# feldroop/floxer

Hardware: AMD Instinct MI355X
Metric: aligned reads/sec, 10 kb ONT-like reads @ 8 % error vs a GRCh38-size reference (seed-and-verify path, CIGAR) (higher is better)
Workload: dtype u64

## Files before the change

### floxer_amd/__init__.py

```python
import ctypes as C

import numpy as np

from . import capi
from .capi import FloxerError, check, lib, ptr, as_u8, u8p, u32p, u64p

if capi.os.path.exists(capi.LIB_PATH):
    lib()

CIGAR_OPS = "MIDNSHP=X"
NULL_ID = 0xFFFFFFFF

ORDER = {"errors_first": 0, "count_first": 1, "none": 2}
CHOICE = {"round_robin": 0, "full_groups": 1, "first_reported": 2}
MODE_EXISTS, MODE_WITHOUT_CIGAR, MODE_WITH_CIGAR = 0, 1, 2


def hw_queue_request():
    requested, found = C.c_int(0), C.c_int(-1)
    check(lib().flx_hw_queue_request(C.byref(requested), C.byref(found)))
    return requested.value, found.value


def cigar_string(words):
# ... 21 lines not shown

def reverse_complement_rank(r):
    r = as_u8(r)
    out = np.zeros_like(r)
    lib().flx_reverse_complement_rank(ptr(r, u8p), len(r), ptr(out, u8p))
    return out


class pex_tree:

    def __init__(self, total_query_length, query_num_errors, leaf_max_num_errors, bottom_up=False):
        cap = 4 * (query_num_errors + 2) + 16
        nodes = (capi.PexNode * cap)()
        ni, nl = C.c_uint64(), C.c_uint64()
        check(lib().flx_pex_tree_build(total_query_length, query_num_errors, leaf_max_num_errors, int(bottom_up), nodes, cap,
                                       C.byref(ni), C.byref(nl)))
        rows = [(n.parent_id, n.from_, n.to, n.num_errors) for n in nodes[: ni.value + nl.value]]
        self.inner_nodes = rows[: ni.value]
        self.leaves = rows[ni.value:]

    def root(self):
        return self.inner_nodes[0] if self.inner_nodes else self.leaves[0]

    def get_leaves(self):
        return self.leaves

    def generate_seeds(self, step=1):
        return [(l[1], l[2] - l[1] + 1, l[3], i) for i, l in enumerate(self.leaves)][::step]


class fmindex:
    def __init__(self, references=None, path=None, device=None):
        self.h = C.c_void_p()
        if path is not None and references is None:
            check(lib().flx_index_load(path.encode(), C.byref(self.h)))
        else:
            refs = [as_u8(r) for r in references]
            pool = np.concatenate(refs) if refs else np.zeros(0, np.uint8)
            lens = np.array([len(r) for r in refs], dtype=np.uint64)
            if device is None:
                check(lib().flx_index_build(ptr(pool, u8p), ptr(lens, u64p), len(refs), C.byref(self.h)))
            else:
                check(lib().flx_index_build_on_device(int(device), ptr(pool, u8p), ptr(lens, u64p), len(refs), C.byref(self.h)))

    def save(self, path):
        check(lib().flx_index_save(self.h, path.encode()))

    def meta(self):
        n = C.c_uint64(0)
        lib().flx_index_meta_export(self.h, None, C.byref(n))
        buf = np.zeros(n.value, dtype=np.uint8)
        check(lib().flx_index_meta_export(self.h, ptr(buf, u8p), C.byref(n)))
        return buf.tobytes()

    @classmethod
    def from_meta(cls, meta):
        self = cls.__new__(cls)
        self.h = C.c_void_p()
        buf = np.frombuffer(meta, dtype=np.uint8).copy()
        check(lib().flx_index_meta_import(ptr(buf, u8p), len(buf), C.byref(self.h)))
        return self

    def image_layout(self):
        out = np.zeros(5, dtype=np.uint64)
        check(lib().flx_index_image_layout(self.h, ptr(out, u64p)))
        return [int(x) for x in out]

    def image_upload(self, device, pointers):
        arr = (C.c_void_p * 5)(*[C.c_void_p(int(p)) for p in pointers])
        check(lib().flx_index_image_upload(self.h, int(device), arr))

    def __del__(self):
        if getattr(self, "h", None):
            lib().flx_index_free(self.h)
            self.h = None

    @property
    def text_length(self):
        return lib().flx_index_text_length(self.h)

    @property
    def num_references(self):
        return lib().flx_index_num_references(self.h)

    @property
    def device_bytes(self):
        return lib().flx_index_device_bytes(self.h)

    @property
    def derived_device_bytes(self):
        return lib().flx_index_derived_device_bytes(self.h)

    def suffix_array(self):
        out = np.zeros(self.text_length, dtype=np.uint64)
        check(lib().flx_index_copy_sa(self.h, ptr(out, u64p)))
        return out

    def suffix_array_u32(self):
        out = np.empty(self.text_length, dtype=np.uint32)
        check(lib().flx_index_copy_sa_u32(self.h, ptr(out, u32p)))
        return out

    def bwt(self, reversed_text=False):
        out = np.zeros(self.text_length, dtype=np.uint8)
        check(lib().flx_index_copy_bwt(self.h, int(reversed_text), ptr(out, u8p)))
        return out


class context:

    def __init__(self, index, device=0, image=None):
        self.index = index
        self.image = image
        self.h = C.c_void_p()
        if image is None:
            check(lib().flx_ctx_create(device, index.h, C.byref(self.h)))
        else:
            arr = (C.c_void_p * 5)(*[C.c_void_p(int(b.data_ptr())) for b in image])
            sizes = np.array([int(b.numel()) * int(b.element_size()) for b in image], dtype=np.uint64)
            check(lib().flx_ctx_create_on_image(device, index.h, arr, ptr(sizes, u64p), C.byref(self.h)))

    def close(self):
        if getattr(self, "h", None):
            lib().flx_ctx_destroy(self.h)
            self.h = None

    __del__ = close

    def set_stream(self, hip_stream):
        check(lib().flx_ctx_set_stream(self.h, hip_stream))

    def enable_kernel_timing(self, on=True):
        check(lib().flx_ctx_enable_kernel_timing(self.h, int(on)))

    def reset_kernel_stats(self):
        check(lib().flx_ctx_reset_kernel_stats(self.h))

    def path_counters(self, reset=False):
        pc = capi.PathCounters()
        check(lib().flx_ctx_get_path_counters(self.h, C.byref(pc)))
        if reset:
            check(lib().flx_ctx_reset_path_counters(self.h))
        out = {n: int(getattr(pc, n)) for n, _ in capi.PathCounters._fields_ if n != "reserved"}
        out["records_dropped"] = int(pc.reserved[0])
        out["partial_records"] = int(pc.reserved[1])
        out["reads_rescued"] = int(pc.reserved[2])
        out["reads_split"] = int(pc.reserved[3])
        return out

    def search_counters(self):
        sc = capi.SearchCounters()
        check(lib().flx_ctx_get_search_counters(self.h, C.byref(sc)))
        return {n: int(getattr(sc, n)) for n, _ in capi.SearchCounters._fields_ if n != "reserved"}

    def derived_info(self):
        di = capi.DerivedInfo()
        check(lib().flx_ctx_derived_info(self.h, C.byref(di)))
        return {n: int(getattr(di, n)) for n, _ in capi.DerivedInfo._fields_ if n != "reserved"}

    def copy_derived(self, which):
        if which == "isa":
            out = np.empty(self.index.text_length, dtype=np.uint32)
        else:
            out = np.empty((4 ** self.derived_info()["filter_k"] + 63) // 64, dtype=np.uint64)
        check(lib().flx_ctx_copy_derived(self.h, {"isa": 0, "filter": 1, "filter_mirrored": 2}[which], out.ctypes.data_as(C.c_void_p), out.nbytes))
        return out

    def lane_overlap(self, n_lanes, iterations):
        start, stop = (C.c_float * n_lanes)(), (C.c_float * n_lanes)()
        check(lib().flx_ctx_lane_overlap(self.h, n_lanes, iterations, start, stop))
        return list(start), list(stop)

    def kernel_stats(self):
        arr = (capi.KernelStat * 64)()
        n = C.c_uint32(64)
        check(lib().flx_ctx_get_kernel_stats(self.h, arr, C.byref(n)))
        return {a.name.decode(): dict(launches=a.launches, device_ms=a.device_ms, algorithmic_bytes=a.algorithmic_bytes,
                                      work_units=a.work_units) for a in arr[: n.value]}


class statistics:

    def __init__(self, input_hint=None):
        self.h = C.c_void_p()
        check(lib().flx_stats_create(input_hint.encode() if input_hint else None, C.byref(self.h)))

    def __del__(self):
        if getattr(self, "h", None):
            lib().flx_stats_free(self.h)
            self.h = None

    def attach(self, ctx):
        check(lib().flx_ctx_set_stats(ctx.h, self.h))
        return self

    @property
    def num_queries(self):
        return lib().flx_stats_num_queries(self.h)

    def format(self, toml=True):
        n = C.c_uint64(0)
        lib().flx_stats_format(self.h, int(toml), None, C.byref(n))
        buf = C.create_string_buffer(n.value)
        check(lib().flx_stats_format(self.h, int(toml), buf, C.byref(n)))
        return buf.value.decode()


def search_config(max_num_anchors_hard=500, max_num_anchors_soft=50, anchor_group_order="count_first",
                  anchor_choice_strategy="round_robin", erase_useless_anchors=True):
    return capi.SearchConfig(max_num_anchors_hard, max_num_anchors_soft, ORDER[anchor_group_order], CHOICE[anchor_choice_strategy],
                             int(erase_useless_anchors), 0)


class searcher:
    def __init__(self, ctx, config=None):
        self.ctx = ctx
        self.config = config or search_config()

    def _seeds(self, seeds):
        arr = (capi.Seed * len(seeds))()
        for i, (off, ln, err, leaf) in enumerate(seeds):
            arr[i] = capi.Seed(off, ln, err, leaf, 0)
        return arr

    def search_seeds(self, sequence, seeds):
        seq = as_u8(sequence)
        arr = self._seeds(seeds)
        cap = max(64, len(seeds) * (self.config.max_num_anchors_soft + 1))
        out = (capi.Anchor * cap)()
        n = C.c_uint64(cap)
        stats = (capi.SeedStats * max(1, len(seeds)))()
        check(lib().flx_search_seeds(self.ctx.h, ptr(seq, u8p), len(seq), arr, len(seeds), C.byref(self.config), out, C.byref(n), stats))
        anchors = np.array([(a.seed_index, a.pex_leaf_index, a.reference_id, a.reference_position, a.num_errors) for a in out[: n.value]],
                           dtype=np.uint64).reshape(-1, 5)
        st = np.array([(s.num_kept_useful_anchors, s.num_kept_raw_anchors, s.num_excluded_raw_anchors_by_soft_cap, s.fully_excluded)
                       for s in stats[: len(seeds)]], dtype=np.uint64).reshape(-1, 4)
        return anchors, st

    def search_groups(self, sequence, seeds, max_hits=501):
        seq = as_u8(sequence)
        arr = self._seeds(seeds)
        cap = 1 << 16
        while True:
            out = (capi.HitGroup * cap)()
            n = C.c_uint64(cap)
            rc = lib().flx_search_groups(self.ctx.h, ptr(seq, u8p), len(seq), arr, len(seeds), max_hits, out, C.byref(n))
            if rc == -3:
                cap = n.value
                continue
            check(rc)
            break
        return np.array([(g.seed_index, g.lb, g.len, g.num_errors) for g in out[: n.value]], dtype=np.uint64).reshape(-1, 4)


def align_batch(ctx, query_pool, jobs, reference_pool=None, md=False, gaps=None):
    q = as_u8(query_pool)
    arr = (capi.AlignJob * max(1, len(jobs)))()
    cap_words = 16
    for i, (ro, rl, qo, ql, k, mode) in enumerate(jobs):
        arr[i] = capi.AlignJob(ro, qo, rl, ql, k, mode)
        cap_words += 2 * k + 2
    res = (capi.AlignResult * max(1, len(jobs)))()
    cig = np.zeros(cap_words, dtype=np.uint32)
    words = C.c_uint64(cap_words)
    if reference_pool is None:
        rp, rl_ = None, 0
    else:
        ref = as_u8(reference_pool)
        rp, rl_ = ptr(ref, u8p), len(ref)
    if md:
        cap_md = 16 + sum(8 * k + 6 for (_, _, _, _, k, mode) in jobs if mode == MODE_WITH_CIGAR)
        refs = (capi.MdRef * max(1, len(jobs)))()
        mdp = np.zeros(cap_md, dtype=np.uint8)
        md_bytes = C.c_uint64(cap_md)
        if gaps is not None:
            check(lib().flx_align_batch_gaps(ctx.h, rp, rl_, ptr(q, u8p), len(q), arr, len(jobs), res, ptr(cig, u32p), C.byref(words),
                                             refs, ptr(mdp, u8p), C.byref(md_bytes), C.byref(gaps)))
        else:
            check(lib().flx_align_batch_md(ctx.h, rp, rl_, ptr(q, u8p), len(q), arr, len(jobs), res, ptr(cig, u32p), C.byref(words),
                                           refs, ptr(mdp, u8p), C.byref(md_bytes)))
        out = []
        for r, m in zip(res[: len(jobs)], refs[: len(jobs)]):
            out.append((r.num_errors, r.begin, cigar_string(cig[r.cigar_offset: r.cigar_offset + r.cigar_length]),
                        mdp[m.offset: m.offset + m.length].tobytes() if m.length else None) if r.exists else None)
        return out
    if gaps is not None:
        check(lib().flx_align_batch_gaps(ctx.h, rp, rl_, ptr(q, u8p), len(q), arr, len(jobs), res, ptr(cig, u32p), C.byref(words),
                                         None, None, None, C.byref(gaps)))
    else:
        check(lib().flx_align_batch(ctx.h, rp, rl_, ptr(q, u8p), len(q), arr, len(jobs), res, ptr(cig, u32p), C.byref(words)))
    out = []
    for r in res[: len(jobs)]:
        out.append((r.num_errors, r.begin, cigar_string(cig[r.cigar_offset: r.cigar_offset + r.cigar_length])) if r.exists else None)
    return out


def _realign_room(options):
    if options is None or not options.enable:
        return (lambda nm: 2 * nm + 2), (lambda nm: 8 * nm + 6)
    sc = {k: int(getattr(options, k)) or v for k, v in REALIGN_DEFAULTS.items()}
    c_max = max(sc["match"] + sc["mismatch"], sc["gap_open"] + sc["gap_extend"] + sc["match"])
    c_min = min(sc["match"] + sc["mismatch"], sc["gap_open"] + sc["gap_extend"])
    col_min = min(sc["match"] + sc["mismatch"], sc["gap_extend"])
    return (lambda nm: max(2 * nm + 2, 2 * (nm * c_max // c_min) + 1)), (lambda nm: 8 * (nm * c_max // col_min) + 6)


# ... 1395 lines not shown
```

### floxer_amd/capi.py

```python
import ctypes as C
import importlib.util
import os
import sys

import numpy as np

_HERE = os.path.dirname(os.path.abspath(__file__))
LIB_PATH = os.environ.get("FLX_LIBRARY") or os.path.join(_HERE, "libfloxer_amd.so")

u8p = C.POINTER(C.c_uint8)
u32p = C.POINTER(C.c_uint32)
u64p = C.POINTER(C.c_uint64)


class FloxerError(RuntimeError):
    pass


class PexNode(C.Structure):
    _fields_ = [("parent_id", C.c_uint32), ("from_", C.c_uint32), ("to", C.c_uint32), ("num_errors", C.c_uint32)]


class Seed(C.Structure):
    _fields_ = [("seq_offset", C.c_uint64), ("length", C.c_uint32), ("num_errors", C.c_uint32), ("pex_leaf_index", C.c_uint32),
# ... 100 lines not shown
    _fields_ = [("offset", C.c_uint64), ("length", C.c_uint32), ("num_errors", C.c_uint32), ("score", C.c_int32), ("diag_lo", C.c_int32),
                ("diag_hi", C.c_int32), ("kept", C.c_uint32)]


class RealignCounters(C.Structure):
    _fields_ = [("paths_realigned", C.c_uint64), ("paths_changed", C.c_uint64), ("paths_kept", C.c_uint64), ("reserved", C.c_uint64 * 5)]


class CsOptions(C.Structure):
    _fields_ = [("form", C.c_uint32), ("reserved", C.c_uint32 * 7)]


CsJob = LeftAlignJob


class CoverageOptions(C.Structure):
    _fields_ = [("count_deletions", C.c_uint32), ("count_secondary", C.c_uint32), ("min_mapq", C.c_uint32), ("report_zero", C.c_uint32),
                ("reserved", C.c_uint32 * 4)]


class DepthRun(C.Structure):
    _fields_ = [("reference_id", C.c_int32), ("depth", C.c_uint32), ("start", C.c_uint64), ("end", C.c_uint64)]


class DepthWindow(C.Structure):
    _fields_ = [("reference_id", C.c_int32), ("max_depth", C.c_uint32), ("start", C.c_uint64), ("end", C.c_uint64), ("depth_sum", C.c_uint64),
                ("covered", C.c_uint64)]


class PileupOptions(C.Structure):
    _fields_ = [("count_secondary", C.c_uint32), ("min_mapq", C.c_uint32), ("min_depth", C.c_uint32), ("min_count", C.c_uint32),
                ("min_permille", C.c_uint32), ("reserved", C.c_uint32 * 3)]


class PileupSite(C.Structure):
    _fields_ = [("reference_id", C.c_int32), ("position", C.c_uint32), ("depth", C.c_uint32), ("del_", C.c_uint32), ("ins", C.c_uint32),
                ("alt", C.c_uint32 * 4), ("reserved", C.c_uint32)]


class SvOptions(C.Structure):
    _fields_ = [("min_length", C.c_uint32), ("max_distance", C.c_uint32), ("min_support", C.c_uint32), ("count_secondary", C.c_uint32),
                ("min_mapq", C.c_uint32), ("reserved", C.c_uint32 * 3), ("initial_capacity", C.c_uint64)]


class SvSignature(C.Structure):
    _fields_ = [("type", C.c_uint32), ("side_a", C.c_uint32), ("side_b", C.c_uint32), ("reserved", C.c_uint32), ("ref_a", C.c_int32),
                ("ref_b", C.c_int32), ("pos_a", C.c_uint32), ("q", C.c_uint32)]


class SvCluster(C.Structure):
    _fields_ = [("type", C.c_uint32), ("side_a", C.c_uint32), ("side_b", C.c_uint32), ("support", C.c_uint32), ("ref_a", C.c_int32),
                ("ref_b", C.c_int32), ("pos_a_min", C.c_uint32), ("pos_a_max", C.c_uint32), ("q_min", C.c_uint32), ("q_median", C.c_uint32),
                ("q_max", C.c_uint32), ("reserved", C.c_uint32)]


class ErrprofOptions(C.Structure):
    _fields_ = [("count_secondary", C.c_uint32), ("min_mapq", C.c_uint32), ("flush_threshold", C.c_uint32), ("reserved", C.c_uint32 * 5)]


class ConsensusOptions(C.Structure):
    _fields_ = [("count_secondary", C.c_uint32), ("min_mapq", C.c_uint32), ("min_depth", C.c_uint32), ("min_count", C.c_uint32),
                ("min_permille", C.c_uint32), ("mask_low_depth", C.c_uint32), ("reserved", C.c_uint32 * 2)]


class ConsensusChange(C.Structure):
    _fields_ = [("reference_id", C.c_int32), ("position", C.c_uint32), ("kind", C.c_uint32), ("ref_rank", C.c_uint32), ("alt_rank", C.c_uint32),
                ("length", C.c_uint32), ("count", C.c_uint32), ("cov", C.c_uint32), ("letters", C.c_uint64)]


class ConsensusAllele(C.Structure):
    _fields_ = [("reference_id", C.c_int32), ("position", C.c_uint32), ("length", C.c_uint32), ("count", C.c_uint32), ("letters", C.c_uint64)]


class VariantsOptions(C.Structure):
    _fields_ = [("count_secondary", C.c_uint32), ("min_mapq", C.c_uint32), ("min_depth", C.c_uint32), ("min_qual", C.c_uint32), ("max_del", C.c_uint32),
                ("cost_match", C.c_uint32), ("cost_mismatch", C.c_uint32), ("cost_het", C.c_uint32), ("prior_het", C.c_uint32), ("prior_hom", C.c_uint32),
                ("reserved", C.c_uint32 * 2)]


class Variant(C.Structure):
    _fields_ = [("reference_id", C.c_int32), ("position", C.c_uint32), ("kind", C.c_uint32), ("ref_rank", C.c_uint32), ("alt_rank", C.c_uint32),
                ("length", C.c_uint32), ("ref_count", C.c_uint32), ("alt_count", C.c_uint32), ("cov", C.c_uint32), ("gt", C.c_uint32), ("gq", C.c_uint32),
                ("qual", C.c_uint32), ("pl", C.c_uint32 * 3), ("reserved", C.c_uint32), ("letters", C.c_uint64)]


class VariantAllele(C.Structure):
    _fields_ = [("reference_id", C.c_int32), ("position", C.c_uint32), ("kind", C.c_uint32), ("length", C.c_uint32), ("count", C.c_uint32),
                ("reserved", C.c_uint32), ("letters", C.c_uint64)]


ERRPROF_SECTIONS = (("PAIR_EQ", 36), ("PAIR_X", 36), ("INS_LEN", 64), ("DEL_LEN", 64), ("INS_LETTER", 6), ("DEL_LETTER", 6), ("HP_DEL", 34), ("HP_INS", 34),
                    ("POS_MATCH", 100), ("POS_MISMATCH", 100), ("POS_INS", 100), ("POS_CLIP", 100), ("POS_DEL", 100), ("EQ_RUN", 256), ("IDENTITY", 101),
                    ("TOTALS", 8), ("reserved", 7))


class ErrprofTable(C.Structure):
    _fields_ = [(name, C.c_uint64 * n) for name, n in ERRPROF_SECTIONS]


class SortOptions(C.Structure):
    _fields_ = [("initial_capacity", C.c_uint64), ("tile_keys", C.c_uint32), ("reserved", C.c_uint32 * 5)]


class SortEntry(C.Structure):
    _fields_ = [("ordinal", C.c_uint64), ("reference_id", C.c_int32), ("position", C.c_int32), ("end", C.c_uint32), ("flag", C.c_uint32)]


class PafSummary(C.Structure):
    _fields_ = [(n, C.c_uint32) for n in ("query_start", "query_end", "ref_end", "matches", "mismatches", "ins_bases", "del_bases", "gap_opens")]


class PafOptions(C.Structure):
    _fields_ = [("write_cigar", C.c_uint32), ("write_unmapped", C.c_uint32), ("mapq_from_records", C.c_uint32), ("skip_secondary", C.c_uint32),
                ("reserved", C.c_uint32 * 4)]


class TailJob(C.Structure):
    _fields_ = [("cigar_offset", C.c_uint64), ("cigar_length", C.c_uint32), ("error_weight", C.c_uint32), ("x_drop", C.c_uint32),
                ("min_tail_rows", C.c_uint32)]


class TailResult(C.Structure):
    _fields_ = [(n, C.c_uint32) for n in ("left_rows", "left_cols", "left_errors", "left_words", "right_rows", "right_cols", "right_errors",
                                          "right_words")]


class ExtendJob(C.Structure):
    _fields_ = [("text_pos", C.c_uint64), ("q_pos", C.c_uint64), ("ref_limit", C.c_uint32), ("row_limit", C.c_uint32),
                ("direction", C.c_int32), ("error_weight", C.c_uint32), ("x_drop", C.c_uint32), ("max_errors", C.c_uint32)]


class ExtendResult(C.Structure):
    _fields_ = [("rows", C.c_uint32), ("cols", C.c_uint32), ("errors", C.c_uint32), ("stop_reason", C.c_uint32)]


class PartialCandidate(C.Structure):
    _fields_ = [("read_index", C.c_uint64), ("q_from", C.c_uint32), ("q_to", C.c_uint32), ("orientation", C.c_uint32),
                ("reference_id", C.c_int32), ("start", C.c_uint64), ("nm", C.c_uint32), ("cigar_length", C.c_uint32),
                ("cigar_offset", C.c_uint64)]


class MdRef(C.Structure):
    _fields_ = [("offset", C.c_uint64), ("length", C.c_uint32), ("reserved", C.c_uint32)]


class PathCounters(C.Structure):
    _fields_ = [(n, C.c_uint64) for n in ("seeds", "seeds_with_anchors", "seeds_excluded_by_hard_cap", "seeds_selected_on_host", "anchors",
                                          "cursor_extensions", "inner_tests_requested", "root_alignments_requested",
                                          "root_alignments_found", "records", "reads", "search_reruns")] + [("reserved", C.c_uint64 * 4)]


class SearchCounters(C.Structure):
    _fields_ = [(n, C.c_uint64) for n in ("launches", "subtrees_queued", "lane_handovers", "wave_handovers", "walks_abandoned")] + [("reserved", C.c_uint64 * 3)]


class ClimbAnchor(C.Structure):
    _fields_ = [("read", C.c_uint32), ("orientation", C.c_uint32), ("leaf", C.c_uint32), ("reference_id", C.c_uint32), ("position", C.c_uint64)]


class ClimbOptions(C.Structure):
    _fields_ = [("driver", C.c_uint32), ("reserved", C.c_uint32 * 3)]


class DerivedInfo(C.Structure):
    _fields_ = [(n, C.c_uint32) for n in ("filter_k", "filter_tmin", "have_isa", "have_filter", "have_filter_mirrored")] + [("reserved", C.c_uint32 * 3)]


class KernelStat(C.Structure):
    _fields_ = [("name", C.c_char * 32), ("launches", C.c_uint64), ("device_ms", C.c_double), ("algorithmic_bytes", C.c_uint64),
                ("work_units", C.c_uint64)]


EXPORTED = [
    "flx_last_error", "flx_version", "flx_ceil_div", "flx_floating_point_error_aware_ceil", "flx_saturate_value_to_int32_max",
    "flx_chars_to_rank_sequence", "flx_reverse_complement_rank", "flx_pex_tree_build", "flx_index_build", "flx_index_build_on_device", "flx_index_save",
    "flx_index_load", "flx_index_free", "flx_index_text_length", "flx_index_num_references", "flx_index_device_bytes", "flx_index_derived_device_bytes",
    "flx_index_copy_sa", "flx_index_copy_sa_u32", "flx_index_copy_bwt", "flx_ctx_create", "flx_ctx_destroy", "flx_ctx_set_stream", "flx_search_seeds",
    "flx_search_groups", "flx_align_batch", "flx_params_default", "flx_align_reads", "flx_reads_upload", "flx_reads_free",
    "flx_align_reads_resident", "flx_run_num_records",
    "flx_run_num_cigar_words", "flx_run_copy", "flx_run_free", "flx_ctx_enable_kernel_timing", "flx_ctx_reset_kernel_stats",
    "flx_ctx_get_kernel_stats", "flx_sam_open", "flx_sam_write", "flx_sam_close", "flx_sim_genome", "flx_sim_genome_repeats", "flx_sim_reads", "flx_ctx_get_path_counters",
    "flx_ctx_reset_path_counters", "flx_stats_create", "flx_stats_free", "flx_stats_merge", "flx_stats_num_queries", "flx_stats_format",
    "flx_ctx_set_stats", "flx_device_count", "flx_index_matches_reference", "flx_sam_set_threads", "flx_index_image_layout",
    "flx_index_image_upload", "flx_index_meta_export", "flx_index_meta_import", "flx_ctx_create_on_image",
    "flx_align_reads_with_options", "flx_align_reads_resident_with_options", "flx_select_records", "flx_assign_mapq", "flx_sam_set_mapq",
    "flx_align_reads_with_tags", "flx_align_reads_resident_with_tags", "flx_run_num_md_bytes", "flx_run_copy_md", "flx_align_batch_md",
    "flx_sam_write_tagged", "flx_align_reads_opt", "flx_align_reads_resident_opt", "flx_choose_partials", "flx_partial_mapq",
    "flx_extend_batch", "flx_sam_set_sa", "flx_align_reads_split", "flx_align_reads_resident_split", "flx_cigar_tails", "flx_cigar_tails_batch",
    "flx_align_shapes", "flx_align_reads_gaps", "flx_align_reads_resident_gaps", "flx_align_batch_gaps", "flx_left_align", "flx_left_align_batch",
    "flx_realign", "flx_realign_batch", "flx_align_batch_realign", "flx_ctx_get_realign_counters", "flx_align_reads_realign",
    "flx_align_reads_resident_realign", "flx_run_copy_scores", "flx_sam_write_scored",
    "flx_ctx_get_search_counters", "flx_climb_anchors", "flx_ctx_derived_info", "flx_ctx_copy_derived",
    "flx_hw_queue_request", "flx_ctx_lane_overlap",
    "flx_align_reads_cs", "flx_align_reads_resident_cs", "flx_run_num_cs_bytes", "flx_run_copy_cs", "flx_align_batch_cs", "flx_cs", "flx_cs_batch",
    "flx_sam_write_cs",
    "flx_coverage_create", "flx_coverage_create_for_lengths", "flx_coverage_free", "flx_coverage_add_run", "flx_coverage_add_records",
    "flx_coverage_absorb", "flx_coverage_finish", "flx_coverage_num_runs", "flx_coverage_copy_runs", "flx_coverage_num_windows",
    "flx_coverage_copy_windows", "flx_coverage_copy_depth", "flx_coverage_geometry", "flx_coverage_host",
    "flx_pileup_create", "flx_pileup_create_for_lengths", "flx_pileup_free", "flx_pileup_add_records", "flx_pileup_add_run",
    "flx_pileup_add_run_resident", "flx_pileup_absorb", "flx_pileup_finish", "flx_pileup_num_sites", "flx_pileup_copy_sites",
    "flx_pileup_copy_counts", "flx_pileup_host", "flx_pileup_sites_host",
    "flx_sort_create", "flx_sort_free", "flx_sort_add_records", "flx_sort_add_run", "flx_sort_finish", "flx_sort_num_records", "flx_sort_copy",
    "flx_sort_geometry", "flx_sort_host", "flx_sam_open_sorted",
    "flx_paf_create", "flx_paf_free", "flx_paf_summarize", "flx_paf_summarize_host", "flx_paf_open", "flx_paf_write", "flx_paf_close",
    "flx_sv_create", "flx_sv_create_for_lengths", "flx_sv_free", "flx_sv_add_records", "flx_sv_add_run", "flx_sv_absorb", "flx_sv_finish",
    "flx_sv_num_signatures", "flx_sv_copy_signatures", "flx_sv_num_clusters", "flx_sv_copy_clusters", "flx_sv_host", "flx_sv_clusters_host",
    "flx_errprof_create", "flx_errprof_create_for_text", "flx_errprof_free", "flx_errprof_add_records", "flx_errprof_add_run",
    "flx_errprof_add_run_resident", "flx_errprof_absorb", "flx_errprof_copy", "flx_errprof_host",
    "flx_consensus_create", "flx_consensus_create_for_text", "flx_consensus_free", "flx_consensus_add_records", "flx_consensus_add_run",
    "flx_consensus_add_run_resident", "flx_consensus_finish", "flx_consensus_num_letters", "flx_consensus_copy_letters",
    "flx_consensus_num_changes", "flx_consensus_copy_changes", "flx_consensus_num_alleles", "flx_consensus_copy_alleles",
    "flx_consensus_geometry", "flx_consensus_host",
    "flx_variants_create", "flx_variants_create_for_text", "flx_variants_free", "flx_variants_add_records", "flx_variants_add_run",
    "flx_variants_add_run_resident", "flx_variants_finish", "flx_variants_num_rows", "flx_variants_copy_rows", "flx_variants_num_alleles",
    "flx_variants_copy_alleles", "flx_variants_geometry", "flx_variants_genotype", "flx_variants_host",
    "flx_grid_caps",
]

_lib = None


def _share_torchs_hip_runtime():
    if os.environ.get("FLX_SYSTEM_HIP") == "1" or "torch" in sys.modules:
        return
    try:
        spec = importlib.util.find_spec("torch")
    except (ImportError, ValueError):
        spec = None
    if spec is None or not spec.origin:
        return
    path = os.path.join(os.path.dirname(spec.origin), "lib", "libamdhip64.so")
    if os.path.exists(path):
        C.CDLL(path, mode=C.RTLD_GLOBAL)


def hip_runtime_paths():
    with open("/proc/self/maps") as f:
        return sorted({line.split()[-1] for line in f if "libamdhip64" in line})


def lib():
    global _lib
    if _lib is not None:
        return _lib
    if not os.path.exists(LIB_PATH):
        raise FloxerError(f"{LIB_PATH} is missing: build it with `python -c 'import __graft_entry__ as g; g.build()'` "
                          "(floxer_amd has no CPU fallback)")
    _share_torchs_hip_runtime()
    L = C.CDLL(LIB_PATH)
    getenv = C.CDLL(None).getenv
    getenv.restype, getenv.argtypes = C.c_char_p, [C.c_char_p]
    value = getenv(b"GPU_MAX_HW_QUEUES")
    if value is None:
        os.environ.pop("GPU_MAX_HW_QUEUES", None)
    else:
        os.environ["GPU_MAX_HW_QUEUES"] = value.decode()
    L.flx_last_error.restype = C.c_char_p
    L.flx_version.restype = C.c_char_p
    L.flx_ceil_div.restype = C.c_uint64
    L.flx_ceil_div.argtypes = [C.c_uint64, C.c_uint64]
    L.flx_floating_point_error_aware_ceil.restype = C.c_uint64
    L.flx_floating_point_error_aware_ceil.argtypes = [C.c_double]
    L.flx_saturate_value_to_int32_max.restype = C.c_int32
    L.flx_saturate_value_to_int32_max.argtypes = [C.c_uint64]
    L.flx_chars_to_rank_sequence.argtypes = [C.c_char_p, C.c_uint64, u8p]
    L.flx_reverse_complement_rank.argtypes = [u8p, C.c_uint64, u8p]
    L.flx_pex_tree_build.argtypes = [C.c_uint64, C.c_uint64, C.c_uint64, C.c_int, C.POINTER(PexNode), C.c_uint64, u64p, u64p]
    L.flx_index_build.argtypes = [u8p, u64p, C.c_uint32, C.POINTER(C.c_void_p)]
    L.flx_index_build_on_device.argtypes = [C.c_int, u8p, u64p, C.c_uint32, C.POINTER(C.c_void_p)]
    L.flx_index_save.argtypes = [C.c_void_p, C.c_char_p]
    L.flx_index_load.argtypes = [C.c_char_p, C.POINTER(C.c_void_p)]
    L.flx_index_free.argtypes = [C.c_void_p]
    L.flx_index_text_length.restype = C.c_uint64
    L.flx_index_text_length.argtypes = [C.c_void_p]
    L.flx_index_num_references.restype = C.c_uint32
    L.flx_index_num_references.argtypes = [C.c_void_p]
    L.flx_index_device_bytes.restype = C.c_uint64
    L.flx_index_device_bytes.argtypes = [C.c_void_p]
    L.flx_index_derived_device_bytes.restype = C.c_uint64
    L.flx_index_derived_device_bytes.argtypes = [C.c_void_p]
    L.flx_index_copy_sa.argtypes = [C.c_void_p, u64p]
    L.flx_index_copy_sa_u32.argtypes = [C.c_void_p, u32p]
    L.flx_index_copy_bwt.argtypes = [C.c_void_p, C.c_int, u8p]
    L.flx_ctx_create.argtypes = [C.c_int, C.c_void_p, C.POINTER(C.c_void_p)]
    L.flx_ctx_destroy.argtypes = [C.c_void_p]
    L.flx_index_image_layout.argtypes = [C.c_void_p, u64p]
    L.flx_index_image_upload.argtypes = [C.c_void_p, C.c_int, C.POINTER(C.c_void_p)]
    L.flx_index_meta_export.argtypes = [C.c_void_p, u8p, u64p]
    L.flx_index_meta_import.argtypes = [u8p, C.c_uint64, C.POINTER(C.c_void_p)]
    L.flx_ctx_create_on_image.argtypes = [C.c_int, C.c_void_p, C.POINTER(C.c_void_p), u64p, C.POINTER(C.c_void_p)]
    L.flx_ctx_set_stream.argtypes = [C.c_void_p, C.c_void_p]
    L.flx_search_seeds.argtypes = [C.c_void_p, u8p, C.c_uint64, C.POINTER(Seed), C.c_uint64, C.POINTER(SearchConfig),
                                   C.POINTER(Anchor), u64p, C.POINTER(SeedStats)]
    L.flx_search_groups.argtypes = [C.c_void_p, u8p, C.c_uint64, C.POINTER(Seed), C.c_uint64, C.c_uint64, C.POINTER(HitGroup), u64p]
    L.flx_align_batch.argtypes = [C.c_void_p, u8p, C.c_uint64, u8p, C.c_uint64, C.POINTER(AlignJob), C.c_uint64,
                                  C.POINTER(AlignResult), u32p, u64p]
    L.flx_align_shapes.argtypes = [C.POINTER(AlignJob), C.c_uint64, C.POINTER(AlignShape)]
    L.flx_params_default.argtypes = [C.POINTER(Params)]
    L.flx_align_reads.argtypes = [C.c_void_p, C.POINTER(Params), u8p, u64p, C.c_uint64, C.POINTER(C.c_void_p)]
    L.flx_reads_upload.argtypes = [C.c_void_p, u8p, u64p, C.c_uint64, C.POINTER(C.c_void_p)]
    L.flx_reads_free.argtypes = [C.c_void_p]
    L.flx_align_reads_resident.argtypes = [C.c_void_p, C.POINTER(Params), C.c_void_p, C.POINTER(C.c_void_p)]
    L.flx_align_reads_with_options.argtypes = [C.c_void_p, C.POINTER(Params), u8p, u64p, C.c_uint64, C.POINTER(OutputOptions),
                                               C.POINTER(C.c_void_p)]
    L.flx_align_reads_resident_with_options.argtypes = [C.c_void_p, C.POINTER(Params), C.c_void_p, C.POINTER(OutputOptions),
                                                        C.POINTER(C.c_void_p)]
    L.flx_align_reads_with_tags.argtypes = [C.c_void_p, C.POINTER(Params), u8p, u64p, C.c_uint64, C.POINTER(OutputOptions),
                                            C.POINTER(TagOptions), C.POINTER(C.c_void_p)]
    L.flx_align_reads_resident_with_tags.argtypes = [C.c_void_p, C.POINTER(Params), C.c_void_p, C.POINTER(OutputOptions),
                                                     C.POINTER(TagOptions), C.POINTER(C.c_void_p)]
    L.flx_align_reads_opt.argtypes = [C.c_void_p, C.POINTER(Params), u8p, u64p, C.c_uint64, C.POINTER(RunOptions), C.POINTER(C.c_void_p)]
    L.flx_align_reads_resident_opt.argtypes = [C.c_void_p, C.POINTER(Params), C.c_void_p, C.POINTER(RunOptions), C.POINTER(C.c_void_p)]
    L.flx_align_reads_split.argtypes = [C.c_void_p, C.POINTER(Params), u8p, u64p, C.c_uint64, C.POINTER(RunOptions), C.POINTER(SplitOptions),
                                        C.POINTER(C.c_void_p)]
    L.flx_align_reads_resident_split.argtypes = [C.c_void_p, C.POINTER(Params), C.c_void_p, C.POINTER(RunOptions), C.POINTER(SplitOptions),
                                                 C.POINTER(C.c_void_p)]
    L.flx_align_reads_gaps.argtypes = [C.c_void_p, C.POINTER(Params), u8p, u64p, C.c_uint64, C.POINTER(RunOptions), C.POINTER(SplitOptions),
                                       C.POINTER(GapOptions), C.POINTER(C.c_void_p)]
    L.flx_align_reads_resident_gaps.argtypes = [C.c_void_p, C.POINTER(Params), C.c_void_p, C.POINTER(RunOptions), C.POINTER(SplitOptions),
                                                C.POINTER(GapOptions), C.POINTER(C.c_void_p)]
    L.flx_align_batch_gaps.argtypes = [C.c_void_p, u8p, C.c_uint64, u8p, C.c_uint64, C.POINTER(AlignJob), C.c_uint64,
                                       C.POINTER(AlignResult), u32p, u64p, C.POINTER(MdRef), u8p, u64p, C.POINTER(GapOptions)]
    L.flx_left_align.argtypes = [u8p, C.c_uint64, u8p, C.c_uint64, u32p, C.c_uint64, C.POINTER(LeftAlignJob), C.c_uint64, u32p, u64p,
                                 C.POINTER(CigarRef)]
    L.flx_left_align_batch.argtypes = [C.c_void_p] + L.flx_left_align.argtypes
    L.flx_realign.argtypes = [u8p, C.c_uint64, u8p, C.c_uint64, u32p, C.c_uint64, C.POINTER(RealignJob), C.c_uint64, C.POINTER(RealignOptions), u32p, u64p,
                              C.POINTER(RealignResult)]
    L.flx_realign_batch.argtypes = [C.c_void_p] + L.flx_realign.argtypes
    L.flx_align_batch_realign.argtypes = L.flx_align_batch_gaps.argtypes + [C.POINTER(RealignOptions), C.POINTER(C.c_int32)]
    L.flx_ctx_get_realign_counters.argtypes = [C.c_void_p, C.POINTER(RealignCounters)]
    L.flx_align_reads_realign.argtypes = L.flx_align_reads_gaps.argtypes[:-1] + [C.POINTER(RealignOptions), C.POINTER(C.c_void_p)]
    L.flx_align_reads_resident_realign.argtypes = L.flx_align_reads_resident_gaps.argtypes[:-1] + [C.POINTER(RealignOptions), C.POINTER(C.c_void_p)]
    L.flx_run_copy_scores.argtypes = [C.c_void_p, C.POINTER(C.c_int32)]
    L.flx_align_reads_cs.argtypes = L.flx_align_reads_realign.argtypes[:-1] + [C.POINTER(CsOptions), C.POINTER(C.c_void_p)]
    L.flx_align_reads_resident_cs.argtypes = L.flx_align_reads_resident_realign.argtypes[:-1] + [C.POINTER(CsOptions), C.POINTER(C.c_void_p)]
    L.flx_run_num_cs_bytes.restype = C.c_uint64
    L.flx_run_num_cs_bytes.argtypes = [C.c_void_p]
    L.flx_run_copy_cs.argtypes = [C.c_void_p, C.POINTER(MdRef), u8p]
    L.flx_align_batch_cs.argtypes = L.flx_align_batch_realign.argtypes + [C.POINTER(CsOptions), C.POINTER(MdRef), u8p, u64p]
    L.flx_cs.argtypes = [u8p, C.c_uint64, u8p, C.c_uint64, u32p, C.c_uint64, C.POINTER(CsJob), C.c_uint64, C.POINTER(CsOptions), u8p, u64p,
                         C.POINTER(MdRef)]
    L.flx_cs_batch.argtypes = [C.c_void_p] + L.flx_cs.argtypes
    L.flx_coverage_create.argtypes = [C.c_void_p, C.POINTER(CoverageOptions), C.POINTER(C.c_void_p)]
    L.flx_coverage_create_for_lengths.argtypes = [C.c_int, u64p, C.c_uint32, C.POINTER(CoverageOptions), C.POINTER(C.c_void_p)]
    L.flx_coverage_free.restype = None
# ... 7 lines not shown
    L.flx_coverage_copy_runs.argtypes = [C.c_void_p, C.POINTER(DepthRun), C.c_uint64]
    L.flx_coverage_num_windows.restype = C.c_uint64
    L.flx_coverage_num_windows.argtypes = [C.c_void_p, C.c_uint64]
    L.flx_coverage_copy_windows.argtypes = [C.c_void_p, C.c_uint64, C.POINTER(DepthWindow), C.c_uint64]
    L.flx_coverage_copy_depth.argtypes = [C.c_void_p, C.c_uint32, C.c_uint64, C.c_uint64, u32p]
    L.flx_coverage_geometry.argtypes = [u32p]
    L.flx_coverage_host.argtypes = [u64p, C.c_uint32, C.POINTER(CoverageOptions), C.POINTER(Record), C.c_uint64, u32p, C.c_uint64, u32p]
    L.flx_sort_create.argtypes = [C.c_int, C.c_uint32, C.POINTER(SortOptions), C.POINTER(C.c_void_p)]
    L.flx_sort_free.restype = None
    L.flx_sort_free.argtypes = [C.c_void_p]
    L.flx_sort_add_records.argtypes = [C.c_void_p, C.POINTER(Record), C.c_uint64, u32p, C.c_uint64, C.c_uint64, u32p]
    L.flx_sort_add_run.argtypes = [C.c_void_p, C.c_void_p, C.c_uint64, u32p]
    L.flx_sort_finish.argtypes = [C.c_void_p]
    L.flx_sort_num_records.restype = C.c_uint64
    L.flx_sort_num_records.argtypes = [C.c_void_p]
    L.flx_sort_copy.argtypes = [C.c_void_p, C.c_uint64, C.c_uint64, C.POINTER(SortEntry)]
    L.flx_sort_geometry.argtypes = [u32p]
    L.flx_grid_caps.argtypes = [u32p]
    L.flx_sort_host.argtypes = [C.c_uint32, C.POINTER(Record), C.c_uint64, u32p, C.c_uint64, u64p, C.POINTER(SortEntry)]
    L.flx_pileup_create.argtypes = [C.c_void_p, C.POINTER(PileupOptions), C.POINTER(C.c_void_p)]
    L.flx_pileup_create_for_lengths.argtypes = [C.c_int, u64p, C.c_uint32, C.POINTER(PileupOptions), C.POINTER(C.c_void_p)]
    L.flx_pileup_free.restype = None
    L.flx_pileup_free.argtypes = [C.c_void_p]
    L.flx_pileup_add_records.argtypes = [C.c_void_p, C.POINTER(Record), C.c_uint64, u32p, C.c_uint64, u8p, u64p, C.c_uint64]
    L.flx_pileup_add_run.argtypes = [C.c_void_p, C.c_void_p, u8p, u64p, C.c_uint64]
    L.flx_pileup_add_run_resident.argtypes = [C.c_void_p, C.c_void_p, C.c_void_p]
    L.flx_pileup_absorb.argtypes = [C.c_void_p, C.c_void_p]
    L.flx_pileup_finish.argtypes = [C.c_void_p]
    L.flx_pileup_num_sites.restype = C.c_uint64
    L.flx_pileup_num_sites.argtypes = [C.c_void_p]
    L.flx_pileup_copy_sites.argtypes = [C.c_void_p, C.POINTER(PileupSite), C.c_uint64]
    L.flx_pileup_copy_counts.argtypes = [C.c_void_p, C.c_uint32, C.c_uint64, C.c_uint64, u32p]
    L.flx_pileup_host.argtypes = [u64p, C.c_uint32, C.POINTER(PileupOptions), C.POINTER(Record), C.c_uint64, u32p, C.c_uint64, u8p, u64p, C.c_uint64, u32p]
    L.flx_pileup_sites_host.argtypes = [u64p, C.c_uint32, C.POINTER(PileupOptions), u32p, C.POINTER(PileupSite), u64p]
    L.flx_sv_create.argtypes = [C.c_void_p, C.POINTER(SvOptions), C.POINTER(C.c_void_p)]
    L.flx_sv_create_for_lengths.argtypes = [C.c_int, u64p, C.c_uint32, C.POINTER(SvOptions), C.POINTER(C.c_void_p)]
    L.flx_sv_free.restype = None
    L.flx_sv_free.argtypes = [C.c_void_p]
    L.flx_sv_add_records.argtypes = [C.c_void_p, C.POINTER(Record), C.c_uint64, u32p, C.c_uint64, u64p, C.c_uint64]
    L.flx_sv_add_run.argtypes = [C.c_void_p, C.c_void_p, u64p, C.c_uint64]
    L.flx_sv_absorb.argtypes = [C.c_void_p, C.c_void_p]
    L.flx_sv_finish.argtypes = [C.c_void_p]
    L.flx_sv_num_signatures.restype = C.c_uint64
    L.flx_sv_num_signatures.argtypes = [C.c_void_p]
    L.flx_sv_copy_signatures.argtypes = [C.c_void_p, C.c_uint64, C.c_uint64, C.POINTER(SvSignature)]
    L.flx_sv_num_clusters.restype = C.c_uint64
    L.flx_sv_num_clusters.argtypes = [C.c_void_p]
    L.flx_sv_copy_clusters.argtypes = [C.c_void_p, C.POINTER(SvCluster), C.c_uint64]
    L.flx_sv_host.argtypes = [u64p, C.c_uint32, C.POINTER(SvOptions), C.POINTER(Record), C.c_uint64, u32p, C.c_uint64, u64p, C.c_uint64,
                              C.POINTER(SvSignature), u64p]
    L.flx_sv_clusters_host.argtypes = [C.POINTER(SvOptions), C.POINTER(SvSignature), C.c_uint64, C.POINTER(SvCluster), u64p]
    L.flx_errprof_create.argtypes = [C.c_void_p, C.POINTER(ErrprofOptions), C.POINTER(C.c_void_p)]
    L.flx_errprof_create_for_text.argtypes = [C.c_int, u8p, u64p, C.c_uint32, C.POINTER(ErrprofOptions), C.POINTER(C.c_void_p)]
    L.flx_errprof_free.restype = None
    L.flx_errprof_free.argtypes = [C.c_void_p]
    L.flx_errprof_add_records.argtypes = [C.c_void_p, C.POINTER(Record), C.c_uint64, u32p, C.c_uint64, u8p, u64p, C.c_uint64]
    L.flx_errprof_add_run.argtypes = [C.c_void_p, C.c_void_p, u8p, u64p, C.c_uint64]
    L.flx_errprof_add_run_resident.argtypes = [C.c_void_p, C.c_void_p, C.c_void_p]
    L.flx_errprof_absorb.argtypes = [C.c_void_p, C.c_void_p]
    L.flx_errprof_copy.argtypes = [C.c_void_p, C.POINTER(ErrprofTable)]
    L.flx_errprof_host.argtypes = [u8p, u64p, C.c_uint32, C.POINTER(ErrprofOptions), C.POINTER(Record), C.c_uint64, u32p, C.c_uint64, u8p, u64p, C.c_uint64,
                                   C.POINTER(ErrprofTable)]
    L.flx_consensus_create.argtypes = [C.c_void_p, C.POINTER(ConsensusOptions), C.POINTER(C.c_void_p)]
    L.flx_consensus_create_for_text.argtypes = [C.c_int, u8p, u64p, C.c_uint32, C.POINTER(ConsensusOptions), C.POINTER(C.c_void_p)]
    L.flx_consensus_free.restype = None
    L.flx_consensus_free.argtypes = [C.c_void_p]
    L.flx_consensus_add_records.argtypes = [C.c_void_p, C.POINTER(Record), C.c_uint64, u32p, C.c_uint64, u8p, u64p, C.c_uint64]
    L.flx_consensus_add_run.argtypes = [C.c_void_p, C.c_void_p, u8p, u64p, C.c_uint64]
    L.flx_consensus_add_run_resident.argtypes = [C.c_void_p, C.c_void_p, C.c_void_p]
    L.flx_consensus_finish.argtypes = [C.c_void_p]
    L.flx_consensus_num_letters.restype = C.c_uint64
    L.flx_consensus_num_letters.argtypes = [C.c_void_p, C.c_uint32]
    L.flx_consensus_copy_letters.argtypes = [C.c_void_p, C.c_uint32, C.c_char_p, C.c_uint64]
    L.flx_consensus_num_changes.restype = C.c_uint64
    L.flx_consensus_num_changes.argtypes = [C.c_void_p]
    L.flx_consensus_copy_changes.argtypes = [C.c_void_p, C.POINTER(ConsensusChange), C.c_uint64]
    L.flx_consensus_num_alleles.restype = C.c_uint64
    L.flx_consensus_num_alleles.argtypes = [C.c_void_p]
    L.flx_consensus_copy_alleles.argtypes = [C.c_void_p, C.POINTER(ConsensusAllele), C.c_uint64]
    L.flx_consensus_geometry.argtypes = [u32p]
    L.flx_consensus_host.argtypes = [u8p, u64p, C.c_uint32, C.POINTER(ConsensusOptions), C.POINTER(Record), C.c_uint64, u32p, C.c_uint64, u8p, u64p, C.c_uint64,
                                     u64p, C.c_char_p, u64p, C.POINTER(ConsensusChange), u64p, C.POINTER(ConsensusAllele), u64p]
    L.flx_variants_create.argtypes = [C.c_void_p, C.POINTER(VariantsOptions), C.POINTER(C.c_void_p)]
    L.flx_variants_create_for_text.argtypes = [C.c_int, u8p, u64p, C.c_uint32, C.POINTER(VariantsOptions), C.POINTER(C.c_void_p)]
    L.flx_variants_free.restype = None
    L.flx_variants_free.argtypes = [C.c_void_p]
    L.flx_variants_add_records.argtypes = [C.c_void_p, C.POINTER(Record), C.c_uint64, u32p, C.c_uint64, u8p, u64p, C.c_uint64]
    L.flx_variants_add_run.argtypes = [C.c_void_p, C.c_void_p, u8p, u64p, C.c_uint64]
    L.flx_variants_add_run_resident.argtypes = [C.c_void_p, C.c_void_p, C.c_void_p]
    L.flx_variants_finish.argtypes = [C.c_void_p]
    L.flx_variants_num_rows.restype = C.c_uint64
    L.flx_variants_num_rows.argtypes = [C.c_void_p]
    L.flx_variants_copy_rows.argtypes = [C.c_void_p, C.POINTER(Variant), C.c_uint64]
    L.flx_variants_num_alleles.restype = C.c_uint64
    L.flx_variants_num_alleles.argtypes = [C.c_void_p]
    L.flx_variants_copy_alleles.argtypes = [C.c_void_p, C.POINTER(VariantAllele), C.c_uint64]
    L.flx_variants_geometry.argtypes = [u32p]
    L.flx_variants_genotype.argtypes = [C.POINTER(VariantsOptions), C.c_uint64, C.c_uint64, C.c_uint64, u32p]
    L.flx_variants_host.argtypes = [u8p, u64p, C.c_uint32, C.POINTER(VariantsOptions), C.POINTER(Record), C.c_uint64, u32p, C.c_uint64, u8p, u64p, C.c_uint64,
                                    C.POINTER(Variant), u64p, C.POINTER(VariantAllele), u64p]
    L.flx_paf_create.argtypes = [C.c_int, C.POINTER(C.c_void_p)]
    L.flx_paf_free.restype = None
    L.flx_paf_free.argtypes = [C.c_void_p]
    L.flx_paf_summarize.argtypes = [C.c_void_p, C.POINTER(Record), C.c_uint64, u32p, C.c_uint64, u64p, C.c_uint64, u64p, C.c_uint32, C.POINTER(PafSummary)]
    L.flx_paf_summarize_host.argtypes = [C.POINTER(Record), C.c_uint64, u32p, C.c_uint64, u64p, C.c_uint64, u64p, C.c_uint32, C.POINTER(PafSummary)]
    L.flx_paf_open.argtypes = [C.c_char_p, C.POINTER(C.c_char_p), u64p, C.c_uint32, C.POINTER(PafOptions), C.POINTER(C.c_void_p)]
    L.flx_paf_write.argtypes = [C.c_void_p, C.POINTER(C.c_char_p), u64p, C.POINTER(Record), C.c_uint64, u32p, C.POINTER(PafSummary), C.POINTER(C.c_int32),
                                C.POINTER(MdRef), u8p]
    L.flx_paf_close.argtypes = [C.c_void_p]
    L.flx_cigar_tails.argtypes = [u32p, C.c_uint64, C.POINTER(TailJob), C.c_uint64, C.POINTER(TailResult)]
    L.flx_cigar_tails_batch.argtypes = [C.c_void_p, u32p, C.c_uint64, C.POINTER(TailJob), C.c_uint64, C.POINTER(TailResult)]
    L.flx_choose_partials.argtypes = [C.POINTER(PartialCandidate), C.c_uint64, u32p, C.POINTER(PartialOptions), C.POINTER(C.c_int32)]
    L.flx_partial_mapq.argtypes = [C.POINTER(PartialCandidate), C.c_uint64, u32p, C.POINTER(C.c_int32), u8p]
    L.flx_run_num_md_bytes.restype = C.c_uint64
    L.flx_run_num_md_bytes.argtypes = [C.c_void_p]
    L.flx_run_copy_md.argtypes = [C.c_void_p, C.POINTER(MdRef), u8p]
    L.flx_align_batch_md.argtypes = [C.c_void_p, u8p, C.c_uint64, u8p, C.c_uint64, C.POINTER(AlignJob), C.c_uint64,
                                     C.POINTER(AlignResult), u32p, u64p, C.POINTER(MdRef), u8p, u64p]
    L.flx_sam_write_tagged.argtypes = [C.c_void_p, C.POINTER(C.c_char_p), u8p, u64p, C.POINTER(C.c_char_p), C.POINTER(Record), C.c_uint64, u32p,
                                       C.POINTER(MdRef), u8p]
    L.flx_sam_write_scored.argtypes = L.flx_sam_write_tagged.argtypes + [C.POINTER(C.c_int32)]
    L.flx_sam_write_cs.argtypes = L.flx_sam_write_scored.argtypes + [C.POINTER(MdRef), u8p]
    L.flx_select_records.argtypes = [C.POINTER(Record), C.c_uint64, u32p, C.POINTER(OutputOptions), u8p]
    L.flx_assign_mapq.argtypes = [C.POINTER(Record), C.c_uint64, u32p, u64p, u8p]
    L.flx_run_num_records.restype = C.c_uint64
    L.flx_run_num_records.argtypes = [C.c_void_p]
    L.flx_run_num_cigar_words.restype = C.c_uint64
    L.flx_run_num_cigar_words.argtypes = [C.c_void_p]
    L.flx_run_copy.argtypes = [C.c_void_p, C.POINTER(Record), u32p, u8p]
    L.flx_run_free.argtypes = [C.c_void_p]
    L.flx_ctx_enable_kernel_timing.argtypes = [C.c_void_p, C.c_int]
    L.flx_ctx_reset_kernel_stats.argtypes = [C.c_void_p]
    L.flx_ctx_get_kernel_stats.argtypes = [C.c_void_p, C.POINTER(KernelStat), u32p]
    L.flx_sam_open.argtypes = [C.c_char_p, C.POINTER(C.c_char_p), u64p, C.c_uint32, C.POINTER(C.c_void_p)]
    L.flx_sam_write.argtypes = [C.c_void_p, C.POINTER(C.c_char_p), u8p, u64p, C.POINTER(C.c_char_p), C.POINTER(Record), C.c_uint64, u32p]
    L.flx_sam_close.argtypes = [C.c_void_p]
    L.flx_sam_open_sorted.argtypes = [C.c_char_p, C.c_char_p, C.c_int, C.c_int, C.POINTER(C.c_char_p), u64p, C.c_uint32, C.POINTER(C.c_void_p)]
    L.flx_stats_create.argtypes = [C.c_char_p, C.POINTER(C.c_void_p)]
    L.flx_stats_free.argtypes = [C.c_void_p]
    L.flx_stats_merge.argtypes = [C.c_void_p, C.c_void_p]
    L.flx_stats_num_queries.restype = C.c_uint64
    L.flx_stats_num_queries.argtypes = [C.c_void_p]
    L.flx_stats_format.argtypes = [C.c_void_p, C.c_int, C.c_char_p, u64p]
    L.flx_ctx_set_stats.argtypes = [C.c_void_p, C.c_void_p]
    L.flx_device_count.restype = C.c_int
    L.flx_index_matches_reference.argtypes = [C.c_void_p, u8p, u64p, C.c_uint32]
    L.flx_sam_set_threads.argtypes = [C.c_void_p, C.c_uint32]
    L.flx_sam_set_mapq.argtypes = [C.c_void_p, C.c_int]
    L.flx_sam_set_sa.argtypes = [C.c_void_p, C.c_int]
    L.flx_extend_batch.argtypes = [C.c_void_p, u8p, C.c_uint64, u8p, C.c_uint64, C.POINTER(ExtendJob), C.c_uint64, C.POINTER(ExtendResult)]
    L.flx_ctx_get_path_counters.argtypes = [C.c_void_p, C.POINTER(PathCounters)]
    L.flx_ctx_reset_path_counters.argtypes = [C.c_void_p]
    L.flx_ctx_get_search_counters.argtypes = [C.c_void_p, C.POINTER(SearchCounters)]
    L.flx_climb_anchors.argtypes = [C.c_void_p, C.POINTER(Params), C.c_void_p, C.c_void_p, C.c_uint64, C.POINTER(ClimbOptions), u8p, u32p, u64p]
    L.flx_ctx_derived_info.argtypes = [C.c_void_p, C.POINTER(DerivedInfo)]
    L.flx_ctx_copy_derived.argtypes = [C.c_void_p, C.c_int, C.c_void_p, C.c_uint64]
    L.flx_hw_queue_request.argtypes = [C.POINTER(C.c_int), C.POINTER(C.c_int)]
    L.flx_ctx_lane_overlap.argtypes = [C.c_void_p, C.c_uint32, C.c_uint32, C.POINTER(C.c_float), C.POINTER(C.c_float)]
    L.flx_sim_genome.argtypes = [C.c_uint64, C.c_uint64, u8p]
    L.flx_sim_genome_repeats.argtypes = [C.c_uint64, C.c_uint64, u8p]
    L.flx_sim_reads.argtypes = [u8p, u64p, C.c_uint32, C.c_uint64, C.c_uint32, C.c_double, C.c_double, C.c_uint64, u8p, C.c_uint64,
                                u64p, u32p, u64p, u8p]
    _lib = L
    return L


def check(rc):
    if rc != 0:
        raise FloxerError(f"floxer_amd error {rc}: {lib().flx_last_error().decode()}")


def ptr(a, t):
    return a.ctypes.data_as(t)


def as_u8(x):
    return np.ascontiguousarray(np.asarray(x, dtype=np.uint8))
```

### floxer_amd/csrc/flx_capi.cpp

```cpp
#include <algorithm>
#include <cstdlib>
#include <cstring>
#include <malloc.h>
#include <memory>
#include <mutex>
#include <thread>

#include "flx_context.hpp"
#include "flx_fm_core.hpp"

namespace flx {
const char* last_error_cstr();
}
using namespace flx;

extern "C" {

int flx_index_build_on_device(int hip_device, const uint8_t* concat, const uint64_t* lens, uint32_t n_refs, flx_index** out) {
    if (!concat || !lens || !out || n_refs == 0) { set_error("flx_index_build_on_device: null argument or no reference"); return FLX_ERR_INVALID; }
    int count = 0;
    if (hipGetDeviceCount(&count) != hipSuccess || count <= 0) { (void)hipGetLastError(); set_error("flx_index_build_on_device: no HIP device"); return FLX_ERR_NO_DEVICE; }
    if (hip_device < 0 || hip_device >= count) { set_error("flx_index_build_on_device: device ordinal out of range"); return FLX_ERR_INVALID; }
    HostIndex* h = build_host_index(concat, lens, n_refs, hip_device);
    if (!h) return FLX_ERR_INVALID;
// ... 126 lines not shown
        (void)DeviceApi::derived_bytes(H.n, &fk);
        bool have_isa = false;
        {
            size_t free_i = 0, total_i = 0;
            FLX_HIP(hipMemGetInfo(&free_i, &total_i));
            size_t const want = (size_t)H.n * 4 + 64;
            have_isa = want < free_i / 2 && ctx->isa.ensure(want, true) == FLX_OK;
        }
        bool have_filter = false, have_filter_m = false;
        if (fk) {
            size_t free_f = 0, total_f = 0;
            FLX_HIP(hipMemGetInfo(&free_f, &total_f));
            size_t const want = (size_t)(((1ull << (2 * fk)) + 63) / 64) * 8;
            have_filter = want < free_f / 2 && ctx->filter.ensure(want, true) == FLX_OK;
            if (have_filter && getenv("FLX_MIRRORED_FILTER")) {
                FLX_HIP(hipMemGetInfo(&free_f, &total_f));
                have_filter_m = want < free_f / 2 && ctx->filter_m.ensure(want, true) == FLX_OK;
            }
        }
        int const e = DeviceApi::derive_index(s0, ctx->didx, have_isa ? ctx->isa.as<u32>() : nullptr, have_filter ? ctx->filter.as<u64>() : nullptr, have_filter_m ? ctx->filter_m.as<u64>() : nullptr);
        if (e) { set_error(std::string("derive_index: ") + hipGetErrorString((hipError_t)e)); return FLX_ERR_NO_DEVICE; }
        FLX_HIP(hipStreamSynchronize(s0));
    }
    if (getenv("FLX_ALLOC_DEBUG"))
        fprintf(stderr, "[flx alloc] context: occ0 %p occ1 %p sa %p text %p kmer %p (n %llu) isa %p filter %p (K %u, tmin %u) seq_start %p\n", img[0], img[1], img[2], img[3],
                img[4], (unsigned long long)H.n, ctx->isa.ptr, ctx->filter.ptr, ctx->didx.filter_k, ctx->didx.filter_tmin, ctx->seq_start.ptr);
    for (auto& lane : ctx->lanes) {
        int const e = DeviceApi::warm_scratch(lane->stream);
        if (e) { set_error(std::string("warm_scratch: ") + hipGetErrorString((hipError_t)e)); return FLX_ERR_NO_DEVICE; }
    }
    for (auto& lane : ctx->lanes) FLX_HIP(hipStreamSynchronize(lane->stream));
    size_t free_b = 0, total_b = 0;
    FLX_HIP(hipMemGetInfo(&free_b, &total_b));
    size_t budget = std::min<size_t>(free_b / 10 * 4, n_lanes * ((size_t)4 << 30));
    if (const char* env = getenv("FLX_TRACE_ARENA_MB")) { size_t const mb = strtoull(env, nullptr, 10); if (mb) budget = mb << 20; }
    budget = std::max<size_t>(budget, (size_t)256 << 20);
    for (auto& lane : ctx->lanes) lane->trace_budget_bytes = std::max<size_t>(budget / n_lanes, (size_t)128 << 20);
    if (const char* env = getenv("FLX_TRACE_ARENA_KB")) { size_t const kb = strtoull(env, nullptr, 10); if (kb) for (auto& lane : ctx->lanes) lane->trace_budget_bytes = kb << 10; }
    *out = ctx.release();
    return FLX_OK;
}
}

int flx_ctx_create(int hip_device, const flx_index* index, flx_ctx** out) {
    if (!index || !out) { set_error("flx_ctx_create: null argument"); return FLX_ERR_INVALID; }
    if (int const rc = check_device(hip_device, "flx_ctx_create")) return rc;
    if (!has_arrays(*index->host)) { set_error("flx_ctx_create: this index holds no arrays (flx_index_meta_import): use flx_ctx_create_on_image"); return FLX_ERR_INVALID; }
    return make_context(hip_device, index, nullptr, true, out);
}

int flx_ctx_create_on_image(int hip_device, const flx_index* index, void* const device_buffers[5], const flx_index_image* sizes, flx_ctx** out) {
    if (!index || !out || !device_buffers || !sizes) { set_error("flx_ctx_create_on_image: null argument"); return FLX_ERR_INVALID; }
    for (int i = 0; i < 5; ++i) if (!device_buffers[i]) { set_error("flx_ctx_create_on_image: null device buffer"); return FLX_ERR_INVALID; }
    {
        uint64_t want[5];
        image_sizes(*index->host, want);
        for (int i = 0; i < 5; ++i)
            if (sizes->bytes[i] != want[i]) { set_error("flx_ctx_create_on_image: the buffers' sizes are not this index's image layout (flx_index_image_layout)"); return FLX_ERR_INVALID; }
    }
    if (int const rc = check_device(hip_device, "flx_ctx_create_on_image")) return rc;
    return make_context(hip_device, index, device_buffers, false, out);
}

int flx_index_image_layout(const flx_index* index, flx_index_image* out) {
    if (!index || !out) { set_error("flx_index_image_layout: null argument"); return FLX_ERR_INVALID; }
    image_sizes(*index->host, out->bytes);
    return FLX_OK;
}

int flx_index_image_upload(const flx_index* index, int hip_device, void* const device_buffers[5]) {
    if (!index || !device_buffers) { set_error("flx_index_image_upload: null argument"); return FLX_ERR_INVALID; }
    if (!has_arrays(*index->host)) { set_error("flx_index_image_upload: this index holds no arrays"); return FLX_ERR_INVALID; }
    if (int const rc = check_device(hip_device, "flx_index_image_upload")) return rc;
    FLX_HIP(hipSetDevice(hip_device));
    return upload_image(*index->host, device_buffers, nullptr);
}

flx_ctx::~flx_ctx() {
    (void)hipSetDevice(device);
    for (auto& lane : lanes) { if (lane->stream) (void)hipStreamSynchronize(lane->stream); lane->release_all(); }
    for (DeviceBuffer* b : {&occ0, &occ1, &sa, &text, &text_rev, &kmer, &seq_start, &isa, &filter}) b->release();
    if (upload_stream) (void)hipStreamDestroy(upload_stream);
}

int flx_ctx_destroy(flx_ctx* ctx) {
    if (!ctx) return FLX_OK;
    {
        std::lock_guard<std::mutex> g(ctx->spare_mu);
        if (ctx->live_reads > 0) { set_error("flx_ctx_destroy: " + std::to_string(ctx->live_reads) + " read batch(es) of this context are still alive (flx_reads_free them first)"); return FLX_ERR_INVALID; }
        if (ctx->live_errprofs > 0) { set_error("flx_ctx_destroy: " + std::to_string(ctx->live_errprofs) + " error-profile object(s) of this context are still alive (flx_errprof_free them first)"); return FLX_ERR_INVALID; }
        if (ctx->live_consensus > 0) { set_error("flx_ctx_destroy: " + std::to_string(ctx->live_consensus) + " consensus object(s) of this context are still alive (flx_consensus_free them first)"); return FLX_ERR_INVALID; }
        if (ctx->live_variants > 0) { set_error("flx_ctx_destroy: " + std::to_string(ctx->live_variants) + " variants object(s) of this context are still alive (flx_variants_free them first)"); return FLX_ERR_INVALID; }
    }
    delete ctx;
    return FLX_OK;
}

int flx_ctx_set_stream(flx_ctx* ctx, void* hip_stream) {
    if (!ctx) { set_error("null context"); return FLX_ERR_INVALID; }
    int rc = ctx->sync_all();
    if (rc) return rc;
    Lane* l0 = ctx->lane0();
    l0->stream = hip_stream ? (hipStream_t)hip_stream : l0->own_stream;
    ctx->external_stream = hip_stream != nullptr;
    return FLX_OK;
}

int flx_ctx_enable_kernel_timing(flx_ctx* ctx, int enable) {
    if (!ctx) { set_error("null context"); return FLX_ERR_INVALID; }
    int rc = ctx->sync_all();
    if (rc) return rc;
    ctx->timing = enable != 0;
    return FLX_OK;
}
int flx_ctx_reset_kernel_stats(flx_ctx* ctx) {
    if (!ctx) { set_error("null context"); return FLX_ERR_INVALID; }
    int rc = ctx->sync_all();
    if (rc) return rc;
    std::lock_guard<std::mutex> g(ctx->mu);
    ctx->stats.clear();
    ctx->stat_order.clear();
    return FLX_OK;
}
int flx_ctx_get_kernel_stats(flx_ctx* ctx, flx_kernel_stat* out, uint32_t* n) {
    if (!ctx || !n) { set_error("null argument"); return FLX_ERR_INVALID; }
    int rc = ctx->sync_all();
    if (rc) return rc;
    std::lock_guard<std::mutex> g(ctx->mu);
    uint32_t const cap = *n;
    *n = (uint32_t)ctx->stat_order.size();
    if (ctx->stat_order.size() > cap || (!out && cap)) { set_error("stat buffer too small"); return FLX_ERR_CAPACITY; }
    for (size_t i = 0; i < ctx->stat_order.size(); ++i) out[i] = ctx->stats[ctx->stat_order[i]];
    return FLX_OK;
}

int flx_ctx_set_stats(flx_ctx* ctx, flx_stats* stats) {
    if (!ctx) { set_error("null context"); return FLX_ERR_INVALID; }
    int const rc = ctx->sync_all();
    if (rc) return rc;
    ctx->read_stats = stats;
    return FLX_OK;
}
int flx_ctx_get_path_counters(flx_ctx* ctx, flx_path_counters* out) {
    if (!ctx || !out) { set_error("null argument"); return FLX_ERR_INVALID; }
    std::lock_guard<std::mutex> g(ctx->mu);
    *out = ctx->path;
    return FLX_OK;
}
int flx_ctx_reset_path_counters(flx_ctx* ctx) {
    if (!ctx) { set_error("null context"); return FLX_ERR_INVALID; }
    std::lock_guard<std::mutex> g(ctx->mu);
    ctx->path = flx_path_counters{};
    ctx->search = flx_search_counters{};
    ctx->realign = flx_realign_counters{};
    return FLX_OK;
}
int flx_ctx_get_realign_counters(flx_ctx* ctx, flx_realign_counters* out) {
    if (!ctx || !out) { set_error("null argument"); return FLX_ERR_INVALID; }
    std::lock_guard<std::mutex> g(ctx->mu);
    *out = ctx->realign;
    return FLX_OK;
}
int flx_ctx_get_search_counters(flx_ctx* ctx, flx_search_counters* out) {
    if (!ctx || !out) { set_error("null argument"); return FLX_ERR_INVALID; }
    std::lock_guard<std::mutex> g(ctx->mu);
    *out = ctx->search;
    return FLX_OK;
}

int flx_ctx_derived_info(flx_ctx* ctx, flx_derived_info* out) {
    if (!ctx || !out) { set_error("flx_ctx_derived_info: null argument"); return FLX_ERR_INVALID; }
    *out = flx_derived_info{};
    out->filter_k = ctx->didx.filter_k;
    out->filter_tmin = ctx->didx.filter_tmin;
    out->have_isa = ctx->didx.isa != nullptr;
    out->have_filter = ctx->didx.filter != nullptr;
    out->have_filter_mirrored = ctx->didx.filter_m != nullptr;
    return FLX_OK;
}
int flx_ctx_copy_derived(flx_ctx* ctx, int which, void* out, uint64_t bytes) {
    if (!ctx || !out) { set_error("flx_ctx_copy_derived: null argument"); return FLX_ERR_INVALID; }
    const void* src = nullptr;
    uint64_t want = 0;
    switch (which) {
        case 0: src = ctx->didx.isa; want = (uint64_t)ctx->didx.n * 4; break;
        case 1: src = ctx->didx.filter; want = filter_words(ctx->didx.filter_k) * 8; break;
        case 2: src = ctx->didx.filter_m; want = filter_words(ctx->didx.filter_k) * 8; break;
        default: set_error("flx_ctx_copy_derived: which must be 0 (inverse suffix array), 1 (filter) or 2 (mirrored filter)"); return FLX_ERR_INVALID;
    }
    if (!src) { set_error("flx_ctx_copy_derived: this context has no such table"); return FLX_ERR_INVALID; }
    if (bytes != want) { set_error("flx_ctx_copy_derived: the table holds " + std::to_string(want) + " bytes, the caller gave " + std::to_string(bytes)); return FLX_ERR_INVALID; }
    FLX_HIP(hipSetDevice(ctx->device));
    FLX_HIP(hipMemcpy(out, src, want, hipMemcpyDeviceToHost));
    return FLX_OK;
}

int flx_ctx_lane_overlap(flx_ctx* ctx, uint32_t n_lanes, uint32_t iterations, float* start_ms, float* stop_ms) {
    if (!ctx || !start_ms || !stop_ms) { set_error("flx_ctx_lane_overlap: null argument"); return FLX_ERR_INVALID; }
    if (n_lanes == 0 || n_lanes > ctx->lanes.size()) { set_error("flx_ctx_lane_overlap: the context has " + std::to_string(ctx->lanes.size()) + " lanes, the caller asked for " + std::to_string(n_lanes)); return FLX_ERR_INVALID; }
    for (uint32_t l = 0; l < n_lanes; ++l)
        if (!ctx->lanes[l]->own_stream) { set_error("flx_ctx_lane_overlap: lane " + std::to_string(l) + " has no stream of its own (FLX_STREAMS)"); return FLX_ERR_INVALID; }
    iterations = std::min<uint32_t>(iterations, 1u << 24);
    int rc = ctx->sync_all();
    if (rc) return rc;
    FLX_HIP(hipSetDevice(ctx->device));
    struct Probe {
        hipEvent_t ref = nullptr;
        std::vector<hipEvent_t> a, b;
        u32* out = nullptr;
        ~Probe() {
            for (hipEvent_t e : a) if (e) (void)hipEventDestroy(e);
            for (hipEvent_t e : b) if (e) (void)hipEventDestroy(e);
            if (ref) (void)hipEventDestroy(ref);
            if (out) (void)hipFree(out);
        }
    } p;
    p.a.assign(n_lanes, nullptr);
    p.b.assign(n_lanes, nullptr);
    FLX_HIP(hipEventCreate(&p.ref));
    for (uint32_t l = 0; l < n_lanes; ++l) { FLX_HIP(hipEventCreate(&p.a[l])); FLX_HIP(hipEventCreate(&p.b[l])); }
    FLX_HIP(hipMalloc((void**)&p.out, (size_t)n_lanes * 64 * sizeof(u32)));
    FLX_HIP(hipEventRecord(p.ref, ctx->lanes[0]->own_stream));
    for (uint32_t l = 0; l < n_lanes && !rc; ++l) {
        hipStream_t const s = ctx->lanes[l]->own_stream;
        FLX_HIP(hipEventRecord(p.a[l], s));
        rc = DeviceApi::lane_overlap_probe(s, iterations, p.out + (size_t)l * 64);
        FLX_HIP(hipEventRecord(p.b[l], s));
    }
    for (uint32_t l = 0; l < n_lanes; ++l) FLX_HIP(hipStreamSynchronize(ctx->lanes[l]->own_stream));
    if (rc) { set_error(std::string("lane_overlap_probe: ") + hipGetErrorString((hipError_t)rc)); return FLX_ERR_NO_DEVICE; }
    for (uint32_t l = 0; l < n_lanes; ++l) {
        FLX_HIP(hipEventElapsedTime(&start_ms[l], p.ref, p.a[l]));
        FLX_HIP(hipEventElapsedTime(&stop_ms[l], p.ref, p.b[l]));
    }
    return FLX_OK;
}

}
```

### floxer_amd/csrc/flx_context.hpp

```cpp
#pragma once

#include <hip/hip_runtime.h>

#include <condition_variable>
#include <map>
#include <memory>
#include <mutex>
#include <string>
#include <vector>

#include "flx_internal.hpp"

namespace flx {

#define FLX_HIP(expr)                                                                                   \
    do {                                                                                                \
        hipError_t const e__ = (expr);                                                                  \
        if (e__ != hipSuccess) {                                                                        \
            set_error(std::string(#expr) + ": " + hipGetErrorString(e__));                              \
            return FLX_ERR_NO_DEVICE;                                                                   \
        }                                                                                               \
    } while (0)

#define FLX_LAUNCH(name, rc)                                                                            \
    do {                                                                                                \
        int const e__ = (rc);                                                                           \
        if (e__ != 0) {                                                                                 \
            set_error(std::string(name) + ": launch failed: " + hipGetErrorString((hipError_t)e__));    \
            return FLX_ERR_NO_DEVICE;                                                                   \
        }                                                                                               \
    } while (0)

struct DeviceBuffer {
    void* ptr = nullptr;
    size_t cap = 0;
    DeviceBuffer() = default;
    DeviceBuffer(DeviceBuffer const&) = delete;
    DeviceBuffer& operator=(DeviceBuffer const&) = delete;
    ~DeviceBuffer() { release(); }
    int ensure(size_t bytes, bool exact = false);
    void release();
    void take(DeviceBuffer& other) { release(); ptr = other.ptr; cap = other.cap; other.ptr = nullptr; other.cap = 0; }
    template <class T> T* as() const { return reinterpret_cast<T*>(ptr); }
};

struct PinnedBuffer {
    void* ptr = nullptr;
    size_t cap = 0;
    PinnedBuffer() = default;
    PinnedBuffer(PinnedBuffer const&) = delete;
    PinnedBuffer& operator=(PinnedBuffer const&) = delete;
    ~PinnedBuffer() { release(); }
    int ensure(size_t bytes);
    void release();
};

struct PendingTiming { std::string name; hipEvent_t start, stop; u64 bytes, units; };

}


struct flx_ctx;
struct flx_stats;

namespace flx {
struct Lane {
    flx_ctx* ctx = nullptr;
    int id = 0;
    hipStream_t own_stream = nullptr, stream = nullptr;
    DeviceBuffer seq, seq_rev, peq, peq_rev, scheme, seeds, stack, hits, counters, rows, rows_out, qpack, items;
    DeviceBuffer jobs, job_out, trace, tjobs, tjob_out, cigar, md, md_out, user_text, user_text_rev, lastrow, row_windows, row_out,
        seed_cnt, hit_off, grouped, sel_stat, sel_n, sel_off, sel_out, sel_tmp, sel_rows, sel_row_off, sel_sparse, sel_lists, vr, seed_gen, mailboxes, ext_jobs, ext_out, tail_jobs, tail_out, cigar_la, la_jobs, la_stat, cigar_ra, ra_jobs, ra_stat, cs, cs_jobs, cs_out;
    size_t trace_budget_bytes = 0;
    std::vector<PendingTiming> pending;
    std::vector<hipEvent_t> event_pool;
    hipEvent_t sync_event = nullptr;
    u32* vr_host_scalars = nullptr;
    PinnedBuffer staging;
    void* stage_begin(size_t bytes);
    PinnedBuffer results;
    size_t results_used = 0;
    static constexpr size_t RESULT_BLOCK_BYTES = 1u << 20;
    size_t results_limit = RESULT_BLOCK_BYTES;
    bool results_limit_read = false;
    void* result_slot(size_t bytes);
    bool has_run = false;
    double hits_per_seed = 0, items_per_seed = 0, sel_rows_per_seed = 0;
    int wait_idle();
    int sync();
    std::vector<DeviceBuffer*> workspaces();
    int size_like(Lane& other);
    hipEvent_t get_event();
    void release_all();
};
}

struct flx_ctx {
    ~flx_ctx();
    int device = 0;
    const flx::HostIndex* hidx = nullptr;
    flx::DevIndex didx{};
    flx::DeviceBuffer occ0, occ1, sa, text, text_rev, kmer, seq_start;
    flx::DeviceBuffer isa, filter, filter_m;
    bool text_rev_ready = false;
    std::mutex mu;
    std::vector<std::unique_ptr<flx::Lane>> lanes;
    hipStream_t upload_stream = nullptr;
    std::mutex spare_mu;
    std::vector<std::unique_ptr<flx::DeviceBuffer>> spare_read_buffers[5];
    int live_reads = 0;
    int live_errprofs = 0;
    int live_consensus = 0;
    int live_variants = 0;
    bool external_stream = false;
    bool timing = false;
    std::map<std::string, flx_kernel_stat> stats;
    std::vector<std::string> stat_order;
    flx_path_counters path{};
    flx_realign_counters realign{};
    flx_search_counters search{};
    flx_stats* read_stats = nullptr;

    std::mutex lane_mu;
    std::condition_variable lane_cv;
    std::vector<int> free_lanes;
    flx::Lane* acquire_lane(int wanted = -1);
    void release_lane(flx::Lane* lane);
    void warm_one_cold_lane(flx::Lane* like);

    int k1_tokens = 0;
    int k1_running = 0;
    void k1_acquire();
    void k1_release();

    flx::Lane* lane0() { return lanes[0].get(); }
    int sync_all();
    void account(const char* name, flx::u64 bytes, flx::u64 units, hipEvent_t start, hipEvent_t stop);
    void account_more(const char* name, flx::u64 bytes, flx::u64 units);
};

namespace flx {

struct LaneLease {
    flx_ctx* ctx;
    Lane* lane;
    explicit LaneLease(flx_ctx* c, int wanted = -1) : ctx(c), lane(c->acquire_lane(wanted)) {}
    ~LaneLease() { ctx->release_lane(lane); }
    LaneLease(LaneLease const&) = delete;
    LaneLease& operator=(LaneLease const&) = delete;
};

struct ResultScope {
    Lane* lane;
    size_t mark;
    explicit ResultScope(Lane* l) : lane(l), mark(l->results_used) {}
    ~ResultScope() { lane->results_used = mark; }
    ResultScope(ResultScope const&) = delete;
    ResultScope& operator=(ResultScope const&) = delete;
};

template <class F>
int timed_launch(Lane* lane, const char* name, u64 bytes, u64 units, F&& launch) {
    if (!lane->ctx->timing) {
        FLX_LAUNCH(name, launch());
        return FLX_OK;
    }
    hipEvent_t const a = lane->get_event(), b = lane->get_event();
    FLX_HIP(hipEventRecord(a, lane->stream));
    int const rc = launch();
    FLX_HIP(hipEventRecord(b, lane->stream));
    FLX_LAUNCH(name, rc);
    lane->pending.push_back(PendingTiming{name, a, b, bytes, units});
    return FLX_OK;
}

}
```

### floxer_amd/csrc/flx_device.hip

```cpp
#include <hip/hip_runtime.h>

#include <algorithm>
#include <cstdio>
#include <cstdlib>
#include <type_traits>
#include <utility>

#include "flx_internal.hpp"
#include "flx_wave.hpp"

namespace flx {

__device__ __forceinline__ u32 wave_max_u32(u32 v) {
#pragma unroll
    for (int off = 32; off > 0; off >>= 1) {
        u32 const o = (u32)__shfl_xor((int)v, off);
        v = v > o ? v : o;
    }
    return (u32)__builtin_amdgcn_readfirstlane((int)v);
}

__global__ void __launch_bounds__(256) peq_build_kernel(const u8* __restrict__ seq, u64 len, u64* __restrict__ peq, u64 n_words) {
    u64 const wave = ((u64)blockIdx.x * blockDim.x + threadIdx.x) >> 6;
    if (wave >= n_words) return;
    u64 const pos = wave * 64 + lane_id();
    u32 const sym = pos < len ? seq[pos] : 7u;
#pragma unroll
    for (u32 s = 0; s < 6; ++s) {
        u64 const m = __ballot(sym == s);
        if (lane_id() == s) peq[wave * 6 + s] = m;
    }
}

int DeviceApi::build_peq(void* stream, const u8* d_seq, u64 len, u64* d_peq) {
    u64 const n_words = len / 64 + 2;
    u64 const threads = n_words * 64;
    hipLaunchKernelGGL(peq_build_kernel, dim3((unsigned)((threads + 255) / 256)), dim3(256), 0, (hipStream_t)stream, d_seq, len,
                       d_peq, n_words);
    return (int)hipGetLastError();
}

static const u32 kWordsPerLane[] = {1, 2, 3, 4, 5, 6, 8, 13, 25};

template <int W, bool TRACE>
__device__ __forceinline__ void ed_block_body(const u8* __restrict__ text, const u64* __restrict__ peq, const DevAlignJob* __restrict__ jobs, u32 n_jobs,
                                              u32 log2_r, DevAlignOut* __restrict__ out, u32 blk, u64* __restrict__ lds_eq,
                                              u64* __restrict__ trace, u16* __restrict__ lastrow, u32 queue, u32* __restrict__ err) {
    u32 const lane = lane_id();
    u32 const R = 1u << log2_r;
    u32 const p = lane & (R - 1u);
    u32 const jobs_per_wave = 64u >> log2_r;
    u32 const job_id = blk * jobs_per_wave + (lane >> log2_r);
    bool valid = job_id < n_jobs;
    DevAlignJob job;
    if (valid) job = jobs[job_id];
    else { job.ref_off = 0; job.q_off = 0; job.trace_off = 0; job.n = 0; job.m = 1; job.k = 0; job.out_index = 0; }
    int const n = (int)job.n, m = (int)job.m, k = (int)job.k;
    if (valid && (n == 0 || n + k < m)) {
        if (p == 0u) { DevAlignOut o; o.score = (n == 0 && m <= k) ? (u32)m : 0xFFFFFFFFu; o.end_col = 0u; out[job.out_index] = o; }
        valid = false;
    }
    int const nw = (m + 63) >> 6;
    int const Lg = (nw + W - 1) / W;
    int const band_hi = n - m + k;
    u32 const src_lane = (lane & ~(R - 1u)) | ((lane - 1u) & (R - 1u));
    int delay = valid ? (int)ring_delay((u32)n, (u32)m, (u32)k, (u32)W, R) : 0;
    if (delay > 0 && (u32)delay + 1u > queue) {
        if (err && p == 0u) atomicOr(err, 1u);
        if (p == 0u) { DevAlignOut o; o.score = 0xFFFFFFFFu; o.end_col = 0u; out[job.out_index] = o; }
        valid = false;
        delay = 0;
    }
    bool const any_delay = __any(delay > 0);
    uint2* __restrict__ const hand = reinterpret_cast<uint2*>(lds_eq + 7u * 64u * W) + (size_t)(lane >> log2_r) * queue;
    u32 const qmask = queue - 1u;
    auto offset_of = [&](int gg) { return gg + (gg >> log2_r) * delay; };
#pragma unroll
    for (int w = 0; w < W; ++w) lds_eq[(6u * 64u + lane) * W + w] = 0ull;

    int const pad = Lg * 64 * W - m;
    int g = (int)p;
    int b_lo = 0, b_hi = -1, rows_g = 0;
    int above_b_hi = 0;
    int off_g = 0;
    u64 vp[W], vn[W];
    auto enter_group = [&]() {
        int const r0 = max(0, 64 * W * g - pad);
        int const r1 = 64 * W * (g + 1) - pad;
        rows_g = r1 - r0;
        b_lo = max(0, r0 - k) >> 4;
        b_hi = min(n - 1, r1 - 1 + band_hi) >> 4;
        if (g + 1 < Lg) b_hi = max(b_hi, max(0, r1 - k) >> 4);
        above_b_hi = max(min(n - 1, r0 - 1 + band_hi) >> 4, b_lo);
        off_g = offset_of(g);
#pragma unroll
        for (int w = 0; w < W; ++w) {
            int const rs = 64 * (g * W + w) - pad;
            u64 const padmask = rs <= -64 ? ~0ull : rs < 0 ? (1ull << (u32)(-rs)) - 1ull : 0ull;
            i64 const off = (i64)job.q_off + rs;
#pragma unroll
            for (u32 s = 0; s < 6; ++s) {
                u64 v = 0;
                if (rs > -64) {
                    if (off >= 0) {
                        u64 const a = (u64)off >> 6;
                        u32 const sh = (u32)off & 63u;
                        u64 const lo = peq[a * 6 + s];
                        u64 const hi = peq[(a + 1) * 6 + s];
                        v = sh ? (lo >> sh) | (hi << (64 - sh)) : lo;
                    } else v = peq[s] << (u32)(-off);
                }
                lds_eq[(s * 64u + lane) * W + w] = v | padmask;
            }
            lds_eq[(6u * 64u + lane) * W + w] = padmask;
            vp[w] = ~padmask;
            vn[w] = 0ull;
        }
    };
    bool const has_group = valid && g < Lg;
    if (has_group) enter_group();
    else {
#pragma unroll
        for (int w = 0; w < W; ++w) { vp[w] = ~0ull; vn[w] = 0ull; }
    }
    u32 const my_steps = valid ? (u32)(((n - 1) >> 4) + offset_of(Lg - 1) + 1) : 0u;
    u32 const t_max = wave_max_u32(my_steps);
    const u8* __restrict__ ref = text + job.ref_off;
    u32* __restrict__ carry_out = nullptr;
    ulonglong2* __restrict__ ckpt_out = nullptr;
    if (TRACE) {
        TraceLayout const tl = ckpt_trace_layout(job.n, job.m, job.k, (u32)W, R);
        carry_out = reinterpret_cast<u32*>(reinterpret_cast<ulonglong2*>(trace) + job.trace_off);
        ckpt_out = reinterpret_cast<ulonglong2*>(trace) + job.trace_off + tl.carry_slots;
    }

    u32 cw_out = 0x55555555u;
    int botv_out = 0;
    int bot = 0, best = m, best_col = 0;
    uint4 tq_pre = make_uint4(0, 0, 0, 0);
    int pre_b = -1;
    bool pend = false, pend_last = false;
    u64 pend_slot = 0;
    int pend_b = 0;
    u32 cbits[W];
    u32 rowv[8];
    auto flush = [&]() {
        if (TRACE && pend) {
#pragma unroll
            for (int w = 0; w < W; ++w) carry_out[pend_slot + w] = cbits[w];
            if (pend_last && lastrow) {
                uint4* __restrict__ dst = reinterpret_cast<uint4*>(lastrow + job.lastrow_off + 16 * (u64)pend_b);
                dst[0] = make_uint4(rowv[0], rowv[1], rowv[2], rowv[3]);
                dst[1] = make_uint4(rowv[4], rowv[5], rowv[6], rowv[7]);
            }
            pend = false;
        }
    };
    for (u32 T = 0; T < t_max; ++T) {
        int b = (int)T - off_g;
        if (has_group && b > b_hi && g + (int)R < Lg) {
            g += (int)R;
            enter_group();
            b = (int)T - off_g;
        }
        u32 cw_in = (u32)__shfl((int)cw_out, (int)src_lane);
        int botv_in = __shfl(botv_out, (int)src_lane);
        if (any_delay) {
            if (delay > 0 && p == R - 1u) hand[(T - 1u) & qmask] = make_uint2(cw_out, (u32)botv_out);
            if (delay > 0 && p == 0u && g >= (int)R) { uint2 const h = hand[(T - 1u - (u32)delay) & qmask]; cw_in = h.x; botv_in = (int)h.y; }
        }
        bool const active = has_group && b >= b_lo && b <= b_hi;
        if (active) {
            if (g == 0) { cw_in = 0u; botv_in = 0; }
            else if (b > above_b_hi) cw_in = 0x55555555u;
            if (b == b_lo) bot = botv_in + rows_g;
            int const bot_start = bot;
            bool const last = g == Lg - 1;
            uint4 tq = tq_pre;
            if (pre_b != b) __builtin_memcpy(&tq, ref + 16 * b, 16);
            u32 const quad[4] = {tq.x, tq.y, tq.z, tq.w};
            u32 cw = 0;
            u64 const slot = ((u64)T * R + p) * W;
            flush();
            if (TRACE) {
#pragma unroll
                for (int w = 0; w < W; ++w) {
                    ulonglong2 v;
                    v.x = vp[w];
                    v.y = vn[w];
                    ckpt_out[slot + w] = v;
                    cbits[w] = 0;
                }
#pragma unroll
                for (int q = 0; q < 8; ++q) rowv[q] = 0xFFFFFFFFu;
            }
            if (b < b_hi) { __builtin_memcpy(&tq_pre, ref + 16 * (b + 1), 16); pre_b = b + 1; }
            auto block16 = [&](auto track_tag) {
                constexpr bool TRACK = decltype(track_tag)::value;
                u32 qv[4] = {quad[0], quad[1], quad[2], quad[3]};
                u32 cwi = cw_in;
                int bb = b;
                asm volatile("" : "+v"(qv[0]), "+v"(qv[1]), "+v"(qv[2]), "+v"(qv[3]), "+v"(cwi), "+v"(bb));
                u32 acc = 0;
#pragma unroll
                for (int qd = 0; qd < 4; ++qd) {
                    __builtin_amdgcn_sched_barrier(0);
#pragma unroll
                    for (int i = 0; i < 4; ++i) {
                        int const j = 4 * qd + i;
                        int const c = 16 * bb + j;
                        u32 sym = (qv[qd] >> (8 * i)) & 0xFFu;
                        sym = c < n ? sym : 6u;
                        u64 c_hp = (cwi >> (2 * j)) & 1u, c_hn = (cwi >> (2 * j + 1)) & 1u;
                        const u64* __restrict__ eqp = &lds_eq[(sym * 64u + lane) * W];
                        u64 hp_last = 0, hn_last = 0;
#pragma unroll
                        for (int w = 0; w < W; ++w) {
                            if (TRACE) cbits[w] |= ((u32)c_hp | ((u32)c_hn << 1)) << (2 * j);
                            u64 const eq = eqp[w];
                            u64 const pv = vp[w], mv = vn[w];
                            u64 const x = eq | mv;
                            u64 const tt = pv + (x & pv) + c_hn;
                            u64 const d0 = (tt ^ pv) | x;
                            u64 const hn = pv & d0;
                            u64 const hp = mv | ~(pv | d0);
                            u64 const xh = (hp << 1) | c_hp;
                            vn[w] = xh & d0;
                            vp[w] = (hn << 1) | ~(xh | d0) | c_hn;
                            if (w + 1 < W || TRACK) { c_hp = hp >> 63; c_hn = hn >> 63; }
                            if (w + 1 == W) { hp_last = hp; hn_last = hn; }
                        }
                        if (TRACK) {
                            acc |= ((u32)c_hp | ((u32)c_hn << 1)) << (2 * j);
                            bot += (int)(u32)c_hp - (int)(u32)c_hn;
                            if (last && c < n && bot <= best) { best = bot; best_col = c + 1; }
                            if (TRACE && c < n) {
                                u32 const v16 = (u32)min(bot, 0xFFFF);
                                rowv[j >> 1] = (j & 1) ? (rowv[j >> 1] & 0xFFFFu) | (v16 << 16) : (rowv[j >> 1] & 0xFFFF0000u) | v16;
                            }
                        } else {
                            acc = (acc >> 2) | (((u32)(hp_last >> 32) >> 1) & 0x40000000u) | ((u32)(hn_last >> 32) & 0x80000000u);
                        }
                    }
                }
                if (!TRACK) bot += (int)__popc(acc & 0x55555555u) - (int)__popc(acc & 0xAAAAAAAAu);
                return acc;
            };
            cw = __any(last) ? block16(std::true_type{}) : block16(std::false_type{});
            if (TRACE) { pend = true; pend_last = last; pend_slot = slot; pend_b = b; }
            cw_out = cw;
            botv_out = bot_start;
        } else {
            cw_out = 0x55555555u;
            botv_out = 0;
        }
    }
    flush();
    if (valid && has_group && g == Lg - 1) {
        DevAlignOut o;
        o.score = best <= k ? (u32)best : 0xFFFFFFFFu;
        o.end_col = (u32)best_col;
        out[job.out_index] = o;
    }
}


template <int W>
__global__ void __launch_bounds__(64, (W <= 2 ? 4 : W <= 5 ? 3 : W <= 8 ? 2 : 1)) ed_exists_block_kernel(const u8* __restrict__ text, const u64* __restrict__ peq,
                                                             const DevAlignJob* __restrict__ jobs, u32 n_jobs, u32 log2_r,
                                                             DevAlignOut* __restrict__ out, const u32* __restrict__ n_jobs_dev, u32 queue, u32* __restrict__ err) {
    extern __shared__ __attribute__((aligned(16))) u64 lds_eq[];
    if (n_jobs_dev) n_jobs = min(n_jobs, *n_jobs_dev);
    u32 const jobs_per_wave = 64u >> log2_r;
    for (u32 blk = blockIdx.x; blk * jobs_per_wave < n_jobs; blk += gridDim.x)
        ed_block_body<W, false>(text, peq, jobs, n_jobs, log2_r, out, blk, lds_eq, nullptr, nullptr, queue, err);
}

template <int W>
__global__ void __launch_bounds__(64, (W <= 4 ? 3 : W <= 6 ? 2 : 1)) ed_trace_block_kernel(const u8* __restrict__ text, const u64* __restrict__ peq,
                                                            const DevAlignJob* __restrict__ jobs, u32 n_jobs, u32 log2_r,
                                                            u64* __restrict__ trace, DevAlignOut* __restrict__ out, u16* __restrict__ lastrow, u32 queue) {
    extern __shared__ __attribute__((aligned(16))) u64 lds_eq[];
    __builtin_amdgcn_s_setprio(2);
    ed_block_body<W, true>(text, peq, jobs, n_jobs, log2_r, out, blockIdx.x, lds_eq, trace, lastrow, queue, nullptr);
}

static u64 shape_width_cap(u32 nw, AlignShape sh) {
    u32 const w = sh.words_per_lane, r = sh.lanes_per_job;
    if ((nw + w - 1) / w <= r) return 0xFFFFFFFFull;
    u64 const no_wait = (u64)64 * w * (r - 1) + r;
    if (sh.queue < 8) return no_wait;
    return no_wait + 16ull * (sh.queue - 5u);
}
u64 DeviceApi::shape_width_cap(u32 nw, AlignShape sh) { return flx::shape_width_cap(nw, sh); }

static AlignShape choose_align_shape_uncached(u32 n, u32 m, u32 k, bool parallel) {
    u32 const nw = (m + 63) / 64;
    i64 const width = (i64)n - (i64)m + 2 * (i64)k;
    static int const stretch = [] { const char* e = getenv("FLX_RING_STRETCH"); int const v = e ? atoi(e) : 135; return v < 100 ? 100 : v; }();
    bool const may_wait = !parallel && stretch > 100;
    AlignShape best{0, 0};
    u64 best_cost = ~0ull;
    u64 shortest = ~0ull, shortest_key = ~0ull;
    for (int pass = 0; pass < (may_wait ? 2 : 1); ++pass)
    for (u32 w : kWordsPerLane)
        for (u32 r = 1; r <= 64; r *= 2) {
            u32 const groups = (nw + w - 1) / w;
            bool ok = groups <= r;
            if (!ok) ok = (i64)64 * w * (r - 1) + r + 1 > width;
            u32 delay = 0;
            if (!ok && may_wait && pass == 1) {
                delay = ring_delay(n, m, k, w, r);
                ok = delay + 1u <= RING_QUEUE_MAX;
            }
            if (!ok) continue;
            u64 const steps = ring_steps(n, m, k, w, r);
            if (pass == 0 && may_wait) { u64 const key = (u64)w * r * 1000 + w; if (key < shortest_key) { shortest_key = key; shortest = steps; } continue; }
            u64 cost;
            if (may_wait) {
                if (steps * 100 > shortest * (u64)stretch) continue;
                cost = steps * r * (8 * w + 1);
            } else cost = parallel ? (u64)w * 1000 + r : (u64)w * r * 1000 + w;
            if (cost < best_cost) { best_cost = cost; best = AlignShape{w, r, ring_queue_for(delay)}; }
        }
    return best;
}

AlignShape choose_align_shape(u32 n, u32 m, u32 k, bool parallel) {
    u32 const nw = (m + 63) / 64;
    i64 const width = (i64)n - (i64)m + 2 * (i64)k;
    if (const char* forced = getenv("FLX_FORCE_SHAPE")) {
        u32 w = 0, r = 0;
        if (sscanf(forced, "%u,%u", &w, &r) == 2 && w && r) {
            if ((nw + w - 1) / w <= r || (i64)64 * w * (r - 1) + r + 1 > width) return AlignShape{w, r};
            u32 const delay = ring_delay(n, m, k, w, r);
            if (delay + 1u <= RING_QUEUE_MAX) return AlignShape{w, r, ring_queue_for(delay)};
        }
    }
    struct Entry { u32 n, m, k; AlignShape shape; bool valid; };
    thread_local Entry memo[2][256] = {};
    Entry& e = memo[parallel ? 1 : 0][(m * 31u + n * 7u + k) & 255u];
    if (e.valid && e.n == n && e.m == m && e.k == k) return e.shape;
    e = Entry{n, m, k, choose_align_shape_uncached(n, m, k, parallel), true};
    return e.shape;
}
u32 align_supported_max_query() { return 25u * 64u * 64u; }

u64 align_trace_slots(u32 n, u32 m, u32 k, AlignShape sh) {
    TraceLayout const tl = ckpt_trace_layout(n, m, k, sh.words_per_lane, sh.lanes_per_job);
    return tl.carry_slots + tl.ckpt_slots;
}

template <class F, int... Ws>
static int with_words_per_lane(u32 words_per_lane, F&& f, std::integer_sequence<int, Ws...>) {
    int rc = (int)hipErrorInvalidValue;
    (void)((words_per_lane == (u32)Ws && ((rc = f(std::integral_constant<int, Ws>{})), true)) || ...);
    return rc;
}
template <class F>
static int with_words_per_lane(u32 words_per_lane, F&& f) {
    return with_words_per_lane(words_per_lane, f, std::integer_sequence<int, 1, 2, 3, 4, 5, 6, 8, 13, 25>{});
}
static u32 log2_lanes(AlignShape shape) {
    u32 log2_g = 0;
    while ((1u << log2_g) < shape.lanes_per_job) ++log2_g;
    return log2_g;
}
static size_t block_lds_bytes(u32 w, u32 jobs_per_wave, u32 queue) {
    return (size_t)7 * 64 * w * sizeof(u64) + (size_t)jobs_per_wave * queue * sizeof(uint2);
}

template <int W>
static int launch_align(hipStream_t s, const u8* d_text, const u64* d_peq, const DevAlignJob* d_jobs, u32 n_jobs, u32 log2_g, bool trace,
                        u64* d_trace, DevAlignOut* d_out, u16* d_lastrow, u32 queue) {
    u32 const jobs_per_wave = 64u >> log2_g;
    u32 const blocks = (n_jobs + jobs_per_wave - 1) / jobs_per_wave;
    size_t const lds_b = block_lds_bytes(W, jobs_per_wave, queue);
    if (trace) {
        (void)hipFuncSetAttribute(reinterpret_cast<const void*>(&ed_trace_block_kernel<W>), hipFuncAttributeMaxDynamicSharedMemorySize, (int)lds_b);
        hipLaunchKernelGGL((ed_trace_block_kernel<W>), dim3(blocks), dim3(64), lds_b, s, d_text, d_peq, d_jobs, n_jobs, log2_g, d_trace, d_out, d_lastrow, queue);
    } else {
        (void)hipFuncSetAttribute(reinterpret_cast<const void*>(&ed_exists_block_kernel<W>), hipFuncAttributeMaxDynamicSharedMemorySize, (int)lds_b);
        hipLaunchKernelGGL((ed_exists_block_kernel<W>), dim3(blocks), dim3(64), lds_b, s, d_text, d_peq, d_jobs, n_jobs, log2_g, d_out, (const u32*)nullptr, queue, (u32*)nullptr);
    }
    return (int)hipGetLastError();
}

template <int W>
static int launch_exists_counted(hipStream_t s, const u8* d_text, const u64* d_peq, const DevAlignJob* d_jobs, u32 max_jobs, u32 log2_g, DevAlignOut* d_out,
                                 const u32* d_n_jobs, u32 max_waves, u32 queue, u32* d_err) {
    u32 const jobs_per_wave = 64u >> log2_g;
    u32 const blocks = std::max(1u, std::min((max_jobs + jobs_per_wave - 1) / jobs_per_wave, max_waves));
    size_t const lds_b = block_lds_bytes(W, jobs_per_wave, queue);
    (void)hipFuncSetAttribute(reinterpret_cast<const void*>(&ed_exists_block_kernel<W>), hipFuncAttributeMaxDynamicSharedMemorySize, (int)lds_b);
    hipLaunchKernelGGL((ed_exists_block_kernel<W>), dim3(blocks), dim3(64), lds_b, s, d_text, d_peq, d_jobs, max_jobs, log2_g, d_out, d_n_jobs, queue, d_err);
    return (int)hipGetLastError();
}
int DeviceApi::align_exists_counted(void* stream, const u8* d_text, const u64* d_peq, const DevAlignJob* d_jobs, u32 max_jobs, const u32* d_n_jobs,
                                    AlignShape shape, u32 max_waves, DevAlignOut* d_out, u32* d_err) {
    if (max_jobs == 0) return 0;
    return with_words_per_lane(shape.words_per_lane, [&](auto w) {
        return launch_exists_counted<decltype(w)::value>((hipStream_t)stream, d_text, d_peq, d_jobs, max_jobs, log2_lanes(shape), d_out, d_n_jobs, max_waves, shape.queue, d_err);
    });
}
AlignShape DeviceApi::shape_holding(u32 nw, i64 width, bool parallel) {
    u32 const m = 64u * nw, k = (u32)(std::max<i64>(width, 1) / 4), n = (u32)((i64)m + std::max<i64>(width, 1) - 2 * (i64)k);
    AlignShape sh = choose_align_shape_uncached(n, m, k, parallel);
    if (sh.queue) { u32 const wider = ring_queue_for(ring_delay(n + (u32)(width / 4), m, k, sh.words_per_lane, sh.lanes_per_job) + 3u); if (wider <= RING_QUEUE_MAX) sh.queue = std::max(sh.queue, wider); }
    return sh;
}

int DeviceApi::align(void* stream, const u8* d_text, const u64* d_peq, const DevAlignJob* d_jobs, u32 n_jobs, AlignShape shape, bool trace,
                     u64* d_trace, DevAlignOut* d_out, u16* d_lastrow) {
    if (n_jobs == 0) return 0;
    u32 const queue = RING_QUEUE_MAX;
    return with_words_per_lane(shape.words_per_lane, [&](auto w) {
        return launch_align<decltype(w)::value>((hipStream_t)stream, d_text, d_peq, d_jobs, n_jobs, log2_lanes(shape), trace, d_trace, d_out, d_lastrow, queue);
    });
}

__global__ void __launch_bounds__(64) lastrow_min_kernel(const u16* __restrict__ lastrow, const DevRowWindow* __restrict__ windows,
                                                         u32 n_windows, DevAlignOut* __restrict__ out) {
    u32 const id = blockIdx.x;
    if (id >= n_windows) return;
    DevRowWindow const w = windows[id];
    u32 const lane = threadIdx.x & 63u;
    const u16* __restrict__ row = lastrow + w.first;
    u32 best = 0xFFFFu, col = 0;
    for (u32 c = lane; c < w.n; c += 64u) {
        u32 const v = c < w.skip ? 0xFFFFu : row[c];
        if (v <= best) { best = v; col = c + 1u; }
    }
    u64 key = ((u64)best << 32) | (u64)(0xFFFFFFFFu - col);
#pragma unroll
    for (int off = 32; off > 0; off >>= 1) {
        u64 const other = __shfl_xor(key, off);
        key = other < key ? other : key;
    }
    if (lane == 0) {
        u32 const v = (u32)(key >> 32), c = 0xFFFFFFFFu - (u32)key;
        DevAlignOut o;
        o.score = (v != 0xFFFFu && v <= w.k) ? v : 0xFFFFFFFFu;
        o.end_col = c;
        out[w.out_index] = o;
    }
}

int DeviceApi::lastrow_min(void* stream, const u16* d_lastrow, const DevRowWindow* d_windows, u32 n_windows, DevAlignOut* d_out) {
    if (n_windows == 0) return 0;
    hipLaunchKernelGGL(lastrow_min_kernel, dim3(n_windows), dim3(64), 0, (hipStream_t)stream, d_lastrow, d_windows, n_windows, d_out);
    return (int)hipGetLastError();
}

constexpr u32 TBW_WORDS = 8, TBW_BLOCKS = 8;
constexpr u32 TBW_REF = 1024;

__global__ void __launch_bounds__(64) ed_traceback_wave_kernel(const u8* __restrict__ text, const u64* __restrict__ peq,
                                                               const u64* __restrict__ trace, const DevTraceJob* __restrict__ jobs,
                                                               u32 n_jobs, u32* __restrict__ cigar, DevTraceOut* __restrict__ out) {
    __shared__ ulonglong2 win[64 * 17];
    __shared__ u32 win_valid[64];
    __shared__ u64 eqm[TBW_WORDS][6];
    __shared__ u8 refs[TBW_REF];
    u32 const lane = threadIdx.x & 63u;
    __builtin_amdgcn_s_setprio(2);
    for (u32 id = blockIdx.x; id < n_jobs; id += gridDim.x) {
    __syncthreads();
    DevTraceJob const job = jobs[id];
    const u8* __restrict__ r = text + job.ref_off;
    u32* __restrict__ slab = cigar + job.cigar_off;
    int const W = (int)job.words_per_lane, R = (int)job.lanes;
    int const n = (int)job.n, m = (int)job.m, k = (int)job.k;
    int const band_hi = n - m + k;
    int const nw = (max(m, 1) + 63) >> 6;
    int const Lg = (nw + W - 1) / W;
    int const pad = Lg * 64 * W - max(m, 1);
    TraceLayout const tl = ckpt_trace_layout(job.n, job.m ? job.m : 1u, job.k, (u32)W, (u32)R);
    int const ring_wait = (int)ring_delay(job.n, job.m ? job.m : 1u, job.k, (u32)W, (u32)R);
    const u32* __restrict__ carry = reinterpret_cast<const u32*>(reinterpret_cast<const ulonglong2*>(trace) + job.trace_off);
    const ulonglong2* __restrict__ ckpt = reinterpret_cast<const ulonglong2*>(trace) + job.trace_off + tl.carry_slots;

    u32 wpos = job.cigar_cap;
    int i = m, j = (int)job.end_col;
    u32 cur_op = 0xFFu, cur_len = 0;
    bool overflow = false;
    auto emit = [&](u32 op, u32 len) {
        if (len == 0) return;
        if (op == cur_op) { cur_len += len; return; }
        if (cur_len) {
            if (wpos == 0) overflow = true;
            else { --wpos; if (lane == 0) slab[wpos] = (cur_len << 4) | cur_op; }
        }
        cur_op = op;
        cur_len = len;
    };
    auto first_block = [&](int w, int diag) {
        int const c_lo = 64 * w - pad + diag;
        return (c_lo >= 0 ? c_lo / 16 : -((-c_lo + 15) / 16)) - 1;
    };

    while (i > 0 && !overflow) {
        if (j == 0) { emit(1u, (u32)i); i = 0; break; }
        int const gw_top = (i - 1 + pad) >> 6;
        int const diag = j - i;
        int const ref_base = max(0, j - 640) & ~15;
        __syncthreads();
        for (u32 x = lane; x < TBW_REF; x += 64u) { int const c = ref_base + (int)x; refs[x] = c < n ? r[c] : (u8)7; }
        __syncthreads();
        {
            int const w = gw_top - (int)(lane / TBW_BLOCKS);
            u32 valid = 0;
            if (w >= 0) {
                int const g = w / W, ww = w - g * W, p = g % R;
                int const b = first_block(w, diag) + (int)(lane % TBW_BLOCKS);
                int const r0 = max(0, 64 * W * g - pad), r1 = 64 * W * (g + 1) - pad;
                int const b_lo = max(0, r0 - k) >> 4;
                int b_hi = min(n - 1, r1 - 1 + band_hi) >> 4;
                if (g + 1 < Lg) b_hi = max(b_hi, max(0, r1 - k) >> 4);
                u64 eq[6];
                int const rs = 64 * w - pad;
                u64 const padmask = rs <= -64 ? ~0ull : rs < 0 ? (1ull << (u32)(-rs)) - 1ull : 0ull;
                {
                    i64 const off = (i64)job.q_off + rs;
#pragma unroll
                    for (u32 sy = 0; sy < 6; ++sy) {
                        u64 v = 0;
                        if (rs > -64) {
                            if (off >= 0) {
                                u64 const a = (u64)off >> 6;
                                u32 const sh = (u32)off & 63u;
                                u64 const lo = peq[a * 6 + sy];
                                u64 const hi = peq[(a + 1) * 6 + sy];
                                v = sh ? (lo >> sh) | (hi << (64 - sh)) : lo;
                            } else v = peq[sy] << (u32)(-off);
                        }
                        eq[sy] = v | padmask;
                    }
                    if (lane % TBW_BLOCKS == 0) {
#pragma unroll
                        for (u32 sy = 0; sy < 6; ++sy) eqm[lane / TBW_BLOCKS][sy] = eq[sy];
                    }
                }
                if (b >= b_lo && b <= b_hi && 16 * b >= ref_base && 16 * b + 16 <= ref_base + (int)TBW_REF) {
                    u64 const slot = ((u64)(b + g + (g / R) * ring_wait) * R + p) * W + ww;
                    ulonglong2 const v = ckpt[slot];
                    u64 pv = v.x, mv = v.y;
                    u32 const cw = carry[slot];
#pragma unroll 4
                    for (u32 sidx = 0; sidx < 16u; ++sidx) {
                        u32 const cb = (cw >> (2u * sidx)) & 3u;
                        u64 const c_hp = cb & 1u, c_hn = cb >> 1;
                        u32 const rsym = refs[16 * b + (int)sidx - ref_base] & 7u;
                        u64 const e = rsym == 0 ? eq[0] : rsym == 1 ? eq[1] : rsym == 2 ? eq[2] : rsym == 3 ? eq[3] : rsym == 4 ? eq[4] : rsym == 5 ? eq[5] : padmask;
                        u64 const x_ = e | mv;
                        u64 const sum = pv + (x_ & pv) + c_hn;
// ... 100 lines not shown
```

### floxer_amd/csrc/flx_internal.hpp

```cpp
#pragma once

#include <atomic>
#include <cstddef>
#include <cstdint>
#include <string>
#include <vector>

#include "../../include/floxer_amd.h"

namespace flx {

using u8 = uint8_t;
using u16 = uint16_t;
using u32 = uint32_t;
using u64 = uint64_t;
using i64 = int64_t;

void set_error(const std::string& msg);

void* host_pool_get(size_t bytes);
void host_pool_put(void* p, size_t bytes);
extern std::atomic<void (*)(void* p, size_t bytes, int pin)> host_pool_pin_hook;
template <class T>
struct PoolAlloc {
// ... 24 lines not shown
    std::vector<u32> kmer_table;
};
constexpr u32 KMER_Q = 8;
inline bool index_has_arrays(HostIndex const& H) { return H.text.size() == H.n && H.sa.size() == H.n && !H.occ[0].empty() && !H.occ[1].empty() && !H.kmer_table.empty(); }

struct DevIndex {
    const OccBlock* occ[2];
    const u32* sa;
    const u8* text;
    const u32* kmer;
    const u32* isa;
    const u64* filter;
    const u64* filter_m;
    u32 filter_k, filter_tmin;
    u32 C[7];
    u32 n;
};

constexpr u32 SCH_POS_MASK = 0xFFFFF;
inline u32 sch_pack(u32 pos, u32 l, u32 u, bool right, bool exact_prefix) {
    return pos | (l << 20) | (u << 23) | ((right ? 1u : 0u) << 26) | ((exact_prefix ? 1u : 0u) << 27);
}

struct DevSeed {
    u64 seq_off;
    u64 stack_off;
    u32 length;
    u32 scheme_off;
    u32 frames_searches;
    u32 id;
    u32 flags;
    u32 pad;
};

struct DevFrame {
    u32 v[16];
};
static_assert(sizeof(DevFrame) == 64, "frame is four 16-byte slots");

struct DevHit { u32 seed, lb, len, errors; u64 key; };
struct DevSeedLeaf { u32 from, length, cls, rank; };
struct DevSeedClass { u32 pos_base, count, scheme_off, frames_searches; };
struct DevSeedRead { u64 pool_fwd, pool_rev; u32 leaf_first, n_leaves, seed_base, class_first, flags, pad; };
struct SeedGen {
    std::vector<DevSeedRead, PoolAlloc<DevSeedRead>> reads;
    std::vector<DevSeedLeaf, PoolAlloc<DevSeedLeaf>> leaves;
    std::vector<DevSeedClass, PoolAlloc<DevSeedClass>> classes;
    std::vector<u64, PoolAlloc<u64>> scheme_table;
    u64 n_seeds = 0;
    u32 max_errors = 0, max_length = 0;
};
struct DevSelStat { u8 useful, raw, flag, excluded; u32 excluded_soft; };
struct DevOutAnchor { u32 seed_index, leaf, ref_id, errors; u64 pos; };

struct DevAlignJob {
    u64 ref_off;
    u64 q_off;
    u64 trace_off;
    u32 n, m, k;
    u32 out_index;
    u64 lastrow_off;
};
struct DevAlignOut { u32 score; u32 end_col; };

struct DevRowWindow { u64 first; u32 n, k; u32 out_index, skip; };

struct DevTraceJob {
    u64 ref_off, q_off, trace_off, cigar_off;
    u32 n, m, lanes, words_per_lane;
    u32 end_col, cigar_cap, out_index;
    u32 k;
};
struct DevTraceOut { u32 begin; u32 cigar_start; u32 cigar_len; u32 pad; };

struct DevMdJob {
    u64 ref_off, cigar_off, md_off;
    u32 n;
    u32 md_cap;
    u32 out_index, pad;
};
struct DevMdOut { u32 len; u32 pad; };
constexpr u64 md_slab_bytes(u64 nm) { return 8 * nm + 6; }
constexpr u32 MD_GRID_CAP = 1u << 16;

struct DevCsJob {
    u64 ref_off, q_off;
    u64 cigar_off, cs_off;
    u32 n, m;
    u32 cs_cap;
    u32 out_index;
};
struct DevCsOut { u32 len; u32 pad; };
static_assert(sizeof(DevCsJob) == 48, "device layout");
constexpr u64 cs_slab_bytes(u64 nm, u64 m, u32 form) { return form == 2u ? m + 3 * nm + 1 : 10 * nm + 7; }
constexpr u32 CS_GRID_CAP = 1u << 16;

struct DevTailJob {
    u64 cigar_off;
    u32 out_index;
    u32 w, x_drop, min_rows;
};
struct DevTailOut { u32 left_rows, left_cols, left_errors, left_words, right_rows, right_cols, right_errors, right_words; };
static_assert(sizeof(DevTailOut) == 32 && sizeof(DevTailOut) == sizeof(flx_tail_result), "one 32-byte result per job");
constexpr u32 TAILS_GRID_CAP = 1u << 16;

struct DevLeftAlignJob {
    u64 ref_off, q_off;
    u64 cigar_off, out_off;
    u32 n, m;
    u32 out_cap;
    u32 out_index;
};
struct DevLeftAlignStat { u32 words_in, letters, gaps, moved; };
constexpr u32 LEFT_ALIGN_GRID_CAP = 1u << 16;

struct DevRealignJob {
    u64 ref_off, q_off;
    u64 cigar_off, out_off;
    u64 trace_off;
    u32 n, m;
    u32 out_cap;
    u32 out_index;
    u32 trace_cap;
    u32 pad;
};
struct DevRealignStat { int32_t score; u32 num_errors; int32_t diag_lo, diag_hi; u32 kept, changed; u64 cells; };
static_assert(sizeof(DevRealignJob) == 64 && sizeof(DevRealignStat) == 32, "device layouts");
struct RealignScores;

struct DevExtendJob {
    u64 text_pos, q_pos;
    u32 ref_limit, row_limit;
    int direction;
    u32 w, x_drop, d_max;
    u32 out_index, pad;
};
struct DevExtendOut { u32 rows, cols, errors, reason; u32 last_d; u32 pad[3]; };
constexpr u32 EXTEND_DEFAULT_WEIGHT = 4, EXTEND_DEFAULT_XDROP = 100, EXTEND_DEFAULT_MAX_ERRORS = 1024;
constexpr u32 EXTEND_MAX_ERRORS = 4093;
constexpr u32 EXTEND_GRID_CAP = 1u << 16;
constexpr u32 EXTEND_MAX_WEIGHT = 0xFFFFu, EXTEND_MAX_XDROP = 1u << 30, EXTEND_MAX_ROWS = (1u << 19) - 1;

struct DevVrAnchor {
    i64 diag_rel;
    u64 seq_start, seq_len;
    u64 q_base;
    u32 tree_base;
    u32 query;
};
struct DevVrNode { u32 parent, from, rows, errors; };
enum : u8 { VR_CLIMBING = 0, VR_DEAD = 1, VR_AT_ROOT = 2, VR_SOLO = 3 };

enum : u32 { VR2_N_JOBS = 0 , VR2_N_CLIMBING = 2, VR2_SMALLEST = 3, VR2_WORD_STEPS = 4, VR2_BYTES = 6, VR2_N_REQ = 8, VR2_DONE = 9,
             VR2_QUEUE_ERR = 11 , VR2_SCALARS = 16 };
struct Vr2Buffers {
    const DevVrAnchor* anchors; const DevVrNode* nodes;
    const u32* q_first;
    u32* node; u8* status;
    u32* a_slot;
    DevAlignJob* jobs; DevAlignOut* outs;
    u32* scalars;
};

struct AlignShape { u32 words_per_lane; u32 lanes_per_job; u32 queue = 0; };

struct TraceLayout { u64 steps, carry_words, carry_slots, ckpt_slots; };
#if defined(__HIPCC__)
#define FLX_HD __host__ __device__
#else
#define FLX_HD
#endif

constexpr u32 RING_QUEUE_MAX = 128;
inline u32 ring_queue_for(u32 delay) {
    if (delay == 0) return 0;
    u32 q = 32;
    while (q < delay + 1u) q *= 2;
    return q;
}
FLX_HD inline void ring_group_blocks(int n, int m, int k, int W, int Lg, int pad, int g, int& b_lo, int& b_hi) {
    int const band_hi = n - m + k;
    int const r0 = 64 * W * g - pad > 0 ? 64 * W * g - pad : 0, r1 = 64 * W * (g + 1) - pad;
    b_lo = (r0 - k > 0 ? r0 - k : 0) >> 4;
    int const hi = r1 - 1 + band_hi < n - 1 ? r1 - 1 + band_hi : n - 1;
    b_hi = hi >> 4;
    if (g + 1 < Lg) { int const next_lo = (r1 - k > 0 ? r1 - k : 0) >> 4; if (next_lo > b_hi) b_hi = next_lo; }
}
FLX_HD inline u32 ring_delay(u32 n, u32 m, u32 k, u32 W, u32 R) {
    if (n == 0 || m == 0 || (u64)n + k < m) return 0;
    int const nw = (int)((m + 63u) / 64u), Lg = (nw + (int)W - 1) / (int)W, pad = Lg * 64 * (int)W - (int)m;
    int delay = 0;
    for (int g = 0; g + (int)R < Lg; ++g) {
        int lo0, hi0, lo1, hi1;
        ring_group_blocks((int)n, (int)m, (int)k, (int)W, Lg, pad, g, lo0, hi0);
        ring_group_blocks((int)n, (int)m, (int)k, (int)W, Lg, pad, g + (int)R, lo1, hi1);
        int const d = hi0 - lo1 + 1 - (int)R;
        if (d > delay) delay = d;
    }
    return (u32)delay;
}
FLX_HD inline u32 lastrow_first_written(u32 n, u32 m, u32 k, u32 W) {
    if (n == 0 || m == 0 || (u64)n + k < m) return n;
    int const nw = (int)((m + 63u) / 64u), Lg = (nw + (int)W - 1) / (int)W, pad = Lg * 64 * (int)W - (int)m;
    int lo, hi;
    ring_group_blocks((int)n, (int)m, (int)k, (int)W, Lg, pad, Lg - 1, lo, hi);
    return (u32)lo * 16u;
}
FLX_HD inline u64 ring_offset(u32 g, u32 R, u32 delay) { return (u64)g + (u64)(g / R) * delay; }
FLX_HD inline u64 ring_steps(u32 n, u32 m, u32 k, u32 W, u32 R) {
    u64 const nw = (m + 63u) / 64u, groups = (nw + W - 1) / W;
    return (n ? (u64)(n - 1) / 16 : 0) + ring_offset((u32)groups - 1u, R, ring_delay(n, m, k, W, R)) + 1;
}
FLX_HD inline TraceLayout ckpt_trace_layout(u32 n, u32 m, u32 k, u32 W, u32 R) {
    TraceLayout l;
    l.steps = ring_steps(n, m, k, W, R);
    l.carry_words = l.steps * R * W;
    l.carry_slots = (l.carry_words + 3) / 4;
    l.ckpt_slots = l.steps * R * W;
    return l;
}
AlignShape choose_align_shape(u32 n, u32 m, u32 k, bool parallel = false);
u64 align_trace_slots(u32 n, u32 m, u32 k, AlignShape sh);
u32 align_supported_max_query();
u32 fm_search_max_keyed_length();

struct KernelTimer;

struct ClearItem { u32* ptr; u32 words; u32 value; };
struct ClearList {
    static constexpr u32 MAX = 8;
    ClearItem item[MAX];
    u32 n = 0;
    bool add(void* p, size_t words, u32 value = 0) {
        if (n == MAX || words > 0xFFFFFFFFull) return false;
        if (words) item[n++] = ClearItem{(u32*)p, (u32)words, value};
        return true;
    }
};
struct PublishItem { const u32* src; u32* dst; u32 words; };
struct PublishList {
    static constexpr u32 MAX = 4;
    PublishItem item[MAX];
    u32 n = 0;
    bool add(const void* src, void* dst, size_t words) {
        if (n == MAX || words > 0xFFFFFFFFull) return false;
        if (words) item[n++] = PublishItem{(const u32*)src, (u32*)dst, (u32)words};
        return true;
    }
};

struct DeviceApi {
    static int clear_stage(void* stream, ClearList const& L);
    static int publish_stage(void* stream, PublishList const& L);
    static int lane_overlap_probe(void* stream, u32 iterations, u32* d_out);
    static int suffix_array(int hip_device, const u8* text, u64 n, u32* out);
    static int index_arrays(int hip_device, const u8* text, u64 n, u32* out_sa, u8* out_bwt0, u8* out_bwt1, OccBlock* out_occ0, OccBlock* out_occ1);
    static int build_peq(void* stream, const u8* d_seq, u64 len, u64* d_peq);
    static int search(void* stream, const DevIndex& idx, const u8* d_seq, const u64* d_scheme, const DevSeed* d_seeds,
                      u32 n_seeds, u32 max_hits_per_seed, DevFrame* d_stack, DevHit* d_hits, u32 hit_cap,
                      u32* d_counters, u32* d_seed_cnt = nullptr);
    static int search_filtered(void* stream, const DevIndex& idx, const u8* d_seq, const u32* d_qpack, const u64* d_scheme, const DevSeed* d_seeds,
                               u32 n_seeds, u32 max_hits_per_seed, u32 frame_levels, DevHit* d_hits, u32 hit_cap, DevHit* d_items, u32 item_cap,
                               u32* d_counters, u32* d_seed_cnt, u32* d_seed_rows, void* d_mailboxes, u32 mailbox_waves, u32 concurrent_launches,
                               bool long_seeds, ClearList clears);
    static size_t mailbox_bytes(u32 waves);
    static size_t derived_bytes(u64 n, u32* filter_k_out);
    static int derive_index(void* stream, DevIndex& idx, u32* d_isa, u64* d_filter, u64* d_filter_mirrored = nullptr);
    static int warm_scratch(void* stream);
    static int build_seeds(void* stream, const DevSeedRead* reads, u32 n_reads, const DevSeedLeaf* leaves, const DevSeedClass* classes, DevSeed* out);
    static int pack_pool(void* stream, const u8* d_seq, u64 len, u32* d_qpack);
    static size_t select_scan_bytes(u32 n_seeds);
    static int select(void* stream, const DevHit* d_hits, const u32* d_counters, u32 hit_cap, u32* d_seed_cnt, u32* d_hit_offset,
                      DevHit* d_grouped, u32 n_seeds, const DevIndex& idx, const u64* d_seq_start, u32 n_ref, u32 hard_cap, u32 soft_cap,
                      bool erase, void* d_stat, u32* d_n_out, u32* d_out_offset, DevOutAnchor* d_out, u32 out_cap, u32* d_rows,
                      u32* d_row_offset, DevOutAnchor* d_sparse, u32 sparse_cap, void* d_scan_tmp, size_t scan_bytes, u32* d_lists);
    static int locate(void* stream, const DevIndex& idx, const u32* d_rows, u32 n, u32* d_out);
    static int align(void* stream, const u8* d_text, const u64* d_peq, const DevAlignJob* d_jobs, u32 n_jobs, AlignShape shape,
                     bool trace, u64* d_trace, DevAlignOut* d_out, u16* d_lastrow = nullptr);
    static int vr2_request(void* stream, Vr2Buffers const& B, u32 n_queries, u32 limit, u32 acct_words, u32 width_cap, u32 parity);
    static int vr2_apply(void* stream, Vr2Buffers const& B, u32 n_anchors, u32* host_scalars);
    static int align_exists_counted(void* stream, const u8* d_text, const u64* d_peq, const DevAlignJob* d_jobs, u32 max_jobs, const u32* d_n_jobs,
                                    AlignShape shape, u32 max_waves, DevAlignOut* d_out, u32* d_err = nullptr);
    static AlignShape shape_holding(u32 nw, i64 width, bool parallel);
    static u64 shape_width_cap(u32 nw, AlignShape sh);
    static int lastrow_min(void* stream, const u16* d_lastrow, const DevRowWindow* d_windows, u32 n_windows, DevAlignOut* d_out);
    static int traceback(void* stream, const u8* d_text, const u64* d_peq, const u64* d_trace, const DevTraceJob* d_jobs, u32 n_jobs,
                         u32* d_cigar, DevTraceOut* d_out);
    static int md_build(void* stream, const u8* d_text, const u32* d_cigar, const DevTraceOut* d_trace_out, const DevMdJob* d_jobs, u32 n_jobs,
                        u8* d_md, DevMdOut* d_out);
    static int cs_build(void* stream, const u8* d_text, const u8* d_query, const u32* d_cigar, const DevTraceOut* d_trace_out, const DevCsJob* d_jobs,
                        u32 n_jobs, u32 form, u8* d_cs, DevCsOut* d_out);
    static int cigar_tails(void* stream, const u32* d_cigar, const DevTraceOut* d_trace_out, const DevTailJob* d_jobs, u32 n_jobs, DevTailOut* d_out);
    static int cigar_left_align(void* stream, const u8* d_text, const u8* d_query, const u32* d_cigar, DevTraceOut* d_trace_out, const DevLeftAlignJob* d_jobs,
                                u32 n_jobs, u32* d_cigar_out, DevLeftAlignStat* d_stats);
    static int cigar_realign(void* stream, const u8* d_text, const u8* d_query, const u32* d_cigar, DevTraceOut* d_trace_out, const DevRealignJob* d_jobs,
                             u32 n_jobs, RealignScores const& scores, u32* d_trace, u32* d_cigar_out, DevRealignStat* d_stats);
    static size_t extend_lds_bytes(u32 d_max);
    static int extend(void* stream, const u8* d_text, const u8* d_query, const DevExtendJob* d_jobs, u32 n_jobs, u32 lds_d, DevExtendOut* d_out);
};

u64 ceil_div(u64 a, u64 b);
u64 fp_aware_ceil(double v);
int32_t saturate_i32(u64 v);
u8 char_to_rank(char c);
char rank_to_char(u8 r);
void reverse_complement(const u8* in, u64 n, u8* out);

struct PexTree {
    std::vector<flx_pex_node> inner, leaves;
    const flx_pex_node& root() const { return inner.empty() ? leaves[0] : inner[0]; }
};
PexTree build_pex_tree(u64 len, u64 k, u64 s, bool bottom_up);

struct SearchDef { std::vector<u32> pi, l, u; };
const std::vector<SearchDef>& optimum_scheme(u32 k);
std::vector<u64> expanded_scheme(u32 k, u32 len);

HostIndex* build_host_index(const u8* concat, const u64* lens, u32 n_refs, int hip_device = -1);
int save_host_index(const HostIndex& idx, const char* path);
HostIndex* load_host_index(const char* path);

}

struct flx_index { flx::HostIndex* host = nullptr; };
```

### floxer_amd/csrc/flx_rounds.hip

```cpp
#include <hip/hip_runtime.h>

#include <algorithm>

#include "flx_internal.hpp"

namespace flx {

namespace {

constexpr u32 VR2_TILE = 256;
constexpr u32 VR2_THREADS = 64;
constexpr u64 VR2_NO_KEY = ~0ull;

__device__ __forceinline__ u64 vr2_word_steps(u32 n, u32 m, u32 k, u32 W) {
    u64 const nw = (m + 63u) / 64u;
    i64 const band_hi = (i64)n - (i64)m + (i64)k;
    u64 total = 0;
    for (i64 g = 0; g * W < (i64)nw; ++g) {
        i64 const r0 = 64 * (i64)W * g, r1 = min((i64)m, r0 + 64 * (i64)W);
        i64 const lo = max((i64)0, r0 - (i64)k), hi = min((i64)n - 1, r1 - 1 + band_hi);
        if (hi >= lo) total += (u64)(hi - lo + 1) * (u64)min((i64)W, (i64)nw - g * W);
    }
    return total;
}

__device__ __forceinline__ u64 vr2_key(u32 node, u64 start, u32 solo) { return ((u64)node << 33) | (start << 1) | solo; }

}

__global__ void __launch_bounds__(VR2_THREADS) vr2_request_kernel(Vr2Buffers B, u32 limit, u32 acct_words, u32 width_cap, u32 parity) {
    __shared__ u64 s_key[VR2_TILE];
    __shared__ u32 s_len[VR2_TILE];
    __shared__ u16 s_val[VR2_TILE];
    __shared__ u8 s_flag[VR2_TILE];
    __shared__ u32 s_jobs[VR2_TILE];
    __shared__ u32 s_count, s_base;
    u32 const tid = threadIdx.x;
    u32 const q = blockIdx.x;
    if (q == 0 && tid == 0) {
        B.scalars[VR2_N_CLIMBING] = 0u; B.scalars[VR2_SMALLEST] = 0xFFFFFFFFu; B.scalars[VR2_DONE] = 0u;
        B.scalars[VR2_N_JOBS + (parity ^ 1u)] = 0u;
    }
    u32 const a0 = B.q_first[q], a1 = B.q_first[q + 1];
    u32* const n_jobs = &B.scalars[VR2_N_JOBS + parity];
    for (u32 tile = a0; tile < a1; tile += VR2_TILE) {
        u32 const n_here = min(VR2_TILE, a1 - tile);
        u32 size = 64;
        while (size < n_here) size <<= 1;
        __syncthreads();
        if (tid == 0) s_count = 0;
        __syncthreads();
        u32 mine = 0;
        u32 tree_base = 0;
        for (u32 t = tid; t < size; t += VR2_THREADS) {
            u64 key = VR2_NO_KEY;
            if (t < n_here) {
                u32 const i = tile + t;
                u8 const st = B.status[i];
                if (st == VR_CLIMBING || st == VR_SOLO) {
                    DevVrAnchor const a = B.anchors[i];
                    u32 const nd_i = B.node[i];
                    DevVrNode const nd = B.nodes[a.tree_base + nd_i];
                    if (nd.rows <= limit) {
                        i64 const start_signed = a.diag_rel + (i64)nd.from - (i64)nd.errors;
                        u64 const start = start_signed > 0 ? (u64)start_signed : 0ull;
                        u64 const base = (u64)nd.rows + 2ull * nd.errors + 1ull;
                        key = vr2_key(nd_i, a.seq_start + start, st == VR_SOLO ? 1u : 0u);
                        s_len[t] = (u32)min(base, a.seq_len - start);
                        ++mine;
                    }
                }
            }
            s_key[t] = key;
            s_val[t] = (u16)t;
        }
        if (mine) atomicAdd(&s_count, mine);
        __syncthreads();
        u32 const cnt = s_count;
        if (cnt == 0) continue;
        DevVrAnchor const a_first = B.anchors[tile];
        tree_base = a_first.tree_base;
        for (u32 k = 2; k <= size; k <<= 1)
            for (u32 j = k >> 1; j > 0; j >>= 1) {
                for (u32 t = tid; t < size; t += VR2_THREADS) {
                    u32 const p = t ^ j;
                    if (p > t) {
                        u64 const x = s_key[t], y = s_key[p];
                        bool const up = (t & k) == 0;
                        if ((x > y) == up) { s_key[t] = y; s_key[p] = x; u16 const v = s_val[t]; s_val[t] = s_val[p]; s_val[p] = v; }
                    }
                }
                __syncthreads();
            }
        for (u32 t = tid; t < cnt; t += VR2_THREADS) {
            u64 const key = s_key[t];
            u32 const node = (u32)(key >> 33);
            if (t > 0 && (u32)(s_key[t - 1] >> 33) == node) continue;
            DevVrNode const nd = B.nodes[tree_base + node];
            u64 const d = max((u64)8, (u64)nd.rows / 8ull);
            u64 const first = (key >> 1) & 0xFFFFFFFFull;
            u64 prev_key = VR2_NO_KEY, prev_bucket = ~0ull, c_lo = 0, c_hi = 0;
            bool prev_solo = false;
            for (u32 j = t; j < cnt && (u32)(s_key[j] >> 33) == node; ++j) {
                u64 const kj = s_key[j];
                bool const solo = kj & 1ull;
                u64 const st = (kj >> 1) & 0xFFFFFFFFull;
                u64 const bucket = (st - first) / d;
                u8 f = 0;
                if (kj != prev_key) {
                    u64 const en = st + s_len[s_val[j]];
                    f = 1;
                    u64 const u_hi = max(c_hi, en);
                    bool const too_wide = (u_hi - c_lo) + 2ull * nd.errors > (u64)nd.rows + width_cap;
                    if (j == t || solo || prev_solo || bucket != prev_bucket || too_wide) { f = 3; c_lo = st; c_hi = en; }
                    else c_hi = u_hi;
                }
                s_flag[j] = f;
                prev_key = kj; prev_bucket = bucket; prev_solo = solo;
            }
        }
        __syncthreads();
        for (u32 t = tid; t < size; t += VR2_THREADS) {
            u32 nj = 0;
            if (t < cnt && (s_flag[t] & 2u)) {
                u32 distinct = 0;
                u64 hi_start = 0, lo_end = 0;
                for (u32 j = t; j < cnt && (j == t || !(s_flag[j] & 2u)); ++j) {
                    if (!(s_flag[j] & 1u)) continue;
                    u64 const st = (s_key[j] >> 1) & 0xFFFFFFFFull, en = st + s_len[s_val[j]];
                    if (distinct == 0) { hi_start = st; lo_end = en; } else { hi_start = max(hi_start, st); lo_end = min(lo_end, en); }
                    ++distinct;
                }
                nj = distinct > 1 && lo_end > hi_start ? 2u : 1u;
            }
            s_jobs[t] = nj;
        }
        __syncthreads();
        {
            u32 const per = size / VR2_THREADS;
            u32 const first = tid * per;
            u32 run = 0;
            for (u32 x = 0; x < per; ++x) run += s_jobs[first + x];
            u32 incl = run;
#pragma unroll
            for (u32 off = 1; off < 64u; off <<= 1) { u32 const up = (u32)__shfl_up((int)incl, off); if (tid >= off) incl += up; }
            u32 at = incl - run;
            for (u32 x = 0; x < per; ++x) { u32 const v = s_jobs[first + x]; s_jobs[first + x] = at; at += v; }
            if (tid == VR2_THREADS - 1u) s_base = incl ? atomicAdd(n_jobs, incl) : 0u;
            __syncthreads();
        }
        u32 const base_slot = s_base;
        u64 steps = 0, bytes = 0;
        u32 n_req = 0;
        for (u32 t = tid; t < cnt; t += VR2_THREADS) {
            if (!(s_flag[t] & 2u)) continue;
            u32 const slot = base_slot + s_jobs[t];
            u32 distinct = 0;
            u64 lo_start = 0, hi_start = 0, lo_end = 0, hi_end = 0;
            u32 last = t;
            for (u32 j = t; j < cnt && (j == t || !(s_flag[j] & 2u)); ++j) {
                last = j;
                if (!(s_flag[j] & 1u)) continue;
                u64 const st = (s_key[j] >> 1) & 0xFFFFFFFFull, en = st + s_len[s_val[j]];
                if (distinct == 0) { lo_start = hi_start = st; lo_end = hi_end = en; }
                else { hi_start = max(hi_start, st); lo_start = min(lo_start, st); lo_end = min(lo_end, en); hi_end = max(hi_end, en); }
                ++distinct;
            }
            DevVrNode const nd = B.nodes[tree_base + (u32)(s_key[t] >> 33)];
            u64 const q_off = a_first.q_base + nd.from;
            u32 code;
            if (distinct == 1) {
                B.jobs[slot] = DevAlignJob{lo_start, q_off, 0, (u32)(hi_end - lo_start), nd.rows, nd.errors, slot, 0};
                code = (slot << 2) | 1u;
                steps += vr2_word_steps((u32)(hi_end - lo_start), nd.rows, nd.errors, acct_words); bytes += (hi_end - lo_start) + nd.rows;
            } else if (lo_end > hi_start) {
                B.jobs[slot] = DevAlignJob{hi_start, q_off, 0, (u32)(lo_end - hi_start), nd.rows, nd.errors, slot, 0};
                B.jobs[slot + 1u] = DevAlignJob{lo_start, q_off, 0, (u32)(hi_end - lo_start), nd.rows, nd.errors, slot + 1u, 0};
                code = (slot << 2) | 3u;
                steps += vr2_word_steps((u32)(lo_end - hi_start), nd.rows, nd.errors, acct_words) + vr2_word_steps((u32)(hi_end - lo_start), nd.rows, nd.errors, acct_words);
                bytes += (lo_end - hi_start) + (hi_end - lo_start) + 2ull * nd.rows;
            } else {
                B.jobs[slot] = DevAlignJob{lo_start, q_off, 0, (u32)(hi_end - lo_start), nd.rows, nd.errors, slot, 0};
                code = (slot << 2) | 2u;
                steps += vr2_word_steps((u32)(hi_end - lo_start), nd.rows, nd.errors, acct_words); bytes += (hi_end - lo_start) + nd.rows;
            }
            for (u32 j = t; j <= last; ++j) B.a_slot[tile + s_val[j]] = code;
            n_req += last - t + 1u;
        }
#pragma unroll
        for (int off = 32; off > 0; off >>= 1) { steps += __shfl_xor(steps, off); bytes += __shfl_xor(bytes, off); n_req += (u32)__shfl_xor((int)n_req, off); }
        if (tid == 0u && n_req) {
            atomicAdd(&B.scalars[VR2_N_REQ], n_req);
            atomicAdd((unsigned long long*)&B.scalars[VR2_WORD_STEPS], (unsigned long long)steps);
            atomicAdd((unsigned long long*)&B.scalars[VR2_BYTES], (unsigned long long)bytes);
        }
    }
}

__global__ void __launch_bounds__(256) vr2_apply_kernel(Vr2Buffers B, u32 n, u32* __restrict__ host_scalars) {
    __shared__ u32 s_cnt[4], s_min[4];
    u32 count = 0, smallest = 0xFFFFFFFFu;
    for (u32 i = blockIdx.x * blockDim.x + threadIdx.x; i < n; i += gridDim.x * blockDim.x) {
        u8 st = B.status[i];
        u32 const code = B.a_slot[i];
        if (code != 0xFFFFFFFFu) {
            B.a_slot[i] = 0xFFFFFFFFu;
            u32 const slot = code >> 2;
            bool const has_a = code & 1u, has_b = code & 2u;
            u8 dec;
            if (has_a && B.outs[slot].score != 0xFFFFFFFFu) dec = 1;
            else if (!has_b) dec = 2;
            else if (B.outs[slot + (has_a ? 1u : 0u)].score == 0xFFFFFFFFu) dec = 2;
            else dec = 0;
            if (dec == 1) {
                u32 const tb = B.anchors[i].tree_base;
                u32 const parent = B.nodes[tb + B.node[i]].parent;
                B.node[i] = parent;
                st = B.nodes[tb + parent].parent == 0xFFFFFFFFu ? VR_AT_ROOT : VR_CLIMBING;
            } else st = dec == 2 ? VR_DEAD : VR_SOLO;
            B.status[i] = st;
        }
        if (st == VR_CLIMBING || st == VR_SOLO) {
            ++count;
            u32 const rows = B.nodes[B.anchors[i].tree_base + B.node[i]].rows;
            smallest = min(smallest, rows);
        }
    }
#pragma unroll
    for (int off = 32; off > 0; off >>= 1) {
        count += (u32)__shfl_xor((int)count, off);
        smallest = min(smallest, (u32)__shfl_xor((int)smallest, off));
    }
    if ((threadIdx.x & 63u) == 0u) { s_cnt[threadIdx.x >> 6] = count; s_min[threadIdx.x >> 6] = smallest; }
    __syncthreads();
    if (threadIdx.x == 0) {
        u32 const c = s_cnt[0] + s_cnt[1] + s_cnt[2] + s_cnt[3], m = min(min(s_min[0], s_min[1]), min(s_min[2], s_min[3]));
        if (c) { atomicAdd(&B.scalars[VR2_N_CLIMBING], c); atomicMin(&B.scalars[VR2_SMALLEST], m); }
        __threadfence();
        if (atomicAdd(&B.scalars[VR2_DONE], 1u) == gridDim.x - 1u && host_scalars) {
            __threadfence();
            for (u32 w = 0; w < VR2_SCALARS; ++w) host_scalars[w] = __hip_atomic_load(&B.scalars[w], __ATOMIC_RELAXED, __HIP_MEMORY_SCOPE_AGENT);
            __threadfence_system();
        }
    }
}

int DeviceApi::vr2_request(void* stream, Vr2Buffers const& B, u32 n_queries, u32 limit, u32 acct_words, u32 width_cap, u32 parity) {
    if (n_queries == 0) return 0;
    hipLaunchKernelGGL(vr2_request_kernel, dim3(n_queries), dim3(VR2_THREADS), 0, (hipStream_t)stream, B, limit, std::max(1u, acct_words), width_cap, parity & 1u);
    return (int)hipGetLastError();
}
int DeviceApi::vr2_apply(void* stream, Vr2Buffers const& B, u32 n_anchors, u32* host_scalars) {
    if (n_anchors == 0) return 0;
    hipLaunchKernelGGL(vr2_apply_kernel, dim3(std::min<u32>((n_anchors + 255) / 256, 1024u)), dim3(256), 0, (hipStream_t)stream, B, n_anchors, host_scalars);
    return (int)hipGetLastError();
}

}
```

### floxer_amd/csrc/flx_verify.cpp

```cpp
#include <algorithm>
#include <chrono>
#include <cstdio>
#include <cstdlib>
#include <cstring>
#include <map>
#include <memory>
#include <mutex>
#include <queue>
#include <string>
#include <tuple>
#include <vector>

#include "flx_fm_core.hpp"
#include "flx_mapq.hpp"
#include "flx_partial.hpp"
#include "flx_pipeline.hpp"
#include "flx_realign.hpp"
#include "flx_select.hpp"
#include "flx_tails.hpp"

namespace flx {

namespace {

// ... 150 lines not shown
    hvec<u8> const& pool = RD->pool;
    const u8* d_pool = RD->d_pool.as<u8>();
    hvec<HostAnchor>& anchors = S.anchors;
    hvec<SeedStats>& sstats = S.sstats;
    if (lane->ctx->read_stats) S.st_local = std::make_unique<Stats>(stats_simulated(lane->ctx->read_stats));
    S.t_slice = std::chrono::steady_clock::now();
    FLX_HIP(hipStreamWaitEvent(lane->stream, RD->peq_event, 0));
    int rc = S.use_gen ? search_seeds_device(lane, d_pool, pool.data(), pool.size(), nullptr, 0, P->search, anchors, sstats, nullptr, 0,
                                       RD->d_pack.ptr ? RD->d_pack.as<u32>() : nullptr, nullptr, &S.gen)
                 : SEARCH_NEEDS_HOST_SEEDS;
    if (rc == SEARCH_NEEDS_HOST_SEEDS) {
        if (S.use_gen) build_host_seeds(S, RD);
        rc = search_seeds_device(lane, d_pool, pool.data(), pool.size(), S.seeds.data(), S.seeds.size(), P->search, anchors, sstats, nullptr, 0,
                                 RD->d_pack.ptr ? RD->d_pack.as<u32>() : nullptr, S.seed_flags.data());
    }
    return rc;
}

void anchors_to_reads(Slice& S) {
    hvec<ReadState>& reads = S.reads;
    hvec<u32> const& seed_first = S.seed_first;
    hvec<HostAnchor> const& anchors = S.anchors;
    hvec<SeedStats> const& sstats = S.sstats;
    u64 const step = S.step;
    auto n_sampled = [&](ReadState const& r) { return S.n_sampled(r); };
    Stats* const st_local = S.st_local.get();
    double const search_ms = S.search_ms = std::chrono::duration<double, std::milli>(std::chrono::steady_clock::now() - S.t_slice).count();
    if (st_local) {
        hvec<SeedStatRow> rows;
        for (size_t r = 0; r < reads.size(); ++r) {
            st_local->at(Stats::QUERY_LENGTHS).add(reads[r].len);
            rows.clear();
            u32 const nl = n_sampled(reads[r]);
            for (u32 si = seed_first[r]; si < seed_first[r + 1]; ++si) {
                flx_pex_node const& leaf = reads[r].tree_ref().leaves[(u64)((si - seed_first[r]) % nl) * step];
                st_local->at(Stats::ERRORS_PER_SEED).add(leaf.num_errors);
                st_local->at(Stats::SEED_LENGTHS).add(leaf.to - leaf.from + 1);
                rows.push_back(SeedStatRow{sstats[si].useful, sstats[si].raw, sstats[si].excluded_soft});
            }
            st_local->at(Stats::SEEDS_PER_QUERY).add(rows.size());
            st_local->add_search_result(rows.data(), rows.size());
            st_local->at(Stats::MS_SEARCH).add((u64)(search_ms / (double)std::max<size_t>(1, reads.size())));
        }
    }
    hvec<AnchorState>& A = S.A;
    A.assign(anchors.size(), AnchorState{});
    u32 rd_i = 0;
    for (size_t a = 0; a < anchors.size(); ++a) {
        u32 const si = anchors[a].seed_index;
        if (si < seed_first[rd_i] || si >= seed_first[rd_i + 1]) {
            if (si >= seed_first[rd_i + 1] && rd_i + 2 < seed_first.size() && si < seed_first[rd_i + 2]) ++rd_i;
            else rd_i = (u32)(std::upper_bound(seed_first.begin(), seed_first.end(), si) - seed_first.begin() - 1);
        }
        u32 const nl = n_sampled(reads[rd_i]), local = si - seed_first[rd_i];
        u8 const orientation = local >= nl ? 1 : 0;
        A[a].read = rd_i;
        A[a].orientation = orientation;
        A[a].leaf = (u32)((u64)(local - (orientation ? nl : 0u)) * step);
        A[a].ref_id = anchors[a].ref_id;
        A[a].pos = anchors[a].pos;
        reads[rd_i].anchor_ids[orientation].push_back((u32)a);
    }
}

void verification_order(Slice& S, const flx_params* P) {
    hvec<ReadState> const& reads = S.reads;
    hvec<hvec<u32>>& exec_order = S.exec_order;
    exec_order.assign(reads.size(), hvec<u32>{});
    for (size_t r = 0; r < reads.size(); ++r) {
        hvec<std::pair<u32, u32>> pkgs;
        hvec<u32> concat;
        for (int o = 0; o < 2; ++o) {
            auto const& ids = reads[r].anchor_ids[o];
            for (size_t i = 0; i < ids.size(); i += P->num_anchors_per_verification_task) {
                u32 const cnt = (u32)std::min<size_t>(P->num_anchors_per_verification_task, ids.size() - i);
                pkgs.emplace_back((u32)concat.size(), cnt);
                concat.insert(concat.end(), ids.begin() + i, ids.begin() + i + cnt);
            }
        }
        for (int pid : package_order((int)pkgs.size()))
            for (u32 j = 0; j < pkgs[pid].second; ++j) exec_order[r].push_back(concat[pkgs[pid].first + j]);
    }
}

u32 start_climb(Slice& S, const flx_params* P) {
    u32 n_climbing = 0;
    for (auto& a : S.A) {
        ReadState const& rs = S.reads[a.read];
        flx_pex_node const& leaf = rs.tree_ref().leaves[a.leaf];
        if (P->direct_full_verification || leaf.parent_id == FLX_NULL_ID) { a.at_root = true; continue; }
        a.node = leaf.parent_id;
        if (rs.tree_ref().inner[a.node].parent_id == FLX_NULL_ID) a.at_root = true;
        n_climbing += !a.at_root;
    }
    return n_climbing;
}

int climb_on_device(Slice& S, Lane* lane, const flx_reads* RD) {
    flx_ctx* ctx = lane->ctx;
    HostIndex const& H = *ctx->hidx;
    hvec<ReadState> const& reads = S.reads;
    hvec<AnchorState>& A = S.A;
    const u8* d_text = ctx->didx.text;
    const u64* const d_peq = RD->d_peq.as<u64>();
    int rc;
    u32 const n = (u32)A.size();
    PhaseTimer vprof("rounds");
    std::map<const PexTree*, u32> tree_base;
    hvec<DevVrNode> nodes;
    for (auto const& kv : S.tree_cache) {
        PexTree const& t = *kv.second;
        tree_base[&t] = (u32)nodes.size();
        for (auto const& nd : t.inner) nodes.push_back(DevVrNode{nd.parent_id, nd.from, nd.to - nd.from + 1, nd.num_errors});
    }
    if (nodes.empty()) nodes.push_back(DevVrNode{0xFFFFFFFFu, 0, 1, 0});
    u32 const n_queries = (u32)(2 * reads.size());
    size_t off = 0;
    auto take = [&](size_t bytes) { size_t const at = off; off += (bytes + 255) & ~(size_t)255; return at; };
    size_t const o_anchors = take((size_t)n * sizeof(DevVrAnchor)), o_nodes = take(nodes.size() * sizeof(DevVrNode)), o_qfirst = take(((size_t)n_queries + 1) * 4),
                 o_node = take((size_t)n * 4), o_status = take(n), o_slot = take((size_t)n * 4), o_scalars = take(VR2_SCALARS * 4), image_bytes = off,
                 o_jobs = take((size_t)n * 2 * sizeof(DevAlignJob)), o_outs = take((size_t)n * 2 * sizeof(DevAlignOut));
    if ((rc = lane->vr.ensure(off))) return rc;
    char* const image = (char*)lane->stage_begin(image_bytes);
    if (!image) return FLX_ERR_NO_DEVICE;
    memset(image, 0, image_bytes);
    DevVrAnchor* const da = (DevVrAnchor*)(image + o_anchors);
    u32* const q_first = (u32*)(image + o_qfirst);
    u32* const h_node = (u32*)(image + o_node);
    u8* const h_status = (u8*)(image + o_status);
    memcpy(image + o_nodes, nodes.data(), nodes.size() * sizeof(DevVrNode));
    memset(image + o_slot, 0xFF, (size_t)n * 4);
    u32 n_climbing = 0, smallest = 0xFFFFFFFFu;
    for (u32 i = 0; i < n; ++i) {
        AnchorState const& a = A[i];
        ReadState const& rs = reads[a.read];
        flx_pex_node const& leaf = rs.tree_ref().leaves[a.leaf];
        u32 const tb = tree_base[rs.tree_ptr];
        u32 const query = 2u * a.read + a.orientation;
        q_first[query + 1]++;
        da[i] = DevVrAnchor{(i64)a.pos - (i64)leaf.from, H.seq_start[a.ref_id], H.seq_len[a.ref_id], rs.pool_off[a.orientation], tb, query};
        bool const climbs = a.alive && !a.at_root;
        h_node[i] = climbs ? a.node : 0u;
        h_status[i] = climbs ? VR_CLIMBING : a.at_root ? VR_AT_ROOT : VR_DEAD;
        if (climbs) { ++n_climbing; smallest = std::min(smallest, nodes[tb + a.node].rows); }
        if (i > 0 && 2u * A[i - 1].read + A[i - 1].orientation > query) { set_error("verification rounds: anchors out of query order"); return FLX_ERR_INTERNAL; }
    }
    for (u32 qi = 0; qi < n_queries; ++qi) q_first[qi + 1] += q_first[qi];
    vprof.mark("anchor-table");
    char* const base = (char*)lane->vr.ptr;
    Vr2Buffers B{};
    B.anchors = (const DevVrAnchor*)(base + o_anchors); B.nodes = (const DevVrNode*)(base + o_nodes); B.q_first = (const u32*)(base + o_qfirst);
    B.node = (u32*)(base + o_node); B.status = (u8*)(base + o_status); B.a_slot = (u32*)(base + o_slot);
    B.jobs = (DevAlignJob*)(base + o_jobs); B.outs = (DevAlignOut*)(base + o_outs); B.scalars = (u32*)(base + o_scalars);
    FLX_HIP(hipMemcpyAsync(base, image, image_bytes, hipMemcpyHostToDevice, lane->stream));
    if (!lane->vr_host_scalars) FLX_HIP(hipHostMalloc((void**)&lane->vr_host_scalars, VR2_SCALARS * 4, hipHostMallocMapped));
    vprof.mark("upload");
    u64 const few_waves = align_few_waves();
    u64 prev_jobs = n_climbing / 2, acc_steps = 0, acc_bytes = 0, acc_req = 0;
    for (u32 round = 0; n_climbing > 0; ++round) {
        u64 const limit = (u64)smallest * round_span_percent() / 100;
        u32 nw_max = 0;
        i64 width_max = 0;
        for (auto const& nd : nodes)
            if (nd.rows >= smallest && nd.rows <= limit) {
                nw_max = std::max(nw_max, (nd.rows + 63u) / 64u);
                width_max = std::max<i64>(width_max, 4 * (i64)nd.errors + 1);
            }
        AlignShape const shape_t = DeviceApi::shape_holding(nw_max, width_max, false), shape_p = DeviceApi::shape_holding(nw_max, width_max, true);
        if (shape_t.words_per_lane == 0 || shape_p.words_per_lane == 0) { set_error("query longer than the supported maximum"); return FLX_ERR_UNSUPPORTED; }
        AlignShape const shape = prev_jobs * shape_t.lanes_per_job / 64 >= few_waves ? shape_t : shape_p;
        u64 const width_cap = DeviceApi::shape_width_cap(nw_max, shape);
        u32 const max_jobs = (u32)std::min<u64>(2ull * n_climbing, 2ull * n);
        int const e1 = DeviceApi::vr2_request(lane->stream, B, n_queries, (u32)std::min<u64>(limit, 0xFFFFFFFFu), shape.words_per_lane,
                                              (u32)std::min<u64>(width_cap, 0xFFFFFFFFull), round);
        if (e1) { set_error(std::string("verification round: ") + hipGetErrorString((hipError_t)e1)); return FLX_ERR_NO_DEVICE; }
        rc = timed_launch(lane, "ed_align_exists", 0, 0, [&] {
            static u32 const exists_waves = [] { const char* e = getenv("FLX_EXISTS_MAX_WAVES"); return (u32)(e ? std::max(64, atoi(e)) : 8192); }();
            return DeviceApi::align_exists_counted(lane->stream, d_text, d_peq, B.jobs, max_jobs, B.scalars + VR2_N_JOBS + (round & 1u), shape, exists_waves, B.outs, B.scalars + VR2_QUEUE_ERR);
        });
        if (rc) return rc;
        int const e2 = DeviceApi::vr2_apply(lane->stream, B, n, lane->vr_host_scalars);
        if (e2) { set_error(std::string("verification round: ") + hipGetErrorString((hipError_t)e2)); return FLX_ERR_NO_DEVICE; }
        if ((rc = lane->sync())) return rc;
        u32 sc[VR2_SCALARS];
        memcpy(sc, lane->vr_host_scalars, sizeof(sc));
        if (sc[VR2_QUEUE_ERR]) { set_error("existence tests: a window did not fit the row buffers"); return FLX_ERR_INTERNAL; }
        u64 ws, by;
        memcpy(&ws, &sc[VR2_WORD_STEPS], 8);
        memcpy(&by, &sc[VR2_BYTES], 8);
        if (ctx->timing) {
            std::lock_guard<std::mutex> g(ctx->mu);
            auto it = ctx->stats.find("ed_align_exists");
            if (it != ctx->stats.end()) { it->second.algorithmic_bytes += by - acc_bytes; it->second.work_units += ws - acc_steps; }
        }
        u64 const round_req = sc[VR2_N_REQ] - acc_req;
        acc_steps = ws; acc_bytes = by; acc_req = sc[VR2_N_REQ];
        S.n_inner_requested += round_req;
        if (round_req == 0 && sc[VR2_N_CLIMBING] >= n_climbing) { set_error("verification rounds do not advance"); return FLX_ERR_INTERNAL; }
        prev_jobs = sc[VR2_N_JOBS + (round & 1u)];
        n_climbing = sc[VR2_N_CLIMBING];
        smallest = sc[VR2_SMALLEST];
        vprof.mark("round");
    }
    if ((rc = lane->wait_idle())) return rc;
    if (n) FLX_HIP(hipMemcpyAsync(image + o_node, base + o_node, o_status + n - o_node, hipMemcpyDeviceToHost, lane->stream));
    if ((rc = lane->sync())) return rc;
    for (u32 i = 0; i < n; ++i) {
        AnchorState& a = A[i];
        if (h_status[i] == VR_DEAD && a.alive && !a.at_root) { a.alive = false; a.node = h_node[i]; }
        else if (h_status[i] == VR_AT_ROOT && !a.at_root) { a.at_root = true; a.node = h_node[i]; }
    }
    vprof.mark("read-back");
    return FLX_OK;
}

int climb_on_host(Slice& S, Lane* lane, const flx_reads* RD, ExistsTimes& times) {
    flx_ctx* ctx = lane->ctx;
    HostIndex const& H = *ctx->hidx;
    hvec<ReadState> const& reads = S.reads;
    hvec<AnchorState>& A = S.A;
    const u8* d_text = ctx->didx.text;
    const u64* const d_peq = RD->d_peq.as<u64>();
    int rc;
    hvec<u32> climbing;
    for (u32 ai = 0; ai < A.size(); ++ai) if (A[ai].alive && !A[ai].at_root) climbing.push_back(ai);
    hvec<AlignRequest> reqs;
    hvec<DevAlignOut> outs;
    auto rows_of = [&](AnchorState const& a) { flx_pex_node const& nd = reads[a.read].tree_ref().inner[a.node]; return nd.to - nd.from + 1; };
    struct Climber { u32 anchor, rows; };
    hvec<Climber> climbers, sel, wait, surv;
    u32 smallest = 0xFFFFFFFFu;
    climbers.reserve(climbing.size());
    for (u32 ai : climbing) { u32 const r = rows_of(A[ai]); climbers.push_back(Climber{ai, r}); smallest = std::min(smallest, r); }
    while (!climbers.empty()) {
        u64 const limit = (u64)smallest * round_span_percent() / 100;
        auto const tb0 = std::chrono::steady_clock::now();
        sel.clear();
        wait.clear();
        surv.clear();
        reqs.clear();
        u32 next_smallest = 0xFFFFFFFFu;
        for (Climber const& c : climbers) {
            if (c.rows <= limit) {
                sel.push_back(c);
                reqs.push_back(window_request(S, H, A[c.anchor], reads[A[c.anchor].read].tree_ref().inner[A[c.anchor].node], 0.0, nullptr));
            } else { wait.push_back(c); next_smallest = std::min(next_smallest, c.rows); }
        }
        times.build_requests += std::chrono::duration<double, std::milli>(std::chrono::steady_clock::now() - tb0).count();
        S.n_inner_requested += reqs.size();
        if ((rc = run_exists_jobs(lane, d_text, d_peq, reqs, outs, times))) return rc;
        for (size_t i = 0; i < outs.size(); ++i) {
            AnchorState& a = A[sel[i].anchor];
            if (outs[i].score == 0xFFFFFFFFu) { a.alive = false; continue; }
            a.node = reads[a.read].tree_ref().inner[a.node].parent_id;
            if (reads[a.read].tree_ref().inner[a.node].parent_id == FLX_NULL_ID) a.at_root = true;
            else { u32 const r = rows_of(a); surv.push_back(Climber{sel[i].anchor, r}); next_smallest = std::min(next_smallest, r); }
        }
        climbers.resize(wait.size() + surv.size());
        std::merge(wait.begin(), wait.end(), surv.begin(), surv.end(), climbers.begin(), [](Climber const& x, Climber const& y) { return x.anchor < y.anchor; });
        smallest = next_smallest;
    }
    return FLX_OK;
}

void interval_pass(Slice& S, const flx_params* P, HostIndex const& H) {
    hvec<ReadState> const& reads = S.reads;
    hvec<AnchorState>& A = S.A;
    hvec<hvec<u32>> const& exec_order = S.exec_order;
    Stats* const st_local = S.st_local.get();
    hvec<AlignRequest>& root_reqs = S.root_reqs;
    hvec<u32>& root_anchor = S.root_anchor;
    hvec<Span>& root_spans = S.root_spans;
    auto add_inner_spans = [&](AnchorState const& a) {
        auto const& tree = reads[a.read].tree_ref();
        flx_pex_node const& leaf = tree.leaves[a.leaf];
        if (P->direct_full_verification || leaf.parent_id == FLX_NULL_ID) return;
        for (u32 nd = leaf.parent_id; tree.inner[nd].parent_id != FLX_NULL_ID; nd = tree.inner[nd].parent_id) {
            st_local->at(Stats::SPAN_INNER).add(window_request(S, H, a, tree.inner[nd], 0.0, nullptr).n);
            if (!a.alive && nd == a.node) break;
        }
    };
    for (size_t r = 0; r < reads.size(); ++r) {
        hvec<VerifiedIntervals> cache[2];
        if (P->use_interval_optimization) { cache[0].resize(H.seq_len.size()); cache[1].resize(H.seq_len.size()); }
        for (u32 ai : exec_order[r]) {
            AnchorState& a = A[ai];
            ReadState const& rs = reads[a.read];
            Span sp;
            AlignRequest const req = window_request(S, H, a, rs.tree_ref().root(), P->extra_verification_ratio, &sp);
            if (P->use_interval_optimization) {
                auto& ivs = cache[a.orientation][a.ref_id];
                if (ivs.contains(trim_both({sp.offset, sp.offset + sp.length}, sp.extra))) {
                    if (st_local) st_local->at(Stats::SPAN_ROOT_AVOIDED).add(sp.length);
                    continue;
                }
                if (st_local) add_inner_spans(a);
                if (!(a.alive && a.at_root)) continue;
                ivs.insert({sp.offset, sp.offset + sp.length});
            } else {
                if (st_local) add_inner_spans(a);
                if (!(a.alive && a.at_root)) continue;
            }
            a.wants_root = true;
            if (st_local) st_local->at(Stats::SPAN_ROOT).add(sp.length);
            root_reqs.push_back(req);
            root_anchor.push_back(ai);
            root_spans.push_back(sp);
        }
    }
}

int align_roots(Slice& S, Lane* lane, const flx_params* P, RunOptions const& R, const flx_reads* RD) {
    flx_ctx* ctx = lane->ctx;
    HostIndex const& H = *ctx->hidx;
    hvec<u8> const& pool = RD->pool;
    hvec<AlignRequest> const& root_reqs = S.root_reqs;
    hvec<Span> const& root_spans = S.root_spans;
    hvec<RootAlignment>& root_res = S.root_res;
    root_res.assign(root_reqs.size(), RootAlignment{});
    int rc;
    if (P->without_cigar) {
        if ((rc = ensure_reversed_text(lane))) return rc;
        {
            std::lock_guard<std::mutex> g(RD->peq_mu);
            if (!RD->rev_built) {
                hvec<u8> qrev(pool.rbegin(), pool.rend());
                take_spare_read_buffer(ctx, 3, RD->d_pool_rev);
                take_spare_read_buffer(ctx, 4, RD->d_peq_rev);
                if ((rc = RD->d_pool_rev.ensure(qrev.size() + 256))) return rc;
                FLX_HIP(hipMemcpyAsync(RD->d_pool_rev.ptr, qrev.data(), qrev.size(), hipMemcpyHostToDevice, lane->stream));
                FLX_HIP(hipMemsetAsync((char*)RD->d_pool_rev.ptr + qrev.size(), 0, 192, lane->stream));
                if ((rc = build_peq(lane, RD->d_pool_rev.as<u8>(), qrev.size(), RD->d_peq_rev))) return rc;
                if (!RD->rev_event) FLX_HIP(hipEventCreateWithFlags(&RD->rev_event, hipEventDisableTiming));
                FLX_HIP(hipEventRecord(RD->rev_event, lane->stream));
                FLX_HIP(hipStreamSynchronize(lane->stream));
                RD->rev_built = true;
            }
        }
        FLX_HIP(hipStreamWaitEvent(lane->stream, RD->rev_event, 0));
        hvec<AlignRequest> rev(root_reqs.size());
        for (size_t i = 0; i < rev.size(); ++i)
            rev[i] = AlignRequest{H.n - root_reqs[i].ref_off - root_reqs[i].n, pool.size() - root_reqs[i].q_off - root_reqs[i].m,
                                  root_reqs[i].n, root_reqs[i].m, root_reqs[i].k};
        hvec<DevAlignOut> outs;
        if ((rc = run_score_jobs(lane, ctx->text_rev.as<u8>() + TEXT_PAD, RD->d_peq_rev.as<u64>(), rev, outs, "ed_align_exists"))) return rc;
        for (size_t i = 0; i < outs.size(); ++i)
            if (outs[i].score != 0xFFFFFFFFu) { root_res[i].exists = true; root_res[i].nm = root_res[i].ed = outs[i].score; root_res[i].start = root_spans[i].offset + (root_reqs[i].n - outs[i].end_col); }
    } else {
        hvec<TraceResult> tres;
        TailParams const tails{split_weight(R.split.error_weight), split_x_drop(R.split.x_drop), split_min_tail_rows(R.split.min_tail_rows)};
        if ((rc = S.trace_windows(lane, RD, root_reqs, tres, R.split.enable ? &tails : nullptr))) return rc;
        for (size_t i = 0; i < tres.size(); ++i)
            if (tres[i].exists)
                root_res[i] = RootAlignment{true, root_spans[i].offset + tres[i].begin, tres[i].nm, tres[i].cigar_off, tres[i].cigar_len, tres[i].md_off, tres[i].md_len, tres[i].tail, tres[i].ed, tres[i].cs_off, tres[i].cs_len};
    }
// ... 597 lines not shown
```

### include/floxer_amd.h

```cpp
#ifndef FLOXER_AMD_H
#define FLOXER_AMD_H

#include <stddef.h>
#include <stdint.h>

#ifdef __cplusplus
extern "C" {
#endif

typedef enum flx_status {
    FLX_OK = 0,
    FLX_ERR_INVALID = -1,
    FLX_ERR_NO_DEVICE = -2,
    FLX_ERR_CAPACITY = -3,
    FLX_ERR_UNSUPPORTED = -4,
    FLX_ERR_INTERNAL = -5,
    FLX_ERR_IO = -6
} flx_status;

const char* flx_last_error(void);
const char* flx_version(void);

uint64_t flx_ceil_div(uint64_t a, uint64_t b);
uint64_t flx_floating_point_error_aware_ceil(double value);
// ... 385 lines not shown
int  flx_grid_caps(uint32_t out[16]);

typedef struct flx_sv flx_sv;
typedef struct flx_sv_options { uint32_t min_length, max_distance, min_support, count_secondary, min_mapq; uint32_t reserved[3]; uint64_t initial_capacity; } flx_sv_options;
typedef struct flx_sv_signature { uint32_t type, side_a, side_b, reserved; int32_t ref_a, ref_b; uint32_t pos_a, q; } flx_sv_signature;
typedef struct flx_sv_cluster { uint32_t type, side_a, side_b, support; int32_t ref_a, ref_b; uint32_t pos_a_min, pos_a_max, q_min, q_median, q_max, reserved; } flx_sv_cluster;
int  flx_sv_create(flx_ctx* ctx, const flx_sv_options* o, flx_sv** out);
int  flx_sv_create_for_lengths(int hip_device, const uint64_t* ref_lens, uint32_t n_refs, const flx_sv_options* o, flx_sv** out);
void flx_sv_free(flx_sv* s);
int  flx_sv_add_records(flx_sv* s, const flx_record* records, uint64_t n, const uint32_t* cigar_words, uint64_t n_words,
                        const uint64_t* read_offsets, uint64_t n_reads);
int  flx_sv_add_run(flx_sv* s, const flx_run* run, const uint64_t* read_offsets, uint64_t n_reads);
int  flx_sv_absorb(flx_sv* into, flx_sv* from);
int  flx_sv_finish(flx_sv* s);
uint64_t flx_sv_num_signatures(const flx_sv* s);
int  flx_sv_copy_signatures(const flx_sv* s, uint64_t from, uint64_t to, flx_sv_signature* out);
uint64_t flx_sv_num_clusters(const flx_sv* s);
int  flx_sv_copy_clusters(const flx_sv* s, flx_sv_cluster* out, uint64_t capacity);
int  flx_sv_host(const uint64_t* ref_lens, uint32_t n_refs, const flx_sv_options* o, const flx_record* records, uint64_t n,
                 const uint32_t* cigar_words, uint64_t n_words, const uint64_t* read_offsets, uint64_t n_reads,
                 flx_sv_signature* out, uint64_t* n_signatures );
int  flx_sv_clusters_host(const flx_sv_options* o, const flx_sv_signature* signatures, uint64_t n, flx_sv_cluster* out,
                          uint64_t* n_clusters );

typedef struct flx_errprof flx_errprof;
typedef struct flx_errprof_options { uint32_t count_secondary, min_mapq, flush_threshold; uint32_t reserved[5]; } flx_errprof_options;
typedef struct flx_errprof_table {
    uint64_t pair_eq[36], pair_x[36], ins_len[64], del_len[64], ins_letter[6], del_letter[6], hp_del[34], hp_ins[34];
    uint64_t pos_match[100], pos_mismatch[100], pos_ins[100], pos_clip[100], pos_del[100], eq_run[256], identity[101], totals[8];
    uint64_t reserved[7];
} flx_errprof_table;
int  flx_errprof_create(flx_ctx* ctx, const flx_errprof_options* o, flx_errprof** out);
int  flx_errprof_create_for_text(int hip_device, const uint8_t* ref_ranks_concat, const uint64_t* ref_lens, uint32_t n_refs,
                                 const flx_errprof_options* o, flx_errprof** out);
void flx_errprof_free(flx_errprof* p);
int  flx_errprof_add_records(flx_errprof* p, const flx_record* records, uint64_t n, const uint32_t* cigar_words, uint64_t n_words,
                             const uint8_t* read_pool, const uint64_t* read_offsets, uint64_t n_reads);
int  flx_errprof_add_run(flx_errprof* p, const flx_run* run, const uint8_t* read_pool, const uint64_t* read_offsets, uint64_t n_reads);
int  flx_errprof_add_run_resident(flx_errprof* p, const flx_run* run, const flx_reads* reads);
int  flx_errprof_absorb(flx_errprof* into, flx_errprof* from);
int  flx_errprof_copy(const flx_errprof* p, flx_errprof_table* out);
int  flx_errprof_host(const uint8_t* ref_ranks_concat, const uint64_t* ref_lens, uint32_t n_refs, const flx_errprof_options* o,
                      const flx_record* records, uint64_t n, const uint32_t* cigar_words, uint64_t n_words, const uint8_t* read_pool,
                      const uint64_t* read_offsets, uint64_t n_reads, flx_errprof_table* table );

typedef struct flx_consensus flx_consensus;
typedef struct flx_consensus_options { uint32_t count_secondary, min_mapq, min_depth, min_count, min_permille, mask_low_depth; uint32_t reserved[2]; } flx_consensus_options;
typedef struct flx_consensus_change { int32_t reference_id; uint32_t position , kind, ref_rank, alt_rank, length, count, cov; uint64_t letters; } flx_consensus_change;
typedef struct flx_consensus_allele { int32_t reference_id; uint32_t position , length, count; uint64_t letters; } flx_consensus_allele;
int  flx_consensus_create(flx_ctx* ctx, const flx_consensus_options* o, flx_consensus** out);
int  flx_consensus_create_for_text(int hip_device, const uint8_t* ref_ranks_concat, const uint64_t* ref_lens, uint32_t n_refs,
                                   const flx_consensus_options* o, flx_consensus** out);
void flx_consensus_free(flx_consensus* p);
int  flx_consensus_add_records(flx_consensus* p, const flx_record* records, uint64_t n, const uint32_t* cigar_words, uint64_t n_words,
                               const uint8_t* read_pool, const uint64_t* read_offsets, uint64_t n_reads);
int  flx_consensus_add_run(flx_consensus* p, const flx_run* run, const uint8_t* read_pool, const uint64_t* read_offsets, uint64_t n_reads);
int  flx_consensus_add_run_resident(flx_consensus* p, const flx_run* run, const flx_reads* reads);
int  flx_consensus_finish(flx_consensus* p);
uint64_t flx_consensus_num_letters(const flx_consensus* p, uint32_t reference_id);
int  flx_consensus_copy_letters(const flx_consensus* p, uint32_t reference_id, char* out, uint64_t capacity);
uint64_t flx_consensus_num_changes(const flx_consensus* p);
int  flx_consensus_copy_changes(const flx_consensus* p, flx_consensus_change* out, uint64_t capacity);
uint64_t flx_consensus_num_alleles(const flx_consensus* p);
int  flx_consensus_copy_alleles(const flx_consensus* p, flx_consensus_allele* out, uint64_t capacity);
int  flx_consensus_geometry(uint32_t out[4]);
int  flx_consensus_host(const uint8_t* ref_ranks_concat, const uint64_t* ref_lens, uint32_t n_refs, const flx_consensus_options* o,
                        const flx_record* records, uint64_t n, const uint32_t* cigar_words, uint64_t n_words, const uint8_t* read_pool,
                        const uint64_t* read_offsets, uint64_t n_reads, uint64_t* letter_offsets, char* letters, uint64_t* n_letters,
                        flx_consensus_change* changes, uint64_t* n_changes, flx_consensus_allele* alleles, uint64_t* n_alleles);

typedef struct flx_variants flx_variants;
typedef struct flx_variants_options {
    uint32_t count_secondary, min_mapq, min_depth, min_qual, max_del, cost_match, cost_mismatch, cost_het, prior_het, prior_hom;
    uint32_t reserved[2];
} flx_variants_options;
typedef struct flx_variant {
    int32_t reference_id;
    uint32_t position , kind, ref_rank, alt_rank, length, ref_count, alt_count, cov, gt, gq, qual, pl[3], reserved;
    uint64_t letters;
} flx_variant;
typedef struct flx_variant_allele { int32_t reference_id; uint32_t position , kind, length, count, reserved; uint64_t letters; } flx_variant_allele;
int  flx_variants_create(flx_ctx* ctx, const flx_variants_options* o, flx_variants** out);
int  flx_variants_create_for_text(int hip_device, const uint8_t* ref_ranks_concat, const uint64_t* ref_lens, uint32_t n_refs,
                                  const flx_variants_options* o, flx_variants** out);
void flx_variants_free(flx_variants* p);
int  flx_variants_add_records(flx_variants* p, const flx_record* records, uint64_t n, const uint32_t* cigar_words, uint64_t n_words,
                              const uint8_t* read_pool, const uint64_t* read_offsets, uint64_t n_reads);
int  flx_variants_add_run(flx_variants* p, const flx_run* run, const uint8_t* read_pool, const uint64_t* read_offsets, uint64_t n_reads);
int  flx_variants_add_run_resident(flx_variants* p, const flx_run* run, const flx_reads* reads);
int  flx_variants_finish(flx_variants* p);
uint64_t flx_variants_num_rows(const flx_variants* p);
int  flx_variants_copy_rows(const flx_variants* p, flx_variant* out, uint64_t capacity);
uint64_t flx_variants_num_alleles(const flx_variants* p);
int  flx_variants_copy_alleles(const flx_variants* p, flx_variant_allele* out, uint64_t capacity);
int  flx_variants_geometry(uint32_t out[4]);
int  flx_variants_genotype(const flx_variants_options* o, uint64_t ref_n, uint64_t alt_n, uint64_t oth, uint32_t out[8]);
int  flx_variants_host(const uint8_t* ref_ranks_concat, const uint64_t* ref_lens, uint32_t n_refs, const flx_variants_options* o,
                       const flx_record* records, uint64_t n, const uint32_t* cigar_words, uint64_t n_words, const uint8_t* read_pool,
                       const uint64_t* read_offsets, uint64_t n_reads, flx_variant* rows, uint64_t* n_rows, flx_variant_allele* alleles,
                       uint64_t* n_alleles);

typedef struct flx_paf flx_paf;
typedef struct flx_paf_summary { uint32_t query_start, query_end, ref_end, matches , mismatches , ins_bases, del_bases, gap_opens; } flx_paf_summary;
typedef struct flx_paf_options { uint32_t write_cigar, write_unmapped, mapq_from_records, skip_secondary; uint32_t reserved[4]; } flx_paf_options;
typedef struct flx_paf_writer flx_paf_writer;
int  flx_paf_create(int hip_device, flx_paf** out);
void flx_paf_free(flx_paf* p);
int  flx_paf_summarize(flx_paf* p, const flx_record* records, uint64_t n, const uint32_t* cigar_words, uint64_t n_words,
                       const uint64_t* read_offsets, uint64_t n_reads, const uint64_t* ref_lens, uint32_t n_refs, flx_paf_summary* out);
int  flx_paf_summarize_host(const flx_record* records, uint64_t n, const uint32_t* cigar_words, uint64_t n_words,
                            const uint64_t* read_offsets, uint64_t n_reads, const uint64_t* ref_lens, uint32_t n_refs, flx_paf_summary* out);
int  flx_paf_open(const char* path, const char* const* ref_ids, const uint64_t* ref_lens, uint32_t n_refs, const flx_paf_options* o,
                  flx_paf_writer** out);
int  flx_paf_write(flx_paf_writer* w, const char* const* read_ids, const uint64_t* read_offsets, const flx_record* records, uint64_t n,
                   const uint32_t* cigar_words, const flx_paf_summary* summaries, const int32_t* scores ,
                   const flx_md_ref* cs_refs , const uint8_t* cs_bytes);
int  flx_paf_close(flx_paf_writer* w);

uint64_t flx_run_num_records(const flx_run* run);
uint64_t flx_run_num_cigar_words(const flx_run* run);
int flx_run_copy(const flx_run* run, flx_record* records, uint32_t* cigar_words, uint8_t* skipped);
void flx_run_free(flx_run* run);

typedef struct flx_kernel_stat {
    char name[32];
    uint64_t launches;
    double device_ms;
    uint64_t algorithmic_bytes;
    uint64_t work_units;
} flx_kernel_stat;
int flx_ctx_enable_kernel_timing(flx_ctx* ctx, int enable);
int flx_ctx_reset_kernel_stats(flx_ctx* ctx);
int flx_ctx_get_kernel_stats(flx_ctx* ctx, flx_kernel_stat* out, uint32_t* n );

typedef struct flx_path_counters {
    uint64_t seeds, seeds_with_anchors, seeds_excluded_by_hard_cap, seeds_selected_on_host, anchors, cursor_extensions;
    uint64_t inner_tests_requested, root_alignments_requested, root_alignments_found, records, reads;
    uint64_t search_reruns;
    uint64_t reserved[4];
} flx_path_counters;
int flx_ctx_get_path_counters(flx_ctx* ctx, flx_path_counters* out);
int flx_ctx_reset_path_counters(flx_ctx* ctx);

typedef struct flx_search_counters {
    uint64_t launches;
    uint64_t subtrees_queued;
    uint64_t lane_handovers;
    uint64_t wave_handovers;
    uint64_t walks_abandoned;
    uint64_t reserved[3];
} flx_search_counters;
int flx_ctx_get_search_counters(flx_ctx* ctx, flx_search_counters* out);

typedef struct flx_climb_anchor { uint32_t read, orientation, leaf, reference_id; uint64_t position; } flx_climb_anchor;
typedef struct flx_climb_options { uint32_t driver, reserved[3]; } flx_climb_options;
int flx_climb_anchors(flx_ctx* ctx, const flx_params* params, const flx_reads* reads, const flx_climb_anchor* anchors, uint64_t n_anchors,
                      const flx_climb_options* options, uint8_t* out_status, uint32_t* out_node, uint64_t* out_requests);

typedef struct flx_derived_info { uint32_t filter_k, filter_tmin, have_isa, have_filter, have_filter_mirrored, reserved[3]; } flx_derived_info;
int flx_ctx_derived_info(flx_ctx* ctx, flx_derived_info* out);
int flx_ctx_copy_derived(flx_ctx* ctx, int which, void* out, uint64_t bytes);

int flx_hw_queue_request(int* requested, int* found);

int flx_ctx_lane_overlap(flx_ctx* ctx, uint32_t n_lanes, uint32_t iterations, float* start_ms, float* stop_ms);

typedef struct flx_stats flx_stats;
int flx_stats_create(const char* input_hint, flx_stats** out);
void flx_stats_free(flx_stats* stats);
int flx_stats_merge(flx_stats* into, const flx_stats* other);
uint64_t flx_stats_num_queries(const flx_stats* stats);
int flx_stats_format(const flx_stats* stats, int toml, char* buf, uint64_t* len);
int flx_ctx_set_stats(flx_ctx* ctx, flx_stats* stats);

typedef struct flx_sam_writer flx_sam_writer;
int flx_sam_open(const char* path , const char* const* ref_ids, const uint64_t* ref_lens, uint32_t n_refs,
                 flx_sam_writer** out);
int flx_sam_write(flx_sam_writer* w, const char* const* read_ids, const uint8_t* read_pool, const uint64_t* read_offsets,
                  const char* const* quals, const flx_record* records, uint64_t n_records, const uint32_t* cigar_words);
int flx_sam_write_tagged(flx_sam_writer* w, const char* const* read_ids, const uint8_t* read_pool, const uint64_t* read_offsets,
                         const char* const* quals, const flx_record* records, uint64_t n_records, const uint32_t* cigar_words,
                         const flx_md_ref* md, const uint8_t* md_bytes);
int flx_sam_write_scored(flx_sam_writer* w, const char* const* read_ids, const uint8_t* read_pool, const uint64_t* read_offsets,
                         const char* const* quals, const flx_record* records, uint64_t n_records, const uint32_t* cigar_words,
                         const flx_md_ref* md, const uint8_t* md_bytes, const int32_t* scores);
int flx_sam_write_cs(flx_sam_writer* w, const char* const* read_ids, const uint8_t* read_pool, const uint64_t* read_offsets,
                     const char* const* quals, const flx_record* records, uint64_t n_records, const uint32_t* cigar_words,
                     const flx_md_ref* md, const uint8_t* md_bytes, const int32_t* scores, const flx_md_ref* cs_refs, const uint8_t* cs_bytes);
int flx_sam_close(flx_sam_writer* w);
int flx_sam_set_threads(flx_sam_writer* w, uint32_t n_threads);
int flx_sam_set_mapq(flx_sam_writer* w, int from_records);
int flx_sam_set_sa(flx_sam_writer* w, int on);
int flx_sam_open_sorted(const char* path , const char* spill_path, int hip_device, int write_index,
                        const char* const* ref_ids, const uint64_t* ref_lens, uint32_t n_refs, flx_sam_writer** out);

int flx_sim_genome(uint64_t length, uint64_t seed, uint8_t* out_ranks);
int flx_sim_genome_repeats(uint64_t length, uint64_t seed, uint8_t* out_ranks);
int flx_sim_reads(const uint8_t* genome_concat, const uint64_t* chrom_lens, uint32_t n_chrom, uint64_t n_reads, uint32_t base_len,
                  double error_rate, double revcomp_fraction, uint64_t seed, uint8_t* out_pool, uint64_t pool_capacity,
                  uint64_t* out_offsets, uint32_t* out_chrom, uint64_t* out_pos, uint8_t* out_reverse);

#ifdef __cplusplus
}
#endif
#endif
```

Measured before the change: 186,400.

## Run union existence window only when the intersection window fails

In verification rounds, an overlapping window pair used to produce two jobs, an intersection and a union, and both were always aligned. Now the union job goes to a second half of the job array at a fixed stride. The exists kernel aligns it in a second pass over the same block, and only for lanes whose intersection test found no hit, so union alignments whose outcome is already decided are skipped. It also moves the word-step count into a shared helper and adds counters for skipped and run unions. The cost is a more complex kernel loop with extra ballots and a serialized second pass inside the wave.

```diff
diff --git a/floxer_amd/__init__.py b/floxer_amd/__init__.py
--- a/floxer_amd/__init__.py
+++ b/floxer_amd/__init__.py
@@ -197,6 +197,11 @@
         sc = capi.SearchCounters()
         check(lib().flx_ctx_get_search_counters(self.h, C.byref(sc)))
         return {n: int(getattr(sc, n)) for n, _ in capi.SearchCounters._fields_ if n != "reserved"}
+
+    def rounds_counters(self):
+        rc = capi.RoundsCounters()
+        check(lib().flx_ctx_get_rounds_counters(self.h, C.byref(rc)))
+        return {n: int(getattr(rc, n)) for n, _ in capi.RoundsCounters._fields_ if n != "reserved"}
 
     def derived_info(self):
         di = capi.DerivedInfo()
diff --git a/floxer_amd/capi.py b/floxer_amd/capi.py
--- a/floxer_amd/capi.py
+++ b/floxer_amd/capi.py
@@ -276,6 +276,10 @@
 
 class SearchCounters(C.Structure):
     _fields_ = [(n, C.c_uint64) for n in ("launches", "subtrees_queued", "lane_handovers", "wave_handovers", "walks_abandoned")] + [("reserved", C.c_uint64 * 3)]
+
+
+class RoundsCounters(C.Structure):
+    _fields_ = [(n, C.c_uint64) for n in ("unions_skipped", "unions_run", "word_steps_requested", "word_steps_skipped")] + [("reserved", C.c_uint64 * 4)]
 
 
 class ClimbAnchor(C.Structure):
@@ -314,7 +318,7 @@
     "flx_align_shapes", "flx_align_reads_gaps", "flx_align_reads_resident_gaps", "flx_align_batch_gaps", "flx_left_align", "flx_left_align_batch",
     "flx_realign", "flx_realign_batch", "flx_align_batch_realign", "flx_ctx_get_realign_counters", "flx_align_reads_realign",
     "flx_align_reads_resident_realign", "flx_run_copy_scores", "flx_sam_write_scored",
-    "flx_ctx_get_search_counters", "flx_climb_anchors", "flx_ctx_derived_info", "flx_ctx_copy_derived",
+    "flx_ctx_get_search_counters", "flx_ctx_get_rounds_counters", "flx_climb_anchors", "flx_ctx_derived_info", "flx_ctx_copy_derived",
     "flx_hw_queue_request", "flx_ctx_lane_overlap",
     "flx_align_reads_cs", "flx_align_reads_resident_cs", "flx_run_num_cs_bytes", "flx_run_copy_cs", "flx_align_batch_cs", "flx_cs", "flx_cs_batch",
     "flx_sam_write_cs",
@@ -628,6 +632,7 @@
     L.flx_ctx_get_path_counters.argtypes = [C.c_void_p, C.POINTER(PathCounters)]
     L.flx_ctx_reset_path_counters.argtypes = [C.c_void_p]
     L.flx_ctx_get_search_counters.argtypes = [C.c_void_p, C.POINTER(SearchCounters)]
+    L.flx_ctx_get_rounds_counters.argtypes = [C.c_void_p, C.POINTER(RoundsCounters)]
     L.flx_climb_anchors.argtypes = [C.c_void_p, C.POINTER(Params), C.c_void_p, C.c_void_p, C.c_uint64, C.POINTER(ClimbOptions), u8p, u32p, u64p]
     L.flx_ctx_derived_info.argtypes = [C.c_void_p, C.POINTER(DerivedInfo)]
     L.flx_ctx_copy_derived.argtypes = [C.c_void_p, C.c_int, C.c_void_p, C.c_uint64]
diff --git a/floxer_amd/csrc/flx_capi.cpp b/floxer_amd/csrc/flx_capi.cpp
--- a/floxer_amd/csrc/flx_capi.cpp
+++ b/floxer_amd/csrc/flx_capi.cpp
@@ -302,6 +302,7 @@
     std::lock_guard<std::mutex> g(ctx->mu);
     ctx->path = flx_path_counters{};
     ctx->search = flx_search_counters{};
+    ctx->rounds = flx_rounds_counters{};
     ctx->realign = flx_realign_counters{};
     return FLX_OK;
 }
@@ -309,6 +310,12 @@
     if (!ctx || !out) { set_error("null argument"); return FLX_ERR_INVALID; }
     std::lock_guard<std::mutex> g(ctx->mu);
     *out = ctx->realign;
+    return FLX_OK;
+}
+int flx_ctx_get_rounds_counters(flx_ctx* ctx, flx_rounds_counters* out) {
+    if (!ctx || !out) { set_error("null argument"); return FLX_ERR_INVALID; }
+    std::lock_guard<std::mutex> g(ctx->mu);
+    *out = ctx->rounds;
     return FLX_OK;
 }
 int flx_ctx_get_search_counters(flx_ctx* ctx, flx_search_counters* out) {
diff --git a/floxer_amd/csrc/flx_context.hpp b/floxer_amd/csrc/flx_context.hpp
--- a/floxer_amd/csrc/flx_context.hpp
+++ b/floxer_amd/csrc/flx_context.hpp
@@ -117,6 +117,7 @@
     std::map<std::string, flx_kernel_stat> stats;
     std::vector<std::string> stat_order;
     flx_path_counters path{};
+    flx_rounds_counters rounds{};
     flx_realign_counters realign{};
     flx_search_counters search{};
     flx_stats* read_stats = nullptr;
diff --git a/floxer_amd/csrc/flx_device.hip b/floxer_amd/csrc/flx_device.hip
--- a/floxer_amd/csrc/flx_device.hip
+++ b/floxer_amd/csrc/flx_device.hip
@@ -43,15 +43,15 @@
 static const u32 kWordsPerLane[] = {1, 2, 3, 4, 5, 6, 8, 13, 25};
 
 template <int W, bool TRACE>
-__device__ __forceinline__ void ed_block_body(const u8* __restrict__ text, const u64* __restrict__ peq, const DevAlignJob* __restrict__ jobs, u32 n_jobs,
+__device__ __forceinline__ u64 ed_block_body(const u8* __restrict__ text, const u64* __restrict__ peq, const DevAlignJob* __restrict__ jobs, u32 n_jobs,
                                               u32 log2_r, DevAlignOut* __restrict__ out, u32 blk, u64* __restrict__ lds_eq,
-                                              u64* __restrict__ trace, u16* __restrict__ lastrow, u32 queue, u32* __restrict__ err) {
+                                              u64* __restrict__ trace, u16* __restrict__ lastrow, u32 queue, u32* __restrict__ err, u64 only = ~0ull) {
     u32 const lane = lane_id();
     u32 const R = 1u << log2_r;
     u32 const p = lane & (R - 1u);
     u32 const jobs_per_wave = 64u >> log2_r;
     u32 const job_id = blk * jobs_per_wave + (lane >> log2_r);
-    bool valid = job_id < n_jobs;
+    bool valid = job_id < n_jobs && ((only >> lane) & 1ull);
     DevAlignJob job;
     if (valid) job = jobs[job_id];
     else { job.ref_off = 0; job.q_off = 0; job.trace_off = 0; job.n = 0; job.m = 1; job.k = 0; job.out_index = 0; }
@@ -64,12 +64,14 @@
     int const Lg = (nw + W - 1) / W;
     int const band_hi = n - m + k;
     u32 const src_lane = (lane & ~(R - 1u)) | ((lane - 1u) & (R - 1u));
+    bool unheld = false;
     int delay = valid ? (int)ring_delay((u32)n, (u32)m, (u32)k, (u32)W, R) : 0;
     if (delay > 0 && (u32)delay + 1u > queue) {
         if (err && p == 0u) atomicOr(err, 1u);
         if (p == 0u) { DevAlignOut o; o.score = 0xFFFFFFFFu; o.end_col = 0u; out[job.out_index] = o; }
         valid = false;
         delay = 0;
+        unheld = true;
     }
     bool const any_delay = __any(delay > 0);
     uint2* __restrict__ const hand = reinterpret_cast<uint2*>(lds_eq + 7u * 64u * W) + (size_t)(lane >> log2_r) * queue;
@@ -136,7 +138,7 @@
 
     u32 cw_out = 0x55555555u;
     int botv_out = 0;
-    int bot = 0, best = m, best_col = 0;
+    int bot = 0, best = unheld ? 0x7FFFFFFF : m, best_col = 0;
     uint4 tq_pre = make_uint4(0, 0, 0, 0);
     int pre_b = -1;
     bool pend = false, pend_last = false;
@@ -262,18 +264,53 @@
         o.end_col = (u32)best_col;
         out[job.out_index] = o;
     }
+    if (TRACE) return 0ull;
+    u32 ln = lane_id();
+    asm volatile("" : "+v"(ln));
+    bool const mine = blk * jobs_per_wave + (ln >> log2_r) < n_jobs && ((only >> ln) & 1ull);
+    u64 const held = __ballot(mine && best <= k);
+    u64 const ring = (R == 64u ? ~0ull : (1ull << R) - 1ull) << (ln & ~(R - 1u));
+    return __ballot(mine && !(held & ring));
 }
 
 
 template <int W>
 __global__ void __launch_bounds__(64, (W <= 2 ? 4 : W <= 5 ? 3 : W <= 8 ? 2 : 1)) ed_exists_block_kernel(const u8* __restrict__ text, const u64* __restrict__ peq,
                                                              const DevAlignJob* __restrict__ jobs, u32 n_jobs, u32 log2_r,
-                                                             DevAlignOut* __restrict__ out, const u32* __restrict__ n_jobs_dev, u32 queue, u32* __restrict__ err) {
+                                                             DevAlignOut* __restrict__ out, const u32* __restrict__ n_jobs_dev, u32 queue, u32* __restrict__ err,
+                                                             u32 stride, unsigned long long* __restrict__ acct) {
     extern __shared__ __attribute__((aligned(16))) u64 lds_eq[];
     if (n_jobs_dev) n_jobs = min(n_jobs, *n_jobs_dev);
     u32 const jobs_per_wave = 64u >> log2_r;
-    for (u32 blk = blockIdx.x; blk * jobs_per_wave < n_jobs; blk += gridDim.x)
-        ed_block_body<W, false>(text, peq, jobs, n_jobs, log2_r, out, blk, lds_eq, nullptr, nullptr, queue, err);
+    u32 blk = blockIdx.x;
+    u32 second = 0u;
+    u64 only = ~0ull;
+    while (blk * jobs_per_wave < n_jobs) {
+        u64 const failed = ed_block_body<W, false>(text, peq, jobs + (size_t)second * stride, n_jobs, log2_r, out, blk, lds_eq, nullptr, nullptr, queue, err, only);
+        u64 again = 0ull;
+        if (stride != 0u && second == 0u) {
+            u32 lane = lane_id();
+            asm volatile("" : "+v"(lane));
+            u32 const job_id = blk * jobs_per_wave + (lane >> log2_r);
+            bool const first = (lane & ((1u << log2_r) - 1u)) == 0u;
+            bool const partner = job_id < n_jobs && (jobs[job_id].lastrow_off & 1ull);
+            again = failed & __ballot(partner);
+            if (acct) {
+                bool const skip = partner && first && !((failed >> lane) & 1ull);
+                u64 steps = 0;
+                if (skip) { DevAlignJob const u = jobs[stride + job_id]; steps = banded_word_steps(u.n, u.m, u.k, (u32)W); }
+#pragma unroll
+                for (int off = 32; off > 0; off >>= 1) steps += __shfl_xor(steps, off);
+                u64 const n_skip = (u64)__popcll(__ballot(skip)), n_run = (u64)__popcll(__ballot(partner && first)) - n_skip;
+                if (lane == 0u) {
+                    if (steps) atomicAdd(&acct[0], (unsigned long long)steps);
+                    if (n_skip | n_run) atomicAdd(&acct[1], (unsigned long long)(n_skip | (n_run << 32)));
+                }
+            }
+        }
+        if (again) { second = 1u; only = again; }
+        else { second = 0u; only = ~0ull; blk += gridDim.x; }
+    }
 }
 
 template <int W>
@@ -381,26 +418,26 @@
         hipLaunchKernelGGL((ed_trace_block_kernel<W>), dim3(blocks), dim3(64), lds_b, s, d_text, d_peq, d_jobs, n_jobs, log2_g, d_trace, d_out, d_lastrow, queue);
     } else {
         (void)hipFuncSetAttribute(reinterpret_cast<const void*>(&ed_exists_block_kernel<W>), hipFuncAttributeMaxDynamicSharedMemorySize, (int)lds_b);
-        hipLaunchKernelGGL((ed_exists_block_kernel<W>), dim3(blocks), dim3(64), lds_b, s, d_text, d_peq, d_jobs, n_jobs, log2_g, d_out, (const u32*)nullptr, queue, (u32*)nullptr);
+        hipLaunchKernelGGL((ed_exists_block_kernel<W>), dim3(blocks), dim3(64), lds_b, s, d_text, d_peq, d_jobs, n_jobs, log2_g, d_out, (const u32*)nullptr, queue, (u32*)nullptr, 0u, (unsigned long long*)nullptr);
     }
     return (int)hipGetLastError();
 }
 
 template <int W>
 static int launch_exists_counted(hipStream_t s, const u8* d_text, const u64* d_peq, const DevAlignJob* d_jobs, u32 max_jobs, u32 log2_g, DevAlignOut* d_out,
-                                 const u32* d_n_jobs, u32 max_waves, u32 queue, u32* d_err) {
+                                 const u32* d_n_jobs, u32 max_waves, u32 queue, u32* d_err, u32 stride, unsigned long long* d_acct) {
     u32 const jobs_per_wave = 64u >> log2_g;
     u32 const blocks = std::max(1u, std::min((max_jobs + jobs_per_wave - 1) / jobs_per_wave, max_waves));
     size_t const lds_b = block_lds_bytes(W, jobs_per_wave, queue);
     (void)hipFuncSetAttribute(reinterpret_cast<const void*>(&ed_exists_block_kernel<W>), hipFuncAttributeMaxDynamicSharedMemorySize, (int)lds_b);
-    hipLaunchKernelGGL((ed_exists_block_kernel<W>), dim3(blocks), dim3(64), lds_b, s, d_text, d_peq, d_jobs, max_jobs, log2_g, d_out, d_n_jobs, queue, d_err);
+    hipLaunchKernelGGL((ed_exists_block_kernel<W>), dim3(blocks), dim3(64), lds_b, s, d_text, d_peq, d_jobs, max_jobs, log2_g, d_out, d_n_jobs, queue, d_err, stride, d_acct);
     return (int)hipGetLastError();
 }
 int DeviceApi::align_exists_counted(void* stream, const u8* d_text, const u64* d_peq, const DevAlignJob* d_jobs, u32 max_jobs, const u32* d_n_jobs,
-                                    AlignShape shape, u32 max_waves, DevAlignOut* d_out, u32* d_err) {
+                                    AlignShape shape, u32 max_waves, DevAlignOut* d_out, u32* d_err, u32 stride, u64* d_acct) {
     if (max_jobs == 0) return 0;
     return with_words_per_lane(shape.words_per_lane, [&](auto w) {
-        return launch_exists_counted<decltype(w)::value>((hipStream_t)stream, d_text, d_peq, d_jobs, max_jobs, log2_lanes(shape), d_out, d_n_jobs, max_waves, shape.queue, d_err);
+        return launch_exists_counted<decltype(w)::value>((hipStream_t)stream, d_text, d_peq, d_jobs, max_jobs, log2_lanes(shape), d_out, d_n_jobs, max_waves, shape.queue, d_err, stride, (unsigned long long*)d_acct);
     });
 }
 AlignShape DeviceApi::shape_holding(u32 nw, i64 width, bool parallel) {
diff --git a/floxer_amd/csrc/flx_internal.hpp b/floxer_amd/csrc/flx_internal.hpp
--- a/floxer_amd/csrc/flx_internal.hpp
+++ b/floxer_amd/csrc/flx_internal.hpp
@@ -200,7 +200,9 @@
 enum : u8 { VR_CLIMBING = 0, VR_DEAD = 1, VR_AT_ROOT = 2, VR_SOLO = 3 };
 
 enum : u32 { VR2_N_JOBS = 0 , VR2_N_CLIMBING = 2, VR2_SMALLEST = 3, VR2_WORD_STEPS = 4, VR2_BYTES = 6, VR2_N_REQ = 8, VR2_DONE = 9,
-             VR2_QUEUE_ERR = 11 , VR2_SCALARS = 16 };
+             VR2_QUEUE_ERR = 11 ,
+             VR2_SKIPPED_STEPS = 12 ,
+             VR2_UNIONS_SKIPPED = 14, VR2_UNIONS_RUN = 15 , VR2_SCALARS = 16 };
 struct Vr2Buffers {
     const DevVrAnchor* anchors; const DevVrNode* nodes;
     const u32* q_first;
@@ -208,6 +210,7 @@
     u32* a_slot;
     DevAlignJob* jobs; DevAlignOut* outs;
     u32* scalars;
+    u32 stride;
 };
 
 struct AlignShape { u32 words_per_lane; u32 lanes_per_job; u32 queue = 0; };
@@ -253,6 +256,18 @@
     int lo, hi;
     ring_group_blocks((int)n, (int)m, (int)k, (int)W, Lg, pad, Lg - 1, lo, hi);
     return (u32)lo * 16u;
+}
+FLX_HD inline u64 banded_word_steps(u32 n, u32 m, u32 k, u32 W) {
+    i64 const nw = (i64)((m + 63u) / 64u);
+    i64 const band_hi = (i64)n - (i64)m + (i64)k;
+    u64 total = 0;
+    for (i64 g = 0; g * W < nw; ++g) {
+        i64 const r0 = 64 * (i64)W * g, r1 = (i64)m < r0 + 64 * (i64)W ? (i64)m : r0 + 64 * (i64)W;
+        i64 const lo = r0 - (i64)k > 0 ? r0 - (i64)k : 0, hi = (i64)n - 1 < r1 - 1 + band_hi ? (i64)n - 1 : r1 - 1 + band_hi;
+        i64 const words = (i64)W < nw - g * W ? (i64)W : nw - g * W;
+        if (hi >= lo) total += (u64)(hi - lo + 1) * (u64)words;
+    }
+    return total;
 }
 FLX_HD inline u64 ring_offset(u32 g, u32 R, u32 delay) { return (u64)g + (u64)(g / R) * delay; }
 FLX_HD inline u64 ring_steps(u32 n, u32 m, u32 k, u32 W, u32 R) {
@@ -328,7 +343,7 @@
     static int vr2_request(void* stream, Vr2Buffers const& B, u32 n_queries, u32 limit, u32 acct_words, u32 width_cap, u32 parity);
     static int vr2_apply(void* stream, Vr2Buffers const& B, u32 n_anchors, u32* host_scalars);
     static int align_exists_counted(void* stream, const u8* d_text, const u64* d_peq, const DevAlignJob* d_jobs, u32 max_jobs, const u32* d_n_jobs,
-                                    AlignShape shape, u32 max_waves, DevAlignOut* d_out, u32* d_err = nullptr);
+                                    AlignShape shape, u32 max_waves, DevAlignOut* d_out, u32* d_err = nullptr, u32 stride = 0, u64* d_acct = nullptr);
     static AlignShape shape_holding(u32 nw, i64 width, bool parallel);
     static u64 shape_width_cap(u32 nw, AlignShape sh);
     static int lastrow_min(void* stream, const u16* d_lastrow, const DevRowWindow* d_windows, u32 n_windows, DevAlignOut* d_out);
diff --git a/floxer_amd/csrc/flx_rounds.hip b/floxer_amd/csrc/flx_rounds.hip
--- a/floxer_amd/csrc/flx_rounds.hip
+++ b/floxer_amd/csrc/flx_rounds.hip
@@ -12,17 +12,7 @@
 constexpr u32 VR2_THREADS = 64;
 constexpr u64 VR2_NO_KEY = ~0ull;
 
-__device__ __forceinline__ u64 vr2_word_steps(u32 n, u32 m, u32 k, u32 W) {
-    u64 const nw = (m + 63u) / 64u;
-    i64 const band_hi = (i64)n - (i64)m + (i64)k;
-    u64 total = 0;
-    for (i64 g = 0; g * W < (i64)nw; ++g) {
-        i64 const r0 = 64 * (i64)W * g, r1 = min((i64)m, r0 + 64 * (i64)W);
-        i64 const lo = max((i64)0, r0 - (i64)k), hi = min((i64)n - 1, r1 - 1 + band_hi);
-        if (hi >= lo) total += (u64)(hi - lo + 1) * (u64)min((i64)W, (i64)nw - g * W);
-    }
-    return total;
-}
+__device__ __forceinline__ u64 vr2_word_steps(u32 n, u32 m, u32 k, u32 W) { return banded_word_steps(n, m, k, W); }
 
 __device__ __forceinline__ u64 vr2_key(u32 node, u64 start, u32 solo) { return ((u64)node << 33) | (start << 1) | solo; }
 
@@ -120,21 +110,7 @@
             }
         }
         __syncthreads();
-        for (u32 t = tid; t < size; t += VR2_THREADS) {
-            u32 nj = 0;
-            if (t < cnt && (s_flag[t] & 2u)) {
-                u32 distinct = 0;
-                u64 hi_start = 0, lo_end = 0;
-                for (u32 j = t; j < cnt && (j == t || !(s_flag[j] & 2u)); ++j) {
-                    if (!(s_flag[j] & 1u)) continue;
-                    u64 const st = (s_key[j] >> 1) & 0xFFFFFFFFull, en = st + s_len[s_val[j]];
-                    if (distinct == 0) { hi_start = st; lo_end = en; } else { hi_start = max(hi_start, st); lo_end = min(lo_end, en); }
-                    ++distinct;
-                }
-                nj = distinct > 1 && lo_end > hi_start ? 2u : 1u;
-            }
-            s_jobs[t] = nj;
-        }
+        for (u32 t = tid; t < size; t += VR2_THREADS) s_jobs[t] = t < cnt && (s_flag[t] & 2u) ? 1u : 0u;
         __syncthreads();
         {
             u32 const per = size / VR2_THREADS;
@@ -174,8 +150,8 @@
                 code = (slot << 2) | 1u;
                 steps += vr2_word_steps((u32)(hi_end - lo_start), nd.rows, nd.errors, acct_words); bytes += (hi_end - lo_start) + nd.rows;
             } else if (lo_end > hi_start) {
-                B.jobs[slot] = DevAlignJob{hi_start, q_off, 0, (u32)(lo_end - hi_start), nd.rows, nd.errors, slot, 0};
-                B.jobs[slot + 1u] = DevAlignJob{lo_start, q_off, 0, (u32)(hi_end - lo_start), nd.rows, nd.errors, slot + 1u, 0};
+                B.jobs[slot] = DevAlignJob{hi_start, q_off, 0, (u32)(lo_end - hi_start), nd.rows, nd.errors, slot, 1};
+                B.jobs[B.stride + slot] = DevAlignJob{lo_start, q_off, 0, (u32)(hi_end - lo_start), nd.rows, nd.errors, B.stride + slot, 0};
                 code = (slot << 2) | 3u;
                 steps += vr2_word_steps((u32)(lo_end - hi_start), nd.rows, nd.errors, acct_words) + vr2_word_steps((u32)(hi_end - lo_start), nd.rows, nd.errors, acct_words);
                 bytes += (lo_end - hi_start) + (hi_end - lo_start) + 2ull * nd.rows;
@@ -210,7 +186,7 @@
             u8 dec;
             if (has_a && B.outs[slot].score != 0xFFFFFFFFu) dec = 1;
             else if (!has_b) dec = 2;
-            else if (B.outs[slot + (has_a ? 1u : 0u)].score == 0xFFFFFFFFu) dec = 2;
+            else if (B.outs[has_a ? B.stride + slot : slot].score == 0xFFFFFFFFu) dec = 2;
             else dec = 0;
             if (dec == 1) {
                 u32 const tb = B.anchors[i].tree_base;
diff --git a/floxer_amd/csrc/flx_verify.cpp b/floxer_amd/csrc/flx_verify.cpp
--- a/floxer_amd/csrc/flx_verify.cpp
+++ b/floxer_amd/csrc/flx_verify.cpp
@@ -326,11 +326,12 @@
     B.anchors = (const DevVrAnchor*)(base + o_anchors); B.nodes = (const DevVrNode*)(base + o_nodes); B.q_first = (const u32*)(base + o_qfirst);
     B.node = (u32*)(base + o_node); B.status = (u8*)(base + o_status); B.a_slot = (u32*)(base + o_slot);
     B.jobs = (DevAlignJob*)(base + o_jobs); B.outs = (DevAlignOut*)(base + o_outs); B.scalars = (u32*)(base + o_scalars);
+    B.stride = n;
     FLX_HIP(hipMemcpyAsync(base, image, image_bytes, hipMemcpyHostToDevice, lane->stream));
     if (!lane->vr_host_scalars) FLX_HIP(hipHostMalloc((void**)&lane->vr_host_scalars, VR2_SCALARS * 4, hipHostMallocMapped));
     vprof.mark("upload");
     u64 const few_waves = align_few_waves();
-    u64 prev_jobs = n_climbing / 2, acc_steps = 0, acc_bytes = 0, acc_req = 0;
+    u64 prev_jobs = n_climbing / 2, acc_steps = 0, acc_bytes = 0, acc_req = 0, acc_skipped = 0, unions_skipped = 0, unions_run = 0;
     for (u32 round = 0; n_climbing > 0; ++round) {
         u64 const limit = (u64)smallest * round_span_percent() / 100;
         u32 nw_max = 0;
@@ -344,13 +345,14 @@
         if (shape_t.words_per_lane == 0 || shape_p.words_per_lane == 0) { set_error("query longer than the supported maximum"); return FLX_ERR_UNSUPPORTED; }
         AlignShape const shape = prev_jobs * shape_t.lanes_per_job / 64 >= few_waves ? shape_t : shape_p;
         u64 const width_cap = DeviceApi::shape_width_cap(nw_max, shape);
-        u32 const max_jobs = (u32)std::min<u64>(2ull * n_climbing, 2ull * n);
+        u32 const max_jobs = (u32)std::min<u64>(n_climbing, n);
         int const e1 = DeviceApi::vr2_request(lane->stream, B, n_queries, (u32)std::min<u64>(limit, 0xFFFFFFFFu), shape.words_per_lane,
                                               (u32)std::min<u64>(width_cap, 0xFFFFFFFFull), round);
         if (e1) { set_error(std::string("verification round: ") + hipGetErrorString((hipError_t)e1)); return FLX_ERR_NO_DEVICE; }
         rc = timed_launch(lane, "ed_align_exists", 0, 0, [&] {
             static u32 const exists_waves = [] { const char* e = getenv("FLX_EXISTS_MAX_WAVES"); return (u32)(e ? std::max(64, atoi(e)) : 8192); }();
-            return DeviceApi::align_exists_counted(lane->stream, d_text, d_peq, B.jobs, max_jobs, B.scalars + VR2_N_JOBS + (round & 1u), shape, exists_waves, B.outs, B.scalars + VR2_QUEUE_ERR);
+            return DeviceApi::align_exists_counted(lane->stream, d_text, d_peq, B.jobs, max_jobs, B.scalars + VR2_N_JOBS + (round & 1u), shape, exists_waves, B.outs, B.scalars + VR2_QUEUE_ERR,
+                                                   B.stride, (u64*)(B.scalars + VR2_SKIPPED_STEPS));
         });
         if (rc) return rc;
         int const e2 = DeviceApi::vr2_apply(lane->stream, B, n, lane->vr_host_scalars);
@@ -359,22 +361,31 @@
         u32 sc[VR2_SCALARS];
         memcpy(sc, lane->vr_host_scalars, sizeof(sc));
         if (sc[VR2_QUEUE_ERR]) { set_error("existence tests: a window did not fit the row buffers"); return FLX_ERR_INTERNAL; }
-        u64 ws, by;
+        u64 ws, by, skipped;
         memcpy(&ws, &sc[VR2_WORD_STEPS], 8);
         memcpy(&by, &sc[VR2_BYTES], 8);
+        memcpy(&skipped, &sc[VR2_SKIPPED_STEPS], 8);
         if (ctx->timing) {
             std::lock_guard<std::mutex> g(ctx->mu);
             auto it = ctx->stats.find("ed_align_exists");
-            if (it != ctx->stats.end()) { it->second.algorithmic_bytes += by - acc_bytes; it->second.work_units += ws - acc_steps; }
+            if (it != ctx->stats.end()) { it->second.algorithmic_bytes += by - acc_bytes; it->second.work_units += (ws - acc_steps) - (skipped - acc_skipped); }
         }
         u64 const round_req = sc[VR2_N_REQ] - acc_req;
-        acc_steps = ws; acc_bytes = by; acc_req = sc[VR2_N_REQ];
+        acc_steps = ws; acc_bytes = by; acc_req = sc[VR2_N_REQ]; acc_skipped = skipped;
+        unions_skipped = sc[VR2_UNIONS_SKIPPED]; unions_run = sc[VR2_UNIONS_RUN];
         S.n_inner_requested += round_req;
         if (round_req == 0 && sc[VR2_N_CLIMBING] >= n_climbing) { set_error("verification rounds do not advance"); return FLX_ERR_INTERNAL; }
         prev_jobs = sc[VR2_N_JOBS + (round & 1u)];
         n_climbing = sc[VR2_N_CLIMBING];
         smallest = sc[VR2_SMALLEST];
         vprof.mark("round");
+    }
+    {
+        std::lock_guard<std::mutex> g(ctx->mu);
+        ctx->rounds.unions_skipped += unions_skipped;
+        ctx->rounds.unions_run += unions_run;
+        ctx->rounds.word_steps_skipped += acc_skipped;
+        ctx->rounds.word_steps_requested += acc_steps;
     }
     if ((rc = lane->wait_idle())) return rc;
     if (n) FLX_HIP(hipMemcpyAsync(image + o_node, base + o_node, o_status + n - o_node, hipMemcpyDeviceToHost, lane->stream));
diff --git a/include/floxer_amd.h b/include/floxer_amd.h
--- a/include/floxer_amd.h
+++ b/include/floxer_amd.h
@@ -561,6 +561,15 @@
 } flx_search_counters;
 int flx_ctx_get_search_counters(flx_ctx* ctx, flx_search_counters* out);
 
+typedef struct flx_rounds_counters {
+    uint64_t unions_skipped;
+    uint64_t unions_run;
+    uint64_t word_steps_requested;
+    uint64_t word_steps_skipped;
+    uint64_t reserved[4];
+} flx_rounds_counters;
+int flx_ctx_get_rounds_counters(flx_ctx* ctx, flx_rounds_counters* out);
+
 typedef struct flx_climb_anchor { uint32_t read, orientation, leaf, reference_id; uint64_t position; } flx_climb_anchor;
 typedef struct flx_climb_options { uint32_t driver, reserved[3]; } flx_climb_options;
 int flx_climb_anchors(flx_ctx* ctx, const flx_params* params, const flx_reads* reads, const flx_climb_anchor* anchors, uint64_t n_anchors,
```

Result: slower. 181,500 (-2.6%).
